# h22hyeon/PC-GNN

Measured on NVIDIA B200. Metric: train target-nodes/sec (fwd+bwd), higher is better.
Workload: dtype f32

## Files before the change

### include/pcgnn_b200.h

```cpp
#ifndef PCGNN_B200_H
#define PCGNN_B200_H

#include <stddef.h>
#include <stdint.h>

#ifdef __cplusplus
extern "C" {
#endif

#define PCG_SLOT 64
#define PCG_MAX_REL 8
#define PCG_NORM_MEAN 0
#define PCG_NORM_RSQRT 1

#define PCG_STATUS_WORDS 12
#define PCG_ST_SLOTS 0
#define PCG_ST_OVERFLOW 3

typedef void* pcg_stream_t;

#define PCG_API __attribute__((visibility("default")))

PCG_API const char* pcg_last_error(void);
PCG_API int pcg_version(void);
PCG_API int pcg_device_sms(void);
PCG_API int pcg_set_pdl(int mask);

PCG_API int pcg_score_table(const float* feat, int64_t n_nodes, int F, int64_t ldf, const float* w, const float* b,
                    float* score, const int32_t* pool, int P, float* ps_score, int32_t* ps_pos, int32_t* ps_id,
                    void* workspace, size_t workspace_bytes, pcg_stream_t stream);

PCG_API int pcg_pool_scores(const float* feat, int F, int64_t ldf, const float* w, const float* b, const int32_t* pool,
                    int P, float* pool_score, pcg_stream_t stream);

PCG_API int pcg_stage(const void* src, void* dst, size_t bytes, pcg_stream_t stream);
PCG_API void* pcg_host_device_ptr(void* host_ptr);
PCG_API int pcg_pool_scores_stage(const float* feat, int F, int64_t ldf, const float* w, const float* b, const int32_t* pool,
                          int P, float* pool_score, const void* stage_src, void* stage_dst, size_t stage_bytes,
                          const uint32_t* cursor, uint32_t count, int64_t src_stride_bytes, pcg_stream_t stream);
PCG_API int pcg_stage_indexed(const void* src, void* dst, size_t bytes, uint32_t* cursor, uint32_t count,
                      int64_t src_stride_bytes, int64_t dst_stride_bytes, int bump, pcg_stream_t stream);

PCG_API size_t pcg_sort_pool_workspace_bytes(int P);
PCG_API int pcg_sort_pool(const float* pool_score, const int32_t* pool, int P, float* ps_score, int32_t* ps_pos,
                  int32_t* ps_id, void* workspace, size_t workspace_bytes, pcg_stream_t stream);

PCG_API int pcg_pool_positions(const int32_t* pool, int P, int64_t n_nodes, int32_t* pool_pos_of, pcg_stream_t stream);
PCG_API int pcg_entry_pool_positions(const int32_t* indices, int64_t nnz, const int32_t* pool_pos_of,
                             int32_t* entry_pool_pos, pcg_stream_t stream);

PCG_API size_t pcg_choose_workspace_bytes(int B, int R, int64_t max_degree, int64_t n_nodes);
PCG_API size_t pcg_choose_sticky_offset(int64_t n_nodes);
PCG_API int pcg_choose_workspace_init(void* workspace, size_t workspace_bytes, int64_t n_nodes, pcg_stream_t stream);

PCG_API int pcg_choose(const int64_t* indptr, const int32_t* indices, int64_t n_nodes, int64_t row_lo, int R,
               const float* score,
               const float* entry_score, const float* center_score, const int32_t* targets,
               const int64_t* labels, int B, const double* thresh_host, const int32_t* k_override, double rho,
               const float* ps_score, const int32_t* ps_pos, const int32_t* ps_id, const int32_t* entry_pool_pos, int P,
               int train, int64_t max_degree,
               int32_t* sel_idx, float* sel_dist, int64_t cap_slots, int32_t* slot_item, int32_t* it_slot0,
               int32_t* it_m, int64_t* it_base, int32_t* it_done, int32_t* it_rep, void* workspace,
               size_t workspace_bytes, int32_t* status, int phases, pcg_stream_t stream);

PCG_API int pcg_select_all(const int64_t* indptr, const int32_t* indices, int64_t n_nodes, int R, const int32_t* targets,
                   int B, int add_self, int64_t cap_slots, int32_t* slot_item, int32_t* it_slot0, int32_t* it_m,
                   int64_t* it_base, int32_t* it_extra, int32_t* it_done, int32_t* status, pcg_stream_t stream);

PCG_API int pcg_aggregate(const float* feat, int64_t ldf, const int32_t* idx, const int32_t* slot_item,
                  const int32_t* it_slot0, const int32_t* it_m, const int64_t* it_base, const int32_t* it_extra,
                  const int32_t* it_rep, int copy_dups, int n_items, int64_t cap_slots, const int32_t* status,
                  int norm, float* partial, int32_t* it_done, float* agg, pcg_stream_t stream);

PCG_API int pcg_aggregate_bwd(const float* d_agg, int64_t ldf, const int32_t* idx, const int32_t* slot_item,
                      const int32_t* it_slot0, const int32_t* it_m, const int64_t* it_base, const int32_t* it_extra,
                      int n_items, int64_t cap_slots, const int32_t* status, int norm, float* feat_grad,
                      pcg_stream_t stream);

PCG_API int pcg_dense_fwd(const float* feat, int64_t ldf, int F, const int32_t* targets, int B, int R, int E,
                  const float* agg, const int32_t* agg_rep, const float* const* w_intra_host, const float* w_inter,
                  float* cat, float* out, pcg_stream_t stream);

PCG_API size_t pcg_dense_bwd_scratch_floats(int B, int R, int F, int E);
PCG_API int pcg_dense_bwd(int64_t ldf, int F, int B, int R, int E, const float* agg, const int32_t* agg_rep,
                  const float* w_inter,
                  const float* cat, const float* out, const float* d_out, float* const* d_w_intra_host,
                  float* d_w_inter, float* scratch, pcg_stream_t stream);

PCG_API int pcg_tile_supported(int B, int R, int F, int E);
PCG_API int pcg_tile_fwd(const float* feat, int64_t ldf, int F, const int32_t* targets, int B, int R, int E,
                 const float* agg, int64_t lda, const int32_t* agg_rep, const float* const* w_intra_host,
                 const float* w_inter, const float* w_clf, const float* b_clf, int keep_cat, float* out,
                 float* center, float* cat, pcg_stream_t stream);
PCG_API size_t pcg_tile_scratch_floats(int B, int R, int F, int E);
PCG_API int pcg_tile_train(const float* feat, int64_t ldf, int F, const int32_t* targets, int B, int R, int E,
                   const float* agg, int64_t lda, const int32_t* agg_rep, const float* const* w_intra_host,
                   const float* w_inter, const float* w_clf, const float* b_clf, const float* w_head,
                   const int64_t* labels, float lambda, float* out, float* center, float* logits, float* loss,
                   float* const* d_w_intra_host, float* d_w_inter, float* d_w_clf, float* d_b_clf, float* d_w_head,
                   float* scratch, int pdl, pcg_stream_t stream);

PCG_API size_t pcg_head_scratch_floats(int B, int F, int E);
PCG_API int pcg_center_fwd(const float* feat, int64_t ldf, int F, const int32_t* targets, int B, const float* w,
                   const float* b, float* center, pcg_stream_t stream);
PCG_API int pcg_center_bwd(const float* feat, int64_t ldf, int F, const int32_t* targets, int B, const float* d_center,
                   float* d_w, float* d_b, float* scratch, int32_t* ticket, pcg_stream_t stream);

PCG_API int pcg_head_loss_fwd(const float* emb, int E, int B, const float* w, const float* center,
                      const int64_t* labels, float lambda, float* logits, float* p1, float* q1, float* loss,
                      float* scratch, int32_t* ticket, pcg_stream_t stream);
PCG_API int pcg_head_loss_bwd(const float* emb, int E, int B, const float* w, const int64_t* labels, const float* p1,
                      const float* q1, float lambda, const float* d_loss, float* d_emb, float* d_center, float* d_w,
                      float* scratch, int32_t* ticket, pcg_stream_t stream);

PCG_API size_t pcg_encoder_scratch_floats(int B, int F_in, int E);
PCG_API int pcg_encoder_fwd(const float* agg, int64_t lda, const float* feat, int64_t ldf, const int32_t* targets, int F,
                    const float* w, int B, int E, float* out, pcg_stream_t stream);
PCG_API int pcg_encoder_bwd(const float* agg, int64_t lda, const float* feat, int64_t ldf, const int32_t* targets, int F,
                    int B, int E, const float* out, const float* d_out, float* d_w, float* scratch, int32_t* ticket,
                    pcg_stream_t stream);

PCG_API int pcg_pick_step(const double* cum, int64_t n, const double* u, int64_t k, const int32_t* idx_train,
                  int32_t* out, pcg_stream_t stream);
PCG_API int pcg_pick_step_philox(const double* cum, int64_t n, uint64_t seed, uint64_t offset, int64_t k,
                         const int32_t* idx_train, int32_t* out, pcg_stream_t stream);

PCG_API size_t pcg_comm_region_bytes(int64_t n_params);
PCG_API int pcg_comm_alloc(void** ptr, size_t bytes);
PCG_API int pcg_comm_free(void* ptr);
PCG_API int pcg_comm_export(void* ptr, unsigned char* handle64);
PCG_API int pcg_comm_import(const unsigned char* handle64, void** ptr);
PCG_API int pcg_comm_unmap(void* ptr);
PCG_API int pcg_allreduce_adam(float* grad, float* param, float* m, float* v, int64_t n_params,
                       void* const* peer_regions_host, int rank, int world, uint32_t* epoch, int32_t* ticket,
                       float lr, float beta1, float beta2, float eps, float weight_decay, int do_adam,
                       pcg_stream_t stream);

PCG_API size_t pcg_score_region_bytes(int64_t n_global);
PCG_API int pcg_score_bcast(const float* feat_rows, int64_t n_rows, int F, int64_t ldf, const float* w, const float* b,
                    int64_t row_lo, int64_t n_global, void* const* regions_host, int rank, int world,
                    uint32_t* epoch, pcg_stream_t stream);

#define PCG_METRICS_WORDS 17
#define PCG_MT_AUC 0
#define PCG_MT_F1 1
#define PCG_MT_F1_MACRO 2
#define PCG_MT_RECALL 3
#define PCG_MT_PRECISION 4
#define PCG_MT_RECALL_MACRO 5
#define PCG_MT_PRECISION_MACRO 6
#define PCG_MT_ACCURACY 7
#define PCG_MT_GMEAN 8
#define PCG_MT_BEST_F1_MACRO 9
#define PCG_MT_BEST_THRESHOLD 10
#define PCG_MT_N_POS 11
#define PCG_MT_N_NEG 12
#define PCG_MT_TP 13
#define PCG_MT_FP 14
#define PCG_MT_TN 15
#define PCG_MT_FN 16
PCG_API int pcg_eval_head(const float* emb, int E, int B, const float* w_head, int mode, int64_t n_total,
                  const uint32_t* cursor, uint32_t count, float* prob, pcg_stream_t stream);
PCG_API size_t pcg_binary_metrics_workspace_bytes(int64_t n);
PCG_API int pcg_binary_metrics(const float* prob, const int32_t* labels, int64_t n, double* out, void* workspace,
                       size_t workspace_bytes, pcg_stream_t stream);

#ifdef __cplusplus
}
#endif
#endif
```

### pc-gnn_b200/_lib.py

```python
from __future__ import annotations

import ctypes as C
import os

_HERE = os.path.dirname(os.path.abspath(__file__))
SO_PATH = os.path.join(_HERE, "libpcgnn_b200_trace.so" if os.environ.get("PCG_LIB_VARIANT") == "trace"
                       else "libpcgnn_b200.so")

SLOT = 64
MAX_REL = 8
STATUS_WORDS = 12
ST_SLOTS, ST_OVERFLOW = 0, 3
NORM_MEAN, NORM_RSQRT = 0, 1
KB_MAX_POOL = 8192
METRICS_KEYS = ("auc", "f1", "f1_macro", "recall", "precision", "recall_macro", "precision_macro", "accuracy", "gmean",
                "best_f1_macro", "best_threshold", "n_pos", "n_neg", "tp", "fp", "tn", "fn")
METRICS_WORDS = len(METRICS_KEYS)

_p = C.c_void_p
_i = C.c_int
_l = C.c_int64
_z = C.c_size_t
_d = C.c_double
_u64 = C.c_uint64

SIGNATURES = {
    "pcg_last_error": (C.c_char_p, []),
    "pcg_version": (_i, []),
    "pcg_device_sms": (_i, []),
    "pcg_set_pdl": (_i, [_i]),
    "pcg_score_table": (_i, [_p, _l, _i, _l, _p, _p, _p, _p, _i, _p, _p, _p, _p, _z, _p]),
    "pcg_pool_scores": (_i, [_p, _i, _l, _p, _p, _p, _i, _p, _p]),
    "pcg_stage": (_i, [_p, _p, _z, _p]),
    "pcg_host_device_ptr": (_p, [_p]),
    "pcg_pool_scores_stage": (_i, [_p, _i, _l, _p, _p, _p, _i, _p, _p, _p, _z, _p, C.c_uint32, _l, _p]),
    "pcg_stage_indexed": (_i, [_p, _p, _z, _p, C.c_uint32, _l, _l, _i, _p]),
    "pcg_sort_pool_workspace_bytes": (_z, [_i]),
    "pcg_sort_pool": (_i, [_p, _p, _i, _p, _p, _p, _p, _z, _p]),
    "pcg_choose_workspace_bytes": (_z, [_i, _i, _l, _l]),
    "pcg_choose_sticky_offset": (_z, [_l]),
    "pcg_choose_workspace_init": (_i, [_p, _z, _l, _p]),
    "pcg_pool_positions": (_i, [_p, _i, _l, _p, _p]),
    "pcg_entry_pool_positions": (_i, [_p, _l, _p, _p, _p]),
    "pcg_choose": (_i, [_p, _p, _l, _l, _i, _p, _p, _p, _p, _p, _i, C.POINTER(_d), _p, _d, _p, _p, _p, _p, _i, _i, _l,
                        _p, _p, _l, _p, _p, _p, _p, _p, _p, _p, _z, _p, _i, _p]),
    "pcg_select_all": (_i, [_p, _p, _l, _i, _p, _i, _i, _l, _p, _p, _p, _p, _p, _p, _p, _p]),
    "pcg_aggregate": (_i, [_p, _l, _p, _p, _p, _p, _p, _p, _p, _i, _i, _l, _p, _i, _p, _p, _p, _p]),
    "pcg_aggregate_bwd": (_i, [_p, _l, _p, _p, _p, _p, _p, _p, _i, _l, _p, _i, _p, _p]),
    "pcg_dense_fwd": (_i, [_p, _l, _i, _p, _i, _i, _i, _p, _p, C.POINTER(_p), _p, _p, _p, _p]),
    "pcg_dense_bwd_scratch_floats": (_z, [_i, _i, _i, _i]),
    "pcg_dense_bwd": (_i, [_l, _i, _i, _i, _i, _p, _p, _p, _p, _p, _p, C.POINTER(_p), _p, _p, _p]),
    "pcg_tile_supported": (_i, [_i, _i, _i, _i]),
    "pcg_tile_fwd": (_i, [_p, _l, _i, _p, _i, _i, _i, _p, _l, _p, C.POINTER(_p), _p, _p, _p, _i, _p, _p, _p, _p]),
    "pcg_tile_scratch_floats": (_z, [_i, _i, _i, _i]),
    "pcg_tile_train": (_i, [_p, _l, _i, _p, _i, _i, _i, _p, _l, _p, C.POINTER(_p), _p, _p, _p, _p, _p, C.c_float,
                            _p, _p, _p, _p, C.POINTER(_p), _p, _p, _p, _p, _p, _i, _p]),
    "pcg_head_scratch_floats": (_z, [_i, _i, _i]),
    "pcg_center_fwd": (_i, [_p, _l, _i, _p, _i, _p, _p, _p, _p]),
    "pcg_center_bwd": (_i, [_p, _l, _i, _p, _i, _p, _p, _p, _p, _p, _p]),
    "pcg_head_loss_fwd": (_i, [_p, _i, _i, _p, _p, _p, C.c_float, _p, _p, _p, _p, _p, _p, _p]),
    "pcg_head_loss_bwd": (_i, [_p, _i, _i, _p, _p, _p, _p, C.c_float, _p, _p, _p, _p, _p, _p, _p]),
    "pcg_encoder_scratch_floats": (_z, [_i, _i, _i]),
    "pcg_encoder_fwd": (_i, [_p, _l, _p, _l, _p, _i, _p, _i, _i, _p, _p]),
    "pcg_encoder_bwd": (_i, [_p, _l, _p, _l, _p, _i, _i, _i, _p, _p, _p, _p, _p, _p]),
    "pcg_comm_region_bytes": (_z, [_l]),
    "pcg_comm_alloc": (_i, [C.POINTER(_p), _z]),
    "pcg_comm_free": (_i, [_p]),
    "pcg_comm_export": (_i, [_p, C.c_char_p]),
    "pcg_comm_import": (_i, [C.c_char_p, C.POINTER(_p)]),
    "pcg_comm_unmap": (_i, [_p]),
    "pcg_allreduce_adam": (_i, [_p, _p, _p, _p, _l, C.POINTER(_p), _i, _i, _p, _p, C.c_float, C.c_float, C.c_float,
                                C.c_float, C.c_float, _i, _p]),
    "pcg_score_region_bytes": (_z, [_l]),
    "pcg_score_bcast": (_i, [_p, _l, _i, _l, _p, _p, _l, _l, C.POINTER(_p), _i, _i, _p, _p]),
    "pcg_pick_step": (_i, [_p, _l, _p, _l, _p, _p, _p]),
    "pcg_pick_step_philox": (_i, [_p, _l, _u64, _u64, _l, _p, _p, _p]),
    "pcg_eval_head": (_i, [_p, _i, _i, _p, _i, _l, _p, C.c_uint32, _p, _p]),
    "pcg_binary_metrics_workspace_bytes": (_z, [_l]),
    "pcg_binary_metrics": (_i, [_p, _p, _l, _p, _p, _z, _p]),
}

_lib = None


class PcgError(RuntimeError):
    pass


def lib():
    global _lib
    if _lib is None:
        if not os.path.exists(SO_PATH):
            raise PcgError(
                f"{SO_PATH} is missing: the CUDA extension has not been built "
                "(run `python -c \"import __graft_entry__ as g; g.build()\"`). There is no CPU fallback.")
        L = C.CDLL(SO_PATH)
        for name, (res, args) in SIGNATURES.items():
            fn = getattr(L, name)
            fn.restype = res
            fn.argtypes = args
        _lib = L
    return _lib


def check(rc: int, what: str = ""):
    if rc != 0:
        msg = lib().pcg_last_error().decode("utf-8", "replace")
        raise PcgError(f"{what or 'pcgnn_b200'} failed (code {rc}): {msg}")


def ptr(t):
    return None if t is None else t.data_ptr()


def host_device_ptr(pinned_tensor) -> int:
    dev = lib().pcg_host_device_ptr(pinned_tensor.data_ptr())
    if not dev:
        raise PcgError(lib().pcg_last_error().decode("utf-8", "replace"))
    return int(dev)


class capture:

    def __init__(self, graph, **kw):
        import torch

        self._ctx = torch.cuda.graph(graph, **kw)
        self._was = False

    def __enter__(self):
        import gc

        gc.collect()
        self._was = gc.isenabled()
        gc.disable()
        try:
            return self._ctx.__enter__()
        except BaseException:
            if self._was:
                gc.enable()
            raise

    def __exit__(self, *exc):
        import gc

        try:
            return self._ctx.__exit__(*exc)
        finally:
            if self._was:
                gc.enable()


def stream_ptr():
    import torch

    return torch.cuda.current_stream().cuda_stream
```

### pc-gnn_b200/csrc/pcg_choose.cu

```cuda
#include "pcg_common.cuh"

#include <cooperative_groups.h>
namespace cg = cooperative_groups;




#define PCG_SMALL_MAX 256
#define PCG_WARPS_PER_CTA 8
#define PCG_GRP_NT 256
#define PCG_CTA_MAX 2048
#define PCG_LARGE_NT 1024
#define PCG_CL 8
#define PCG_CL_MAX 16384
#define PCG_HUGE_MAX 131072
#define PCG_HUGE16_MAX 262144
#define PCG_KB_WORDS 256
#define PCG_CAND_CAP 2048
#define PCG_PREP_NT 1024

struct ChooseP {
    const int64_t* indptr;
    const int32_t* indices;
    const float* score;
    const float* entry_score;
    const float* center_score;
    const int32_t* targets;
    const int64_t* labels;
    const int32_t* k_override;
    const float* ps_score;
    const int32_t* ps_pos;
    const int32_t* ps_id;
    const int32_t* entry_pool_pos;
    int64_t n_nodes;
    int64_t row_lo;
    int R, B, P, train;
    double thresh[PCG_MAX_REL];
    double rho;
    int32_t* sel_idx;
    float* sel_dist;
    int64_t cap_slots;
    int32_t* slot_item;
    int32_t* it_slot0;
    int32_t* it_m;
    int64_t* it_base;
    int32_t* it_done;
    int32_t* it_rep;
    int32_t* status;
    int32_t* first;
    int32_t* q_warp;
    int32_t* q_cta;
    int32_t* q_cl;
    int32_t* q_huge;
    int32_t* q_huge16;
    int huge16_ok;
    int32_t* q_big;
    uint32_t* bits_slab;
    int64_t slab_words;
    int32_t* sticky;
};

#ifdef PCG_TRACE
#define PCG_TRACE_SLOTS 40
__device__ long long* g_trace = nullptr;
__device__ __forceinline__ long long trace_now() {
    long long t;
    asm volatile("mov.u64 %0, %%globaltimer;" : "=l"(t));
    return t;
}
#define TRACE(slot) do { if (g_trace && tid == 0) g_trace[(int64_t)w * PCG_TRACE_SLOTS + (slot)] = trace_now(); } while (0)
#define TRACE_VAL(slot, val) do { if (g_trace && tid == 0) g_trace[(int64_t)w * PCG_TRACE_SLOTS + (slot)] = (val); } while (0)
#define PTRACE(slot) do { if (g_trace && threadIdx.x == 0) g_trace[(int64_t)p.R * p.B * PCG_TRACE_SLOTS + (slot)] = trace_now(); } while (0)
#define TRACE0(slot) do { if (g_trace && tid == 0 && cg::this_cluster().block_rank() == 0) g_trace[(int64_t)w * PCG_TRACE_SLOTS + (slot)] = trace_now(); } while (0)
#define TRACE0_VAL(slot, val) do { if (g_trace && tid == 0 && cg::this_cluster().block_rank() == 0) g_trace[(int64_t)w * PCG_TRACE_SLOTS + (slot)] = (val); } while (0)
#else
#define PTRACE(slot) do {} while (0)
#define TRACE(slot) do {} while (0)
#define TRACE_VAL(slot, val) do {} while (0)
#define TRACE0(slot) do {} while (0)
#define TRACE0_VAL(slot, val) do {} while (0)
#endif
template <int NT>
__device__ __forceinline__ void grp_sync() {
    if (NT == 32) __syncwarp(); else __syncthreads();
}

template <int NT>
__device__ __forceinline__ void grp_excl2(bool fa, bool fb, int tid, int* xw, int& ea, int& eb, int& ta, int& tb) {
    const unsigned lt = lanemask_lt();
    unsigned ma = __ballot_sync(PCG_FULL, fa), mb = __ballot_sync(PCG_FULL, fb);
    ea = __popc(ma & lt);
    eb = __popc(mb & lt);
    if (NT == 32) {
        ta = __popc(ma);
        tb = __popc(mb);
    } else {
        constexpr int NW = NT / 32;
        const int wid = tid >> 5, lane = tid & 31;
        if (lane == 0) xw[wid] = __popc(ma) | (__popc(mb) << 16);
        __syncthreads();
        int pk = lane < NW ? xw[lane] : 0;
        int incl = pk;
#pragma unroll
        for (int off = 1; off < NW; off <<= 1) {
            int t = __shfl_up_sync(PCG_FULL, incl, off);
            if (lane >= off) incl += t;
        }
        const int tot = __shfl_sync(PCG_FULL, incl, NW - 1);
        const int mine = __shfl_sync(PCG_FULL, incl - pk, wid);
        ea += mine & 0xffff;
        eb += mine >> 16;
        ta = tot & 0xffff;
        tb = tot >> 16;
        __syncthreads();
    }
}

template <int NT, class Get>
__device__ __forceinline__ void grp_minmax(Get get, int n, int tid, int* xw, uint32_t& kmin, uint32_t& kmax) {
    uint32_t lo = 0xffffffffu, hi = 0u;
    for (int j = tid; j < n; j += NT) { const uint32_t x = get(j); lo = min(lo, x); hi = max(hi, x); }
#pragma unroll
    for (int off = 16; off > 0; off >>= 1) {
        lo = min(lo, __shfl_xor_sync(PCG_FULL, lo, off));
        hi = max(hi, __shfl_xor_sync(PCG_FULL, hi, off));
    }
    if (NT > 32) {
        if (tid == 0) { xw[24] = (int)0xffffffffu; xw[25] = 0; }
        __syncthreads();
        if ((tid & 31) == 0) { atomicMin((uint32_t*)&xw[24], lo); atomicMax((uint32_t*)&xw[25], hi); }
        __syncthreads();
        lo = (uint32_t)xw[24];
        hi = (uint32_t)xw[25];
        __syncthreads();
    }
    kmin = lo;
    kmax = hi;
}
template <int NT, class Get>
__device__ __forceinline__ void radix_select(Get get, int n, int kth, uint32_t* hist, int* xw, int tid, uint32_t& T,
                                             int& need) {
    uint32_t kmin, kmax;
    grp_minmax<NT>(get, n, tid, xw, kmin, kmax);
    if (kmin == kmax) { T = kmin; need = kth; return; }
    int hb = 31 - __clz(kmin ^ kmax);
    uint32_t mask = hb == 31 ? 0u : ~((2u << hb) - 1u);
    uint32_t prefix = kmin & mask;
    int remaining = kth;
    bool first = true;
    while (hb >= 0) {
        const int shift = max(hb - 7, 0);
        const uint32_t dmask = (1u << (hb - shift + 1)) - 1u;
        for (int b = tid; b < 256; b += NT) hist[b] = 0;
        grp_sync<NT>();
        const int n_up = (n + 31) & ~31;
        for (int j = tid; j < n_up; j += NT) {
            const bool valid = j < n;
            const uint32_t key = valid ? get(j) : 0u;
            const bool active = valid && (key & mask) == prefix;
            const uint32_t digit = (key >> shift) & dmask;
            if (first) {
                unsigned rem = __ballot_sync(PCG_FULL, active);
#pragma unroll 1
                for (int it = 0; it < 2 && rem; ++it) {
                    const int ldr = __ffs(rem) - 1;
                    const uint32_t d0 = __shfl_sync(PCG_FULL, digit, ldr);
                    const unsigned same = __ballot_sync(PCG_FULL, active && digit == d0);
                    if ((tid & 31) == ldr) atomicAdd(&hist[d0], (uint32_t)__popc(same));
                    rem &= ~same;
                }
                if ((rem >> (tid & 31)) & 1u) atomicAdd(&hist[digit], 1u);
            } else if (active) {
                atomicAdd(&hist[digit], 1u);
            }
        }
        grp_sync<NT>();
        if (tid < 32) {
            uint32_t c[8];
            int s = 0;
#pragma unroll
            for (int b = 0; b < 8; ++b) { c[b] = hist[tid * 8 + b]; s += (int)c[b]; }
            int incl = s;
#pragma unroll
            for (int off = 1; off < 32; off <<= 1) {
                int t = __shfl_up_sync(PCG_FULL, incl, off);
                if (tid >= off) incl += t;
            }
            int excl = incl - s;
            if (excl < remaining && remaining <= incl) {
                int run = excl;
#pragma unroll
                for (int b = 0; b < 8; ++b) {
                    if (run + (int)c[b] >= remaining) { xw[30] = tid * 8 + b; xw[31] = remaining - run; break; }
                    run += (int)c[b];
                }
            }
        }
        grp_sync<NT>();
        const uint32_t digit = (uint32_t)xw[30];
        remaining = xw[31];
        prefix |= digit << shift;
        mask |= dmask << shift;
        hb = shift - 1;
        first = false;
    }
    T = prefix;
    need = remaining;
}

__device__ __forceinline__ uint32_t pick_digit(int c0, int c1, int c2, int& remaining) {
    if (remaining <= c0) return 0u;
    remaining -= c0;
    if (remaining <= c1) return 1u;
    remaining -= c1;
    if (remaining <= c2) return 2u;
    remaining -= c2;
    return 3u;
}

template <int NT, class Get>
__device__ __forceinline__ void cta_bitselect(Get get, int n, int kth, uint32_t* cand, int cand_cap, int* wsum, int* xw,
                                              int tid, uint32_t& T, int& need) {
    constexpr int NW = NT / 32;
    const int wid = tid >> 5, lane = tid & 31;
    uint32_t kmin, kmax;
    grp_minmax<NT>(get, n, tid, xw, kmin, kmax);
    if (kmin == kmax) { T = kmin; need = kth; return; }
    int hb = 31 - __clz(kmin ^ kmax);
    uint32_t mask = hb == 31 ? 0u : ~((2u << hb) - 1u);
    uint32_t prefix = kmin & mask;
    int remaining = kth;
    bool listed = false;
    int n_list = 0;
    int n_act = n;
    while (hb >= 0) {
        const int shift = max(hb - 1, 0);
        const uint32_t dmask = hb >= 1 ? 3u : 1u;
        int c0 = 0, c1 = 0, c2 = 0;
        const int lim = listed ? n_list : n;
        for (int j = tid; j < lim; j += NT) {
            const uint32_t key = listed ? cand[j] : get(j);
            const bool active = ((key ^ prefix) & mask) == 0u;
            const uint32_t dg = (key >> shift) & dmask;
            c0 += active && dg == 0u;
            c1 += active && dg == 1u;
            c2 += active && dg == 2u;
        }
        c0 = __reduce_add_sync(PCG_FULL, c0);
        c1 = __reduce_add_sync(PCG_FULL, c1);
        c2 = __reduce_add_sync(PCG_FULL, c2);
        if (lane == 0) { wsum[wid * 3] = c0; wsum[wid * 3 + 1] = c1; wsum[wid * 3 + 2] = c2; }
        __syncthreads();
        c0 = lane < NW ? wsum[lane * 3] : 0;
        c1 = lane < NW ? wsum[lane * 3 + 1] : 0;
        c2 = lane < NW ? wsum[lane * 3 + 2] : 0;
        c0 = __reduce_add_sync(PCG_FULL, c0);
        c1 = __reduce_add_sync(PCG_FULL, c1);
        c2 = __reduce_add_sync(PCG_FULL, c2);
        const uint32_t dg = pick_digit(c0, c1, c2, remaining);
        const int cnt_dg = dg == 0u ? c0 : (dg == 1u ? c1 : (dg == 2u ? c2 : n_act - c0 - c1 - c2));
        prefix |= dg << shift;
        mask |= dmask << shift;
        hb = shift - 1;
        n_act = cnt_dg;
        __syncthreads();
        if (!listed && hb >= 0 && n_act <= cand_cap) {
            if (tid == 0) xw[26] = 0;
            __syncthreads();
            const int n_up = (n + 31) & ~31;
            for (int j = tid; j < n_up; j += NT) {
                const uint32_t key = j < n ? get(j) : 0u;
                const bool active = j < n && ((key ^ prefix) & mask) == 0u;
                const unsigned m = __ballot_sync(PCG_FULL, active);
                int base = 0;
                if (lane == 0 && m) base = atomicAdd(&xw[26], __popc(m));
                base = __shfl_sync(PCG_FULL, base, 0);
                if (active) cand[base + __popc(m & lanemask_lt())] = key;
            }
            __syncthreads();
            listed = true;
            n_list = n_act;
        }
    }
    T = prefix;
    need = remaining;
}
template <int NT, int NE, int CL = 1>
__device__ __forceinline__ void hist_select(const uint32_t (&key)[NE], uint32_t vmask, int kth, uint32_t* hist, int* xw,
                                            int tid, uint32_t& T, int& need, uint32_t* chist = nullptr,
                                            int* par = nullptr, int w = 0) {

    constexpr int NH = NT == 32 ? 1 : 8;
    const int lane = tid & 31, wid = tid >> 5;
    uint32_t* myh = hist + (NT == 32 ? 0 : (wid & (NH - 1)) * 256);
    uint32_t prefix = 0u, mask = 0u;
    int remaining = kth;
#pragma unroll 1
    for (int step = 0; step < 4; ++step) {
        const int shift = step == 3 ? 0 : 23 - 8 * step;
        const uint32_t dmask = step == 3 ? 0x7fu : 0xffu;
        if (step == 0) {
            uint32_t pd[3];
            {
                const bool a0 = vmask & 1u;
                const uint32_t dg0 = key[0] >> 23;
                unsigned rem = __ballot_sync(PCG_FULL, a0);
#pragma unroll
                for (int q = 0; q < 3; ++q) {
                    const int ldr = rem ? __ffs(rem) - 1 : 0;
                    pd[q] = rem ? __shfl_sync(PCG_FULL, dg0, ldr) : 0xffffffffu;
                    rem &= ~__ballot_sync(PCG_FULL, a0 && dg0 == pd[q]);
                }
            }
            int pc0 = 0, pc1 = 0, pc2 = 0;
#pragma unroll
            for (int e = 0; e < NE; ++e) {
                const bool active = (vmask >> e) & 1u;
                const uint32_t digit = key[e] >> 23;
                const bool m0 = active && digit == pd[0], m1 = active && digit == pd[1], m2 = active && digit == pd[2];
                pc0 += m0; pc1 += m1; pc2 += m2;
                if (active && !(m0 || m1 || m2)) atomicAdd(&myh[digit], 1u);
            }
            pc0 = __reduce_add_sync(PCG_FULL, pc0);
            pc1 = __reduce_add_sync(PCG_FULL, pc1);
            pc2 = __reduce_add_sync(PCG_FULL, pc2);
            if (lane == 0 && pc0) atomicAdd(&myh[pd[0]], (uint32_t)pc0);
            if (lane == 1 && pc1) atomicAdd(&myh[pd[1]], (uint32_t)pc1);
            if (lane == 2 && pc2) atomicAdd(&myh[pd[2]], (uint32_t)pc2);
        } else {
#pragma unroll
            for (int e = 0; e < NE; ++e) {
                const bool active = ((vmask >> e) & 1u) && ((key[e] ^ prefix) & mask) == 0u;
                if (active) atomicAdd(&myh[(key[e] >> shift) & dmask], 1u);
            }
        }
        grp_sync<NT>();
        if (CL > 1) { TRACE0(12 + 4 * step); TRACE0_VAL(11, step + 1); }
        int dg = -1, rem_in = 0, cnt_in = 0;
        if (NT == 32) {
            uint32_t c[8];
            int s = 0;
#pragma unroll
            for (int b = 0; b < 8; ++b) { c[b] = hist[lane * 8 + b]; hist[lane * 8 + b] = 0u; s += (int)c[b]; }
            int incl = s;
#pragma unroll
            for (int off = 1; off < 32; off <<= 1) {
                const int t = __shfl_up_sync(PCG_FULL, incl, off);
                if (lane >= off) incl += t;
            }
            int run = incl - s;
            if (run < remaining && remaining <= incl) {
#pragma unroll
                for (int b = 0; b < 8; ++b) {
                    if (dg < 0 && run + (int)c[b] >= remaining) { dg = lane * 8 + b; rem_in = remaining - run; cnt_in = (int)c[b]; }
                    run += (int)c[b];
                }
            }
            const unsigned who = __ballot_sync(PCG_FULL, dg >= 0);
            const int src = __ffs(who) - 1;
            dg = __shfl_sync(PCG_FULL, dg, src);
            rem_in = __shfl_sync(PCG_FULL, rem_in, src);
            cnt_in = __shfl_sync(PCG_FULL, cnt_in, src);
        } else {
            int c = 0, incl = 0;
            if (tid < 256) {
#pragma unroll
                for (int h = 0; h < NH; ++h) { c += (int)hist[h * 256 + tid]; hist[h * 256 + tid] = 0u; }
            }
            if (CL > 1) {
                cg::cluster_group cl = cg::this_cluster();
                uint32_t* mine_h = chist + *par * 256 + (tid & 255);
                if (tid < 256) *mine_h = (uint32_t)c;
                cl.sync();
                TRACE0(13 + 4 * step);
                if (tid < 256) {
                    c = 0;
#pragma unroll
                    for (int r = 0; r < CL; ++r) c += (int)*cl.map_shared_rank(mine_h, r);
                }
                *par ^= 1;
                TRACE0(14 + 4 * step);
            }
            if (tid < 256) {
                incl = c;
#pragma unroll
                for (int off = 1; off < 32; off <<= 1) {
                    const int t = __shfl_up_sync(PCG_FULL, incl, off);
                    if (lane >= off) incl += t;
                }
                if (lane == 31) xw[wid] = incl;
            }
            __syncthreads();
            if (tid < 256) {
                int base = 0;
#pragma unroll
                for (int q = 0; q < 8; ++q) base += q < wid ? xw[q] : 0;
                const int excl = base + incl - c;
                if (excl < remaining && remaining <= excl + c) { xw[16] = tid; xw[17] = remaining - excl; xw[18] = c; }
            }
            __syncthreads();
            dg = xw[16]; rem_in = xw[17]; cnt_in = xw[18];
            if (CL > 1) TRACE0(15 + 4 * step);
        }
        remaining = rem_in;
        prefix |= (uint32_t)dg << shift;
        mask |= dmask << shift;
        if (cnt_in == 1 && step < 3) {
            uint32_t mine = 0u;
            bool have = false;
#pragma unroll
            for (int e = 0; e < NE; ++e)
                if (((vmask >> e) & 1u) && ((key[e] ^ prefix) & mask) == 0u) { mine = key[e]; have = true; }
            if (NT == 32) {
                const unsigned who = __ballot_sync(PCG_FULL, have);
                prefix = __shfl_sync(PCG_FULL, mine, __ffs(who) - 1);
            } else if (CL == 1) {
                if (have) xw[19] = (int)mine;
                __syncthreads();
                prefix = (uint32_t)xw[19];
            } else {
                cg::cluster_group cl = cg::this_cluster();
                if (have)
                    for (int r = 0; r < CL; ++r) *cl.map_shared_rank(&xw[19], r) = (int)mine;
                cl.sync();
                prefix = (uint32_t)xw[19];
            }
            break;
        }
    }
    T = prefix;
    need = remaining;
}

template <class Pred>
__device__ __forceinline__ int warp_partition_point(int lo, int hi, Pred pred) {
    const int lane = threadIdx.x & 31;
    while (hi > lo) {
        const int span = hi - lo;
        const int step = (span + 31) >> 5;
        const int idx = lo + lane * step;
        const bool t = idx < hi ? pred(idx) : false;
        const int cnt = __popc(__ballot_sync(PCG_FULL, t));
        if (cnt == 0) return lo;
        const int nlo = lo + (cnt - 1) * step + 1;
        hi = min(hi, lo + cnt * step);
        lo = nlo;
    }
    return lo;
}
struct Item {
    int w, r, i, d, k, o, nslots, slot0;
    int32_t v;
    int64_t beg, off;
    float sv;
    bool use_kb, want_bits;
};

__device__ __forceinline__ void item_header(const ChooseP& p, int w, Item& it) {
    it.w = w;
    it.r = w / p.B;
    it.i = w - it.r * p.B;
    it.v = p.targets[it.i];
    const int64_t row = (int64_t)it.r * p.n_nodes + (it.v - p.row_lo);
    it.beg = p.indptr[row];
    it.d = (int)(p.indptr[row + 1] - it.beg);
    it.sv = p.center_score ? p.center_score[it.i] : p.score[it.v];
    const bool positive = p.train && p.labels && p.labels[it.i] == 1;
    item_counts(it.d, p.thresh[it.r], p.rho, positive, p.P, p.k_override ? p.k_override[w] : 0, p.k_override != nullptr,
                it.k, it.o);
    it.nslots = (it.k + it.o + PCG_SLOT - 1) / PCG_SLOT;
    it.slot0 = p.it_slot0[w];
    it.off = (int64_t)it.slot0 * PCG_SLOT;
    it.use_kb = it.o > 0 && p.entry_pool_pos != nullptr && p.P <= PCG_KB_WORDS * 32;
    it.want_bits = it.o > 0 && !it.use_kb;
}

template <int NT>
__device__ __forceinline__ int oversample(const ChooseP& p, const Item& it, int tid, const int32_t* __restrict__ nbr,
                                          const uint32_t* kbits, const uint32_t* bits, uint32_t* hist, int* xw) {
    const float* __restrict__ S = p.ps_score;
    const int32_t* __restrict__ SP = p.ps_pos;
    const int32_t* __restrict__ SI = p.ps_id;
    const int P = p.P, o = it.o, k = it.k, d = it.d;
    const float sv = it.sv;
    const int w = it.w;
    int c = 0, a_less = 0, a_le = 0, b_less = 0, b_le = 0;
    uint32_t Tp = 0;
    if (NT == 32 || tid < 32) {
        c = warp_partition_point(0, P, [&](int q) { return __ldg(S + q) < sv; });
        const int nA0 = c, nB0 = P - c;
        auto A0 = [&](int q) -> uint32_t { return dist_bits(sv, __ldg(S + (c - 1 - q))); };
        auto B0 = [&](int q) -> uint32_t { return dist_bits(sv, __ldg(S + (c + q))); };
        const int ia = warp_partition_point(max(0, o - nB0), min(o, nA0), [&](int m) { return B0(o - m - 1) > A0(m); });
        const int ib = o - ia;
        if (ia > 0) Tp = A0(ia - 1);
        if (ib > 0) Tp = max(Tp, B0(ib - 1));
        a_less = warp_partition_point(0, nA0, [&](int q) { return A0(q) < Tp; });
        a_le = warp_partition_point(a_less, nA0, [&](int q) { return A0(q) <= Tp; });
        b_less = warp_partition_point(0, nB0, [&](int q) { return B0(q) < Tp; });
        b_le = warp_partition_point(b_less, nB0, [&](int q) { return B0(q) <= Tp; });
    }
    if (NT > 32) {
        if (tid == 0) {
            hist[64] = (uint32_t)c; hist[65] = (uint32_t)a_less; hist[66] = (uint32_t)a_le;
            hist[67] = (uint32_t)b_less; hist[68] = (uint32_t)b_le; hist[69] = Tp;
        }
        __syncthreads();
        c = (int)hist[64]; a_less = (int)hist[65]; a_le = (int)hist[66];
        b_less = (int)hist[67]; b_le = (int)hist[68]; Tp = hist[69];
        __syncthreads();
    }
    if (NT > 32) { TRACE(31); }
    const int cnt_less = a_less + b_less;
    const int tie_a = a_le - a_less, ties = tie_a + (b_le - b_less);
    const int needp = o - cnt_less;
    auto tie_index = [&](int t) -> int { return t < tie_a ? c - 1 - (a_less + t) : c + b_less + (t - tie_a); };
    uint32_t Tpos = 0xffffffffu;
    if (needp < ties) {
        auto getpos = [&](int t) -> uint32_t { return (uint32_t)__ldg(SP + tie_index(t)); };
        int unused;
        radix_select<NT>(getpos, ties, needp, hist, xw, tid, Tpos, unused);
    }
    TRACE(5);
    const int total = cnt_less + ties;
    int run_sel = 0, n_emit = 0;
    for (int base = 0; base < total; base += NT) {
        const int e = base + tid;
        const bool valid = e < total;
        int idx = 0, pos = 0;
        if (valid) {
            idx = e < a_less ? c - 1 - e : (e < cnt_less ? c + (e - a_less) : tie_index(e - cnt_less));
            pos = __ldg(SP + idx);
        }
        const bool selp = valid && (e < cnt_less || (uint32_t)pos <= Tpos);
        bool emit = false;
        int32_t id = 0;
        if (selp) {
            id = __ldg(SI + idx);
            bool dup;
            if (it.use_kb) {
                dup = (kbits[pos >> 5] >> (pos & 31)) & 1u;
            } else {
                int l = 0, h = d;
                while (l < h) {
                    const int mid = (l + h) >> 1;
                    if (nbr[mid] < id) l = mid + 1; else h = mid;
                }
                dup = l < d && nbr[l] == id && ((k == d) || ((bits[l >> 5] >> (l & 31)) & 1u));
            }
            emit = !dup;
        }
        int es, ee, ts, te;
        grp_excl2<NT>(selp, emit, tid, xw, es, ee, ts, te);
        if (selp && p.sel_dist) p.sel_dist[it.off + k + run_sel + es] = __uint_as_float(dist_bits(sv, __ldg(S + idx)));
        if (emit) p.sel_idx[it.off + k + n_emit + ee] = id;
        run_sel += ts;
        n_emit += te;
    }
    return n_emit;
}

template <int NT>
__device__ __forceinline__ void item_finish(const ChooseP& p, const Item& it, int tid, int m) {
    if (tid == 0) {
        p.it_slot0[it.w] = it.slot0;
        p.it_m[it.w] = m;
        p.it_base[it.w] = it.off;
        p.it_done[it.w] = 0;
    }
    for (int c = tid; c < it.nslots; c += NT) p.slot_item[it.slot0 + c] = (c * PCG_SLOT < m) ? it.w : -1;
}
struct WarpSmem {
    uint32_t shist[256];
    uint32_t hist[256];
    uint32_t kbits[PCG_KB_WORDS];
    uint32_t bits[PCG_SMALL_MAX / 32];
    int xw[32];
};

template <int NT, int NE>
__device__ __forceinline__ void row_in_regs(const ChooseP& p, const Item& it, const int32_t* __restrict__ nbr,
                                            uint32_t* kbits, uint32_t* bits, uint32_t* hist, int* xw) {
    const int tid = NT == 32 ? (threadIdx.x & 31) : threadIdx.x;
    const int lane = tid & 31;
    const int w = it.w;
    const int d = it.d, k = it.k;
    const float* __restrict__ escore = p.entry_score ? p.entry_score + it.beg : nullptr;
    const int32_t* __restrict__ epp = it.use_kb ? p.entry_pool_pos + it.beg : nullptr;
    const bool all = k >= d;
    const bool need_dist = !all || p.sel_dist != nullptr;
    int32_t id[NE];
    int pp[NE];
    uint32_t key[NE];
    uint32_t vmask = 0;
#pragma unroll
    for (int e = 0; e < NE; ++e) {
        const int j = e * NT + tid;
        const bool valid = j < d;
        vmask |= (uint32_t)valid << e;
        id[e] = valid ? __ldg(nbr + j) : 0;
        pp[e] = (valid && epp) ? __ldg(epp + j) : -1;
    }
#pragma unroll
    for (int e = 0; e < NE; ++e) {
        const int j = e * NT + tid;
        uint32_t x = 0u;
        if (((vmask >> e) & 1u) && need_dist) x = dist_bits(it.sv, escore ? escore[j] : __ldg(p.score + id[e]));
        key[e] = x;
    }
    TRACE(2);
    uint32_t T = 0xffffffffu;
    int need = 0x7fffffff;
    if (!all) {
        if (k > 0) hist_select<NT, NE>(key, vmask, k, hist, xw, tid, T, need);
        else { T = 0; need = 0; }
    }
    TRACE(3);
    int run_less = 0, run_tie = 0;
#pragma unroll
    for (int e = 0; e < NE; ++e) {
        if (e * NT < d) {
            const bool valid = (vmask >> e) & 1u;
            const bool less = valid && (all || key[e] < T);
            const bool tie = valid && !all && key[e] == T;
            int el, et, tl, tt;
            grp_excl2<NT>(less, tie, tid, xw, el, et, tl, tt);
            const int tie_before = run_tie + et;
            const bool sel = less || (tie && tie_before < need);
            if (sel) {
                const int64_t at = it.off + run_less + el + min(tie_before, need);
                p.sel_idx[at] = id[e];
                if (p.sel_dist) p.sel_dist[at] = __uint_as_float(key[e]);
                if (pp[e] >= 0) atomicOr(&kbits[pp[e] >> 5], 1u << (pp[e] & 31));
            }
            if (it.want_bits) {
                const unsigned sm = __ballot_sync(PCG_FULL, sel);
                if (lane == 0) bits[(e * NT + tid) >> 5] = sm;
            }
            run_less += tl;
            run_tie += tt;
        }
    }
    grp_sync<NT>();
    TRACE(4);
}
__device__ void choose_item_warp(const ChooseP& p, int w, WarpSmem& s) {
    const int lane = threadIdx.x & 31;
    const int tid = lane;
    Item it;
    item_header(p, w, it);
    TRACE(0); TRACE_VAL(8, it.d); TRACE_VAL(9, it.k); TRACE_VAL(10, it.o);
    TRACE(1);
    const int32_t* __restrict__ nbr = p.indices + it.beg;
    if (it.use_kb) {
        for (int q = lane; q < (p.P + 31) >> 5; q += 32) s.kbits[q] = 0u;
        __syncwarp();
    }
    const int d = it.d;
    if (d <= 32) row_in_regs<32, 1>(p, it, nbr, s.kbits, s.bits, s.shist, s.xw);
    else if (d <= 64) row_in_regs<32, 2>(p, it, nbr, s.kbits, s.bits, s.shist, s.xw);
    else if (d <= 128) row_in_regs<32, 4>(p, it, nbr, s.kbits, s.bits, s.shist, s.xw);
    else row_in_regs<32, 8>(p, it, nbr, s.kbits, s.bits, s.shist, s.xw);
    int m = it.k;
    if (it.o > 0) m += oversample<32>(p, it, lane, nbr, s.kbits, s.bits, s.hist, s.xw);
    TRACE(6);
    item_finish<32>(p, it, lane, m);
    __syncwarp();
    TRACE(7);
}


template <int NT>
struct CtaSmem {
    uint32_t hist[8 * 256];
    uint32_t chist[2 * 256];
    int ctot;
    int cnt[16 * (NT / 32)];
    int pre[16 * (NT / 32)];
    uint32_t ohist[256];
    uint32_t kbits[PCG_KB_WORDS];
    uint32_t bits[PCG_CL_MAX / 32];
    int xw[32];
};

template <int NT, int NE, int CL>
__device__ __forceinline__ void cta_body(const ChooseP& p, const Item& it, CtaSmem<NT>& s, int32_t* sid, int16_t* spp,
                                         uint32_t* bits_local, int rank, int* par) {
    constexpr int NW = NT / 32;
    constexpr bool STASH = NT > PCG_GRP_NT;
    const int tid = threadIdx.x, lane = tid & 31, wid = tid >> 5;
    const int w = it.w;
    const int d = it.d, k = it.k;
    const int32_t* __restrict__ nbr = p.indices + it.beg;
    const float* __restrict__ escore = p.entry_score ? p.entry_score + it.beg : nullptr;
    const int32_t* __restrict__ epp = it.use_kb ? p.entry_pool_pos + it.beg : nullptr;
    const bool all = k >= d;
    const bool need_dist = !all || p.sel_dist != nullptr;
    const int pos0 = rank * (NE * NT) + tid;
    uint32_t key[NE];
    int32_t id[NE];
    int pp[NE];
    uint32_t vmask = 0;
#pragma unroll
    for (int e = 0; e < NE; ++e) {
        const int j = pos0 + e * NT;
        const bool valid = j < d;
        vmask |= (uint32_t)valid << e;
        id[e] = valid ? __ldg(nbr + j) : 0;
        pp[e] = (valid && epp) ? __ldg(epp + j) : -1;
    }
#pragma unroll
    for (int e = 0; e < NE; ++e) {
        const int j = pos0 + e * NT;
        uint32_t x = 0u;
        if (((vmask >> e) & 1u) && need_dist) x = dist_bits(it.sv, escore ? escore[j] : __ldg(p.score + id[e]));
        key[e] = x;
        if (STASH) { sid[e * NT + tid] = id[e]; spp[e * NT + tid] = (int16_t)pp[e]; }
    }
    TRACE(2);
    uint32_t T = 0xffffffffu;
    int need = 0x7fffffff;
    if (!all) {
        if (k > 0) hist_select<NT, NE, CL>(key, vmask, k, s.hist, s.xw, tid, T, need, s.chist, par, w);
        else { T = 0; need = 0; }
    }
    TRACE(3);
    const unsigned lt = lanemask_lt();
#pragma unroll
    for (int e = 0; e < NE; ++e) {
        const bool valid = (vmask >> e) & 1u;
        const unsigned ml = __ballot_sync(PCG_FULL, valid && (all || key[e] < T));
        const unsigned mt = __ballot_sync(PCG_FULL, valid && !all && key[e] == T);
        if (lane == 0) s.cnt[e * NW + wid] = __popc(ml) | (__popc(mt) << 16);
    }
    __syncthreads();
    if (CL > 1) TRACE0(28);
    if (wid == 0) {
        constexpr int PER = (NE * NW + 31) / 32;
        int v[PER], sum = 0;
#pragma unroll
        for (int q = 0; q < PER; ++q) {
            const int at = lane * PER + q;
            v[q] = at < NE * NW ? s.cnt[at] : 0;
            sum += v[q];
        }
        int incl = sum;
#pragma unroll
        for (int off = 1; off < 32; off <<= 1) {
            const int t = __shfl_up_sync(PCG_FULL, incl, off);
            if (lane >= off) incl += t;
        }
        int run = incl - sum;
#pragma unroll
        for (int q = 0; q < PER; ++q) {
            const int at = lane * PER + q;
            if (at < NE * NW) s.pre[at] = run;
            run += v[q];
        }
        if (CL > 1 && lane == 31) s.ctot = incl;
    }
    int base_less = 0, base_tie = 0;
    uint32_t* kbits0 = s.kbits;
    uint32_t* bits0 = bits_local;
    if (CL > 1) {
        cg::cluster_group cl = cg::this_cluster();
        cl.sync();
        TRACE0(29);
        for (int c = 0; c < rank; ++c) {
            const int t = *cl.map_shared_rank(&s.ctot, c);
            base_less += t & 0xffff;
            base_tie += t >> 16;
        }
        kbits0 = cl.map_shared_rank(&s.kbits[0], 0);
        bits0 = cl.map_shared_rank(bits_local, 0);
    } else {
        __syncthreads();
    }
#pragma unroll
    for (int e = 0; e < NE; ++e) {
        const int j = pos0 + e * NT;
        const bool valid = (vmask >> e) & 1u;
        const bool less = valid && (all || key[e] < T);
        const bool tie = valid && !all && key[e] == T;
        const unsigned ml = __ballot_sync(PCG_FULL, less), mt = __ballot_sync(PCG_FULL, tie);
        const int pl = s.pre[e * NW + wid];
        const int tie_before = base_tie + (pl >> 16) + __popc(mt & lt);
        const bool sel = less || (tie && tie_before < need);
        if (sel) {
            const int64_t at = it.off + base_less + (pl & 0xffff) + __popc(ml & lt) + min(tie_before, need);
            p.sel_idx[at] = STASH ? sid[e * NT + tid] : id[e];
            if (p.sel_dist) p.sel_dist[at] = __uint_as_float(key[e]);
            const int q = STASH ? (int)spp[e * NT + tid] : pp[e];
            if (q >= 0) atomicOr(&kbits0[q >> 5], 1u << (q & 31));
        }
        if (it.want_bits) {
            const unsigned sm = __ballot_sync(PCG_FULL, sel);
            if (lane == 0 && j < d) bits0[j >> 5] = sm;
        }
    }
    TRACE(4);
}

template <int NT, int CL>
__device__ __forceinline__ void cta_item(const ChooseP& p, int w, CtaSmem<NT>& s, int32_t* sid, int16_t* spp,
                                         uint32_t* bits_local, int rank, int* par) {
    const int tid = threadIdx.x;
    Item it;
    item_header(p, w, it);
    TRACE(0); TRACE_VAL(8, it.d); TRACE_VAL(9, it.k); TRACE_VAL(10, it.o);
    if (rank == 0 && it.use_kb)
        for (int q = tid; q < (p.P + 31) >> 5; q += NT) s.kbits[q] = 0u;
    TRACE(1);
    const int per = (it.d + CL * NT - 1) / (CL * NT);
    constexpr int NE_MAX = NT == PCG_GRP_NT ? 8 : 16;
    if (per <= 1) cta_body<NT, 1, CL>(p, it, s, sid, spp, bits_local, rank, par);
    else if (per <= 2) cta_body<NT, 2, CL>(p, it, s, sid, spp, bits_local, rank, par);
    else if (per <= 4 || NE_MAX == 4) cta_body<NT, 4, CL>(p, it, s, sid, spp, bits_local, rank, par);
    else if (per <= 8 || NE_MAX == 8) cta_body<NT, (NE_MAX < 8 ? NE_MAX : 8), CL>(p, it, s, sid, spp, bits_local, rank, par);
    else cta_body<NT, NE_MAX, CL>(p, it, s, sid, spp, bits_local, rank, par);
    if (CL > 1) {
        if (it.o > 0) cg::this_cluster().sync();
        TRACE0(30);
        if (rank != 0) return;
    }
    __syncthreads();
    int m = it.k;
    if (it.o > 0) m += oversample<NT>(p, it, tid, p.indices + it.beg, s.kbits, bits_local, s.ohist, s.xw);
    TRACE(6);
    item_finish<NT>(p, it, tid, m);
    __syncthreads();
    TRACE(7);
}

__global__ void __launch_bounds__(PCG_GRP_NT, 3) k_choose_small(ChooseP p) {
    constexpr size_t SM_BYTES = sizeof(CtaSmem<PCG_GRP_NT>) > sizeof(WarpSmem) * PCG_WARPS_PER_CTA
                                    ? sizeof(CtaSmem<PCG_GRP_NT>) : sizeof(WarpSmem) * PCG_WARPS_PER_CTA;
    __shared__ __align__(16) unsigned char raw[SM_BYTES];
    __shared__ int s_q;
    const int wid = threadIdx.x >> 5, lane = threadIdx.x & 31;
#pragma unroll 1
    for (int phase = 0; phase < 2; ++phase) {
        const bool cta_phase = ((blockIdx.x + phase) & 1) == 0;
        __syncthreads();
        if (cta_phase) {
            CtaSmem<PCG_GRP_NT>& s = *reinterpret_cast<CtaSmem<PCG_GRP_NT>*>(raw);
            for (int b = threadIdx.x; b < 8 * 256; b += PCG_GRP_NT) s.hist[b] = 0u;
            const int n = p.status[ST_NMID];
            for (;;) {
                __syncthreads();
                if (threadIdx.x == 0) s_q = atomicAdd(&p.status[ST_MID_CTR], 1);
                __syncthreads();
                const int q = s_q;
                if (q >= n) break;
                cta_item<PCG_GRP_NT, 1>(p, p.q_cta[q], s, nullptr, nullptr, s.bits, 0, nullptr);
            }
        } else {
            WarpSmem& ws = reinterpret_cast<WarpSmem*>(raw)[wid];
            for (int b = lane; b < 256; b += 32) ws.shist[b] = 0u;
            __syncwarp();
            const int n = p.status[ST_NSMALL];
            for (;;) {
                int q = 0;
                if (lane == 0) q = atomicAdd(&p.status[ST_SMALL_CTR], 1);
                q = __shfl_sync(PCG_FULL, q, 0);
                if (q >= n) break;
                choose_item_warp(p, p.q_warp[q], ws);
            }
        }
    }
}

__global__ void __cluster_dims__(PCG_CL, 1, 1) __launch_bounds__(PCG_GRP_NT, 3) k_choose_wide(ChooseP p) {
    __shared__ CtaSmem<PCG_GRP_NT> s;
    cg::cluster_group cl = cg::this_cluster();
    const int rank = (int)cl.block_rank();
    for (int b = threadIdx.x; b < 8 * 256; b += PCG_GRP_NT) s.hist[b] = 0u;
    __syncthreads();
    const int n = p.status[ST_NCL];
    const int n_cl = gridDim.x / PCG_CL, cid = blockIdx.x / PCG_CL;
    int par = 0;
    for (int q = cid; q < n; q += n_cl) cta_item<PCG_GRP_NT, PCG_CL>(p, p.q_cl[q], s, nullptr, nullptr, s.bits, rank, &par);
    cl.sync();
}

#define PCG_HUGE_PER_CTA (PCG_HUGE_MAX / PCG_CL)
template <int CL>
__global__ void __launch_bounds__(PCG_LARGE_NT, 1) k_choose_huge(ChooseP p) {
    extern __shared__ uint32_t dyn_huge[];
    int32_t* sid = reinterpret_cast<int32_t*>(dyn_huge);
    int16_t* spp = reinterpret_cast<int16_t*>(dyn_huge + PCG_HUGE_PER_CTA);
    uint32_t* bits = dyn_huge + PCG_HUGE_PER_CTA + PCG_HUGE_PER_CTA / 2;
    __shared__ CtaSmem<PCG_LARGE_NT> s;
    cg::cluster_group cl = cg::this_cluster();
    const int rank = (int)cl.block_rank();
    for (int b = threadIdx.x; b < 8 * 256; b += PCG_LARGE_NT) s.hist[b] = 0u;
    __syncthreads();
    const int n = p.status[CL == 16 ? ST_NHUGE16 : ST_NHUGE];
    const int32_t* queue = CL == 16 ? p.q_huge16 : p.q_huge;
    const int n_cl = gridDim.x / CL, cid = blockIdx.x / CL;
    int par = 0;
    for (int q = cid; q < n; q += n_cl) cta_item<PCG_LARGE_NT, CL>(p, queue[q], s, sid, spp, bits, rank, &par);
    cl.sync();
}

template <int CL>
static cudaError_t launch_huge(const ChooseP& p, int n_clusters, cudaStream_t stream, bool probe_only, int* max_clusters) {
    const size_t dyn = (size_t)PCG_HUGE_PER_CTA * 6 + (size_t)CL * PCG_HUGE_PER_CTA / 8;
    static bool configured_dev[PCG_MAX_DEVICES];
    bool& configured = configured_dev[pcg_current_device()];
    cudaError_t e;
    if (!configured) {
        e = cudaFuncSetAttribute(k_choose_huge<CL>, cudaFuncAttributeMaxDynamicSharedMemorySize, (int)dyn);
        if (e != cudaSuccess) return e;
        if (CL > 8) {
            e = cudaFuncSetAttribute(k_choose_huge<CL>, cudaFuncAttributeNonPortableClusterSizeAllowed, 1);
            if (e != cudaSuccess) return e;
        }
        configured = true;
    }
    cudaLaunchConfig_t cfg = {};
    cfg.gridDim = dim3((unsigned)(n_clusters * CL));
    cfg.blockDim = dim3(PCG_LARGE_NT);
    cfg.dynamicSmemBytes = dyn;
    cfg.stream = stream;
    cudaLaunchAttribute attr[1];
    attr[0].id = cudaLaunchAttributeClusterDimension;
    attr[0].val.clusterDim.x = CL; attr[0].val.clusterDim.y = 1; attr[0].val.clusterDim.z = 1;
    cfg.attrs = attr;
    cfg.numAttrs = 1;
    if (probe_only) return cudaOccupancyMaxActiveClusters(max_clusters, k_choose_huge<CL>, &cfg);
    return cudaLaunchKernelEx(&cfg, k_choose_huge<CL>, p);
}

__device__ void choose_item_big(const ChooseP& p, int w, uint32_t* sd, int sd_cap, uint32_t* hist, uint32_t* kbits,
                                uint32_t* cand, uint32_t* bits, int* xw) {
    constexpr int NT = PCG_LARGE_NT, NW = NT / 32;
    const int tid = threadIdx.x, wid = tid >> 5, lane = tid & 31;
    Item it;
    item_header(p, w, it);
    TRACE(0); TRACE_VAL(8, it.d); TRACE_VAL(9, it.k); TRACE_VAL(10, it.o);
    if (it.use_kb)
        for (int q = tid; q < (p.P + 31) >> 5; q += NT) kbits[q] = 0u;
    __syncthreads();
    TRACE(1);
    const int d = it.d, k = it.k;
    const float sv = it.sv;
    const int32_t* __restrict__ nbr = p.indices + it.beg;
    const float* __restrict__ escore = p.entry_score ? p.entry_score + it.beg : nullptr;
    const float* __restrict__ score = p.score;
    const bool cached = d <= sd_cap;
    if (cached) {
#pragma unroll 4
        for (int j = tid; j < d; j += NT) sd[j] = dist_bits(sv, escore ? escore[j] : __ldg(score + __ldg(nbr + j)));
        __syncthreads();
    }
    auto get = [&](int j) -> uint32_t {
        return cached ? sd[j] : dist_bits(sv, escore ? escore[j] : __ldg(score + __ldg(nbr + j)));
    };
    TRACE(2);
    uint32_t T = 0xffffffffu;
    int need = 0x7fffffff;
    if (k < d) {
        if (k > 0) cta_bitselect<NT>(get, d, k, cand, PCG_CAND_CAP, reinterpret_cast<int*>(hist), xw, tid, T, need);
        else { T = 0; need = 0; }
    }
    TRACE(3);
    const int chunk = (((d + NW - 1) / NW) + 31) & ~31;
    const int cb = min(d, wid * chunk), ce = min(d, cb + chunk);
    int cl = 0, ct = 0;
    if (k < d) {
        for (int base = cb; base < ce; base += 32) {
            const int j = base + lane;
            const uint32_t key = j < ce ? get(j) : 0xffffffffu;
            cl += __popc(__ballot_sync(PCG_FULL, j < ce && key < T));
            ct += __popc(__ballot_sync(PCG_FULL, j < ce && key == T));
        }
    } else {
        cl = ce - cb;
    }
    if (lane == 0) { xw[wid] = cl; hist[wid] = (uint32_t)ct; }
    __syncthreads();
    int run_less = 0, run_tie = 0;
    for (int q = 0; q < wid; ++q) { run_less += xw[q]; run_tie += (int)hist[q]; }
    __syncthreads();
    const int32_t* __restrict__ epp = it.use_kb ? p.entry_pool_pos + it.beg : nullptr;
    int32_t id_n = cb + lane < ce ? __ldg(nbr + cb + lane) : 0;
    int pp_n = (epp && cb + lane < ce) ? __ldg(epp + cb + lane) : -1;
    for (int base = cb; base < ce; base += 32) {
        const int j = base + lane;
        const bool valid = j < ce;
        const int32_t id = id_n;
        const int pp = pp_n;
        if (j + 32 < ce) {
            id_n = __ldg(nbr + j + 32);
            pp_n = epp ? __ldg(epp + j + 32) : -1;
        }
        const uint32_t key = (valid && (k < d || p.sel_dist)) ? get(j) : 0u;
        const bool less = valid && (k >= d || key < T);
        const bool tie = valid && k < d && key == T;
        const unsigned lt = lanemask_lt();
        const unsigned ml = __ballot_sync(PCG_FULL, less), mt = __ballot_sync(PCG_FULL, tie);
        const int tie_before = run_tie + __popc(mt & lt);
        const bool sel = less || (tie && tie_before < need);
        if (sel) {
            const int64_t at = it.off + run_less + __popc(ml & lt) + min(tie_before, need);
            p.sel_idx[at] = id;
            if (p.sel_dist) p.sel_dist[at] = __uint_as_float(key);
            if (pp >= 0) atomicOr(&kbits[pp >> 5], 1u << (pp & 31));
        }
        if (it.want_bits) {
            const unsigned sm = __ballot_sync(PCG_FULL, sel);
            if (lane == 0) bits[base >> 5] = sm;
        }
        run_less += __popc(ml);
        run_tie += __popc(mt);
    }
    __syncthreads();
    TRACE(4);
    int m = k;
    if (it.o > 0) m += oversample<NT>(p, it, tid, nbr, kbits, bits, hist, xw);
    TRACE(6);
    item_finish<NT>(p, it, tid, m);
    __syncthreads();
    TRACE(7);
}

__global__ void __launch_bounds__(PCG_LARGE_NT, 1) k_choose_big(ChooseP p, int sd_cap) {
    extern __shared__ uint32_t dyn[];
    __shared__ uint32_t hist[256];
    __shared__ uint32_t kbits[PCG_KB_WORDS];
    __shared__ uint32_t cand[PCG_CAND_CAP];
    __shared__ int xw[32];
    const int n = p.status[ST_NBIG];
    for (int q = blockIdx.x; q < n; q += gridDim.x)
        choose_item_big(p, p.q_big[q], dyn, sd_cap, hist, kbits, cand, p.bits_slab + (int64_t)blockIdx.x * p.slab_words, xw);
}

#define PCG_PREP_CHUNK 512
#define PCG_PREP_ITEMS 8192

__device__ __forceinline__ void prep_grid_barrier(int32_t* bar, int target) {
    __syncthreads();
    if (threadIdx.x == 0) {
        __threadfence();
        atomicAdd(&bar[0], 1);
        while (*(volatile int32_t*)&bar[0] < target) { }
        __threadfence();
    }
    __syncthreads();
}

template <bool CLUSTER>
__global__ void __launch_bounds__(PCG_PREP_NT, 1) k_choose_prep(ChooseP p, int chunk, int32_t* bar, int32_t* totals) {
    __shared__ int s_info[PCG_PREP_ITEMS];
    __shared__ int s_wsum[32];
    __shared__ int s_base;
    constexpr int NT = PCG_PREP_NT;
    const int tid = threadIdx.x, lane = tid & 31, wid = tid >> 5;
    const int B = p.B, W = p.R * p.B, G = gridDim.x;
    int32_t* first = p.first;
    PTRACE(0);
    if (first)
        for (int i = blockIdx.x * NT + tid; i < B; i += G * NT) {
            const int64_t lv = (int64_t)__ldg(p.targets + i) - p.row_lo;
            if (lv >= 0 && lv < p.n_nodes) atomicMin(&first[lv], i);
        }
    if (blockIdx.x == 0 && tid < PCG_STATUS_WORDS) p.status[tid] = 0;
    auto barrier = [&](int target) {
        if (CLUSTER) { __threadfence(); cg::this_cluster().sync(); }
        else prep_grid_barrier(bar, target);
    };
    barrier(G);
    PTRACE(1);
    const int w0 = min(W, blockIdx.x * chunk), n_items = min(W, w0 + chunk) - w0;
    for (int q0 = tid; q0 < n_items; q0 += 4 * NT) {
        int rr[4], ii[4], rep[4];
        int64_t beg[4], end[4];
        bool pos[4];
#pragma unroll
        for (int u = 0; u < 4; ++u) {
            const int q = q0 + u * NT;
            const int w = w0 + q;
            rr[u] = w / B;
            ii[u] = w - rr[u] * B;
            rep[u] = -1;
            beg[u] = end[u] = 0;
            pos[u] = false;
            if (q < n_items) {
                const int64_t lv = (int64_t)__ldg(p.targets + ii[u]) - p.row_lo;
                if (lv >= 0 && lv < p.n_nodes) {
                    rep[u] = first ? __ldcg(first + lv) : ii[u];
                    const int64_t row = (int64_t)rr[u] * p.n_nodes + lv;
                    beg[u] = __ldg(p.indptr + row);
                    end[u] = __ldg(p.indptr + row + 1);
                    pos[u] = p.train && p.labels && __ldg(p.labels + ii[u]) == 1;
                } else {
                    rep[u] = -2;
                }
            }
        }
#pragma unroll
        for (int u = 0; u < 4; ++u) {
            const int q = q0 + u * NT;
            if (q < n_items) {
                const int w = w0 + q;
                int info = 0;
                p.it_rep[w] = rep[u] >= 0 ? rr[u] * B + rep[u] : w;
                if (rep[u] == -2) {
                    p.it_slot0[w] = 0; p.it_m[w] = 0; p.it_base[w] = 0; p.it_done[w] = 0;
                    atomicExch(&p.status[ST_OVERFLOW], 2);
                    atomicOr(p.sticky, 2);
                }
                if (rep[u] == ii[u]) {
                    const int64_t d = end[u] - beg[u];
                    int k, o;
                    item_counts(d, p.thresh[rr[u]], p.rho, pos[u], p.P, p.k_override ? p.k_override[w] : 0,
                                p.k_override != nullptr, k, o);
                    const int tier = d <= PCG_SMALL_MAX ? 0 : (d <= PCG_CTA_MAX ? 1 : (d <= PCG_CL_MAX ? 2 : (d <= PCG_HUGE_MAX ? 3 :
                                     ((d <= PCG_HUGE16_MAX && p.huge16_ok) ? 4 : 5))));
                    info = (((k + o + PCG_SLOT - 1) / PCG_SLOT) << 3) | (tier + 1);
                }
                s_info[q] = info;
            }
        }
    }
    __syncthreads();
    PTRACE(2);
    const int per = (n_items + NT - 1) / NT;
    const int c0 = min(n_items, tid * per), c1 = min(n_items, c0 + per);
    int mine = 0;
    for (int q = c0; q < c1; ++q) mine += s_info[q] >> 3;
    int incl = mine;
#pragma unroll
    for (int off = 1; off < 32; off <<= 1) {
        const int t = __shfl_up_sync(PCG_FULL, incl, off);
        if (lane >= off) incl += t;
    }
    if (lane == 31) s_wsum[wid] = incl;
    __syncthreads();
    const int ws = s_wsum[lane];
    int wincl = ws;
#pragma unroll
    for (int off = 1; off < 32; off <<= 1) {
        const int t = __shfl_up_sync(PCG_FULL, wincl, off);
        if (lane >= off) wincl += t;
    }
    const int cta_total = __shfl_sync(PCG_FULL, wincl, 31);
    if (tid == 0) totals[blockIdx.x] = cta_total;
    barrier(2 * G);
    if (wid == 0) {
        int acc = 0;
        for (int c = lane; c < (int)blockIdx.x; c += 32) acc += __ldcg(totals + c);
        acc = __reduce_add_sync(PCG_FULL, acc);
        if (lane == 0) s_base = acc;
    }
    __syncthreads();
    int slot0 = s_base + __shfl_sync(PCG_FULL, wincl - ws, wid) + incl - mine;
    bool overflow = false;
    int32_t* const queues[6] = {p.q_warp, p.q_cta, p.q_cl, p.q_huge, p.q_huge16, p.q_big};
    const int counters[6] = {ST_NSMALL, ST_NMID, ST_NCL, ST_NHUGE, ST_NHUGE16, ST_NBIG};
    for (int c = 0; c < per; ++c) {
        const int q = c0 + c;
        int tier = -1;
        if (q < c1) {
            const int info = s_info[q];
            if (info) {
                const int w = w0 + q, nsl = info >> 3;
                tier = (info & 7) - 1;
                if ((int64_t)slot0 + nsl > p.cap_slots) {
                    overflow = true;
                    tier = -1;
                    p.it_slot0[w] = 0; p.it_m[w] = 0; p.it_base[w] = 0; p.it_done[w] = 0;
                    for (int x = 0; x < nsl; ++x)
                        if ((int64_t)slot0 + x < p.cap_slots) p.slot_item[slot0 + x] = -1;
                } else {
                    p.it_slot0[w] = slot0;
                }
                slot0 += nsl;
            }
        }
        unsigned tm[6];
#pragma unroll
        for (int t = 0; t < 6; ++t) tm[t] = __ballot_sync(PCG_FULL, tier == t);
        int qb = 0;
#pragma unroll
        for (int t = 0; t < 6; ++t)
            if (lane == t && tm[t]) qb = atomicAdd(&p.status[counters[t]], __popc(tm[t]));
#pragma unroll
        for (int t = 0; t < 6; ++t) {
            const int b = __shfl_sync(PCG_FULL, qb, t);
            if (tier == t) queues[t][b + __popc(tm[t] & lanemask_lt())] = w0 + q;
        }
    }
    PTRACE(3);
    if (__syncthreads_or(overflow) && tid == 0) { atomicExch(&p.status[ST_OVERFLOW], 1); atomicOr(p.sticky, 1); }
    if (first)
        for (int i = blockIdx.x * NT + tid; i < B; i += G * NT) {
            const int64_t lv = (int64_t)__ldg(p.targets + i) - p.row_lo;
            if (lv >= 0 && lv < p.n_nodes) first[lv] = 0x7f7f7f7f;
        }
    if (tid == 0) {
        if (blockIdx.x == G - 1) p.status[ST_SLOTS] = s_base + cta_total;
        if (!CLUSTER) {
            __threadfence();
            if (atomicAdd(&bar[1], 1) == G - 1) { bar[0] = 0; bar[1] = 0; }
        }
    }
    PTRACE(4);
}

__global__ void k_select_all(const int64_t* __restrict__ indptr, const int32_t* __restrict__ indices, int64_t n_nodes,
                             int R, const int32_t* __restrict__ targets, int B, int add_self, int64_t cap_slots,
                             int32_t* slot_item, int32_t* it_slot0, int32_t* it_m, int64_t* it_base, int32_t* it_extra,
                             int32_t* it_done, int32_t* status) {
    const int w = (blockIdx.x * blockDim.x + threadIdx.x) >> 5, lane = threadIdx.x & 31;
    if (w >= R * B) return;
    const int r = w / B, i = w - r * B;
    const int32_t v = targets[i];
    const int64_t row = (int64_t)r * n_nodes + v;
    const int64_t beg = indptr[row];
    const int d = (int)(indptr[row + 1] - beg);
    int extra = -1;
    if (add_self) {
        int lo = 0, hi = d;
        while (lo < hi) {
            int mid = (lo + hi) >> 1;
            if (indices[beg + mid] < v) lo = mid + 1; else hi = mid;
        }
        if (!(lo < d && indices[beg + lo] == v)) extra = v;
    }
    int nslots = (d + PCG_SLOT - 1) / PCG_SLOT;
    if (nslots == 0 && extra >= 0) nslots = 1;
    int slot0 = 0;
    if (lane == 0) slot0 = atomicAdd(&status[ST_SLOTS], nslots);
    slot0 = __shfl_sync(PCG_FULL, slot0, 0);
    const bool ovf = (int64_t)slot0 + nslots > cap_slots;
    if (lane == 0) {
        if (ovf) atomicExch(&status[ST_OVERFLOW], 1);
        it_slot0[w] = ovf ? 0 : slot0;
        it_m[w] = ovf ? 0 : d;
        it_base[w] = beg;
        it_extra[w] = ovf ? -1 : extra;
        it_done[w] = 0;
    }
    for (int c = lane; c < nslots; c += 32)
        if ((int64_t)slot0 + c < cap_slots) slot_item[slot0 + c] = ovf ? -1 : w;
}

__global__ void k_fill_i32(int32_t* a, int64_t n, int32_t val) {
    const int64_t i = (int64_t)blockIdx.x * blockDim.x + threadIdx.x;
    if (i < n) a[i] = val;
}
__global__ void k_pool_positions(const int32_t* __restrict__ pool, int P, int32_t* __restrict__ pool_pos_of) {
    const int i = blockIdx.x * blockDim.x + threadIdx.x;
    if (i < P) pool_pos_of[pool[i]] = i;
}

__global__ void k_entry_pool_pos(const int32_t* __restrict__ indices, int64_t nnz,
                                 const int32_t* __restrict__ pool_pos_of, int32_t* __restrict__ out) {
    const int64_t e = (int64_t)blockIdx.x * blockDim.x + threadIdx.x;
    if (e < nnz) out[e] = pool_pos_of[indices[e]];
}
struct WsLayout {
    size_t first, bar, totals, bits_slab, q_warp, q_cta, q_cl, q_huge, q_huge16, q_big, total;
    int64_t slab_words;
    int grid_big;
};

static WsLayout ws_layout(int B, int R, int64_t max_degree, int64_t n_nodes, int sms) {
    WsLayout L;
    size_t W = (size_t)B * R;
    auto al = [](size_t x) { return (x + 255) & ~(size_t)255; };
    L.grid_big = sms;
    L.slab_words = max_degree > PCG_HUGE_MAX ? (max_degree + 31) / 32 : 0;
    size_t o = 0;
    L.first = o; o = al(o + (size_t)n_nodes * 4);
    L.bar = o; o = al(o + 16);
    L.totals = o; o = al(o + 1024 * 4);
    L.bits_slab = o; o = al(o + (size_t)L.grid_big * L.slab_words * 4);
    L.q_warp = o; o = al(o + W * 4);
    L.q_cta = o; o = al(o + W * 4);
    L.q_cl = o; o = al(o + W * 4);
    L.q_huge = o; o = al(o + W * 4);
    L.q_huge16 = o; o = al(o + W * 4);
    L.q_big = o; o = al(o + W * 4);
    L.total = o;
    return L;
}

static int g_sms[PCG_MAX_DEVICES];
static int device_sms() {
    const int dev = pcg_current_device();
    if (g_sms[dev] == 0) {
        if (cudaDeviceGetAttribute(&g_sms[dev], cudaDevAttrMultiProcessorCount, dev) != cudaSuccess || g_sms[dev] <= 0)
            g_sms[dev] = 148;
    }
    return g_sms[dev];
}

extern "C" int pcg_device_sms(void) { return device_sms(); }

#ifdef PCG_TRACE
extern "C" __attribute__((visibility("default"))) int pcg_debug_set_trace(long long* buf) {
    return (int)cudaMemcpyToSymbol(g_trace, &buf, sizeof(buf));
}
#endif

extern "C" size_t pcg_choose_workspace_bytes(int B, int R, int64_t max_degree, int64_t n_nodes) {
    return ws_layout(B, R, max_degree, n_nodes, 148 * 2).total;
}

extern "C" size_t pcg_choose_sticky_offset(int64_t n_nodes) { return ws_layout(1, 1, 0, n_nodes, 148).bar + 8; }

extern "C" int pcg_choose_workspace_init(void* workspace, size_t workspace_bytes, int64_t n_nodes, pcg_stream_t stream_) {
    cudaStream_t stream = (cudaStream_t)stream_;
    WsLayout L = ws_layout(1, 1, 0, n_nodes, 148);
    PCG_REQUIRE(workspace && workspace_bytes >= L.bar + 16, "pcg_choose_workspace_init: workspace too small");
    cudaError_t e = cudaMemsetAsync(workspace, 0x7f, (size_t)n_nodes * 4, stream);
    if (e == cudaSuccess) e = cudaMemsetAsync((char*)workspace + L.bar, 0, 16, stream);
    if (e != cudaSuccess) { pcg_set_error("pcg_choose_workspace_init: memset: %s", cudaGetErrorString(e)); return (int)e; }
    return 0;
}

extern "C" int pcg_pool_positions(const int32_t* pool, int P, int64_t n_nodes, int32_t* pool_pos_of,
                                  pcg_stream_t stream_) {
    cudaStream_t stream = (cudaStream_t)stream_;
    PCG_REQUIRE(pool_pos_of && (P == 0 || pool), "pcg_pool_positions: null pointer");
    if (n_nodes > 0) k_fill_i32<<<(int)((n_nodes + 255) / 256), 256, 0, stream>>>(pool_pos_of, n_nodes, -1);
    if (P > 0) k_pool_positions<<<(P + 255) / 256, 256, 0, stream>>>(pool, P, pool_pos_of);
    return pcg_check_launch("pcg_pool_positions");
}

extern "C" int pcg_entry_pool_positions(const int32_t* indices, int64_t nnz, const int32_t* pool_pos_of,
                                        int32_t* entry_pool_pos, pcg_stream_t stream_) {
    cudaStream_t stream = (cudaStream_t)stream_;
    PCG_REQUIRE(nnz == 0 || (indices && pool_pos_of && entry_pool_pos), "pcg_entry_pool_positions: null pointer");
    if (nnz > 0)
        k_entry_pool_pos<<<(unsigned)((nnz + 255) / 256), 256, 0, stream>>>(indices, nnz, pool_pos_of, entry_pool_pos);
    return pcg_check_launch("pcg_entry_pool_positions");
}

#define PCG_N_SIDE 3
struct SideState {
    cudaStream_t side[PCG_N_SIDE];
    cudaEvent_t fork, join[PCG_N_SIDE];
    int huge16_state;
    size_t big_smem;
};
static SideState g_dev[PCG_MAX_DEVICES];

extern "C" int pcg_choose(const int64_t* indptr, const int32_t* indices, int64_t n_nodes, int64_t row_lo, int R,
                          const float* score,
                          const float* entry_score, const float* center_score, const int32_t* targets,
                          const int64_t* labels, int B, const double* thresh_host, const int32_t* k_override,
                          double rho, const float* ps_score, const int32_t* ps_pos, const int32_t* ps_id,
                          const int32_t* entry_pool_pos, int P, int train,
                          int64_t max_degree, int32_t* sel_idx, float* sel_dist, int64_t cap_slots,
                          int32_t* slot_item, int32_t* it_slot0, int32_t* it_m, int64_t* it_base, int32_t* it_done,
                          int32_t* it_rep, void* workspace, size_t workspace_bytes, int32_t* status, int phases,
                          pcg_stream_t stream_) {
    cudaStream_t stream = (cudaStream_t)stream_;
    PCG_REQUIRE(R >= 1 && R <= PCG_MAX_REL, "pcg_choose: R=%d outside [1,%d]", R, PCG_MAX_REL);
    PCG_REQUIRE(phases >= 1 && phases <= 3, "pcg_choose: phases must be 1 (prepare), 2 (select) or 3 (both)");
    PCG_REQUIRE(B >= 0, "pcg_choose: negative batch");
    if (B == 0) {
        if (status) cudaMemsetAsync(status, 0, PCG_STATUS_WORDS * sizeof(int32_t), stream);
        return 0;
    }
    PCG_REQUIRE((phases & 2) == 0 || score || (entry_score && center_score), "pcg_choose: need a score table or explicit scores");
    PCG_REQUIRE(!(train && P > 0) || (ps_score && ps_pos && ps_id), "pcg_choose: sorted pool arrays missing");
    PCG_REQUIRE(indptr && indices && targets && sel_idx && slot_item && it_slot0 && it_m && it_base && it_done &&
                    it_rep && status,
                "pcg_choose: null pointer");
    const int sms = device_sms();
    WsLayout L = ws_layout(B, R, max_degree, n_nodes, sms);
    PCG_REQUIRE(workspace && workspace_bytes >= L.total, "pcg_choose: workspace too small (%zu < %zu)", workspace_bytes,
                L.total);
    cudaError_t e;
    ChooseP p;
    p.indptr = indptr; p.indices = indices; p.score = score; p.entry_score = entry_score;
    p.center_score = center_score; p.targets = targets; p.labels = labels; p.k_override = k_override;
    p.ps_score = ps_score; p.ps_pos = ps_pos; p.ps_id = ps_id; p.entry_pool_pos = entry_pool_pos;
    p.n_nodes = n_nodes; p.row_lo = row_lo; p.R = R; p.B = B;
    p.P = (train && ps_score) ? P : 0; p.train = train;
    for (int r = 0; r < PCG_MAX_REL; ++r) p.thresh[r] = r < R ? thresh_host[r] : 0.5;
    p.rho = rho; p.sel_idx = sel_idx; p.sel_dist = sel_dist; p.cap_slots = cap_slots; p.slot_item = slot_item;
    p.it_slot0 = it_slot0; p.it_m = it_m; p.it_base = it_base; p.it_done = it_done; p.it_rep = it_rep; p.status = status;
    char* ws = (char*)workspace;
    p.first = entry_score == nullptr ? (int32_t*)(ws + L.first) : nullptr;
    p.q_warp = (int32_t*)(ws + L.q_warp);
    p.q_cta = (int32_t*)(ws + L.q_cta);
    p.q_cl = (int32_t*)(ws + L.q_cl);
    p.q_huge = (int32_t*)(ws + L.q_huge);
    p.q_huge16 = (int32_t*)(ws + L.q_huge16);
    p.q_big = (int32_t*)(ws + L.q_big);
    p.sticky = (int32_t*)(ws + L.bar) + 2;
    p.bits_slab = (uint32_t*)(ws + L.bits_slab);
    p.slab_words = L.slab_words;
    const int W = R * B;
    SideState& S = g_dev[pcg_current_device()];
    cudaStream_t* g_side = S.side;
    cudaEvent_t* g_join = S.join;
    cudaEvent_t& g_fork = S.fork;
    if (S.huge16_state == 0) {
        int mc = 0;
        cudaError_t pe = launch_huge<16>(p, 1, stream, true, &mc);
        S.huge16_state = (pe == cudaSuccess && mc >= 1) ? 1 : 2;
        (void)cudaGetLastError();
    }
    p.huge16_ok = S.huge16_state == 1;
    if (phases & 1) {
        cudaLaunchConfig_t cfg = {};
        cfg.blockDim = dim3(PCG_PREP_NT);
        cfg.dynamicSmemBytes = 0;
        cfg.stream = stream;
        cudaLaunchAttribute attr[1];
        cfg.attrs = attr;
        cfg.numAttrs = 1;
        if (W <= 8 * PCG_PREP_ITEMS) {
            int G = 8;
            while (G > 1 && W < G * 64) G >>= 1;
            const int chunk = (W + G - 1) / G;
            cfg.gridDim = dim3((unsigned)G);
            attr[0].id = cudaLaunchAttributeClusterDimension;
            attr[0].val.clusterDim.x = (unsigned)G; attr[0].val.clusterDim.y = 1; attr[0].val.clusterDim.z = 1;
            e = cudaLaunchKernelEx(&cfg, k_choose_prep<true>, p, chunk, (int32_t*)(ws + L.bar), (int32_t*)(ws + L.totals));
        } else {
            int chunk = PCG_PREP_CHUNK;
            if ((W + chunk - 1) / chunk > sms) chunk = (W + sms - 1) / sms;
            PCG_REQUIRE(chunk <= PCG_PREP_ITEMS, "pcg_choose: batch too large (%d items; at most %d)", W, PCG_PREP_ITEMS * sms);
            cfg.gridDim = dim3((unsigned)((W + chunk - 1) / chunk));
            attr[0].id = cudaLaunchAttributeCooperative;
            attr[0].val.cooperative = 1;
            e = cudaLaunchKernelEx(&cfg, k_choose_prep<false>, p, chunk, (int32_t*)(ws + L.bar), (int32_t*)(ws + L.totals));
        }
        if (e != cudaSuccess) { pcg_set_error("pcg_choose: prep launch: %s", cudaGetErrorString(e)); return (int)e; }
    }
    if ((phases & 2) == 0) return pcg_check_launch("pcg_choose");
    const bool have_cta = max_degree > PCG_SMALL_MAX, have_cl = max_degree > PCG_CTA_MAX,
               have_huge = max_degree > PCG_CL_MAX,
               have_big = max_degree > (p.huge16_ok ? PCG_HUGE16_MAX : PCG_HUGE_MAX);
    if (have_cl && !g_fork) {
        int prio_lo = 0, prio_hi = 0;
        cudaDeviceGetStreamPriorityRange(&prio_lo, &prio_hi);
        for (int q = 0; q < PCG_N_SIDE; ++q)
            if ((e = cudaStreamCreateWithPriority(&g_side[q], cudaStreamNonBlocking, prio_hi)) != cudaSuccess ||
                (e = cudaEventCreateWithFlags(&g_join[q], cudaEventDisableTiming)) != cudaSuccess) {
                pcg_set_error("pcg_choose: side stream: %s", cudaGetErrorString(e));
                return (int)e;
            }
        if ((e = cudaEventCreateWithFlags(&g_fork, cudaEventDisableTiming)) != cudaSuccess) {
            pcg_set_error("pcg_choose: event: %s", cudaGetErrorString(e));
            return (int)e;
        }
    }
    if (have_cl) cudaEventRecord(g_fork, stream);
    if (have_big) {
        int64_t cap = max_degree > 49152 ? 49152 : (max_degree + 31) / 32 * 32;
        size_t dyn = (size_t)cap * 4;
        if (dyn > S.big_smem) {
            e = cudaFuncSetAttribute(k_choose_big, cudaFuncAttributeMaxDynamicSharedMemorySize, (int)dyn);
            if (e != cudaSuccess) { pcg_set_error("pcg_choose: smem attr: %s", cudaGetErrorString(e)); return (int)e; }
            S.big_smem = dyn;
        }
        cudaStreamWaitEvent(g_side[2], g_fork, 0);
        k_choose_big<<<W < L.grid_big ? W : L.grid_big, PCG_LARGE_NT, dyn, g_side[2]>>>(p, (int)cap);
        cudaEventRecord(g_join[2], g_side[2]);
    }
    if (have_huge) {
        cudaStreamWaitEvent(g_side[0], g_fork, 0);
        if (max_degree > PCG_HUGE_MAX && p.huge16_ok) {
            e = launch_huge<16>(p, W < 4 ? W : 4, g_side[0], false, nullptr);
            if (e != cudaSuccess) { pcg_set_error("pcg_choose: huge16 launch: %s", cudaGetErrorString(e)); return (int)e; }
        }
        e = launch_huge<8>(p, W < 16 ? W : 16, g_side[0], false, nullptr);
        if (e != cudaSuccess) { pcg_set_error("pcg_choose: huge launch: %s", cudaGetErrorString(e)); return (int)e; }
        cudaEventRecord(g_join[0], g_side[0]);
    }
    if (have_cl) {
        cudaStreamWaitEvent(g_side[1], g_fork, 0);
        const int n_cl = W < 56 ? W : 56;
        k_choose_wide<<<n_cl * PCG_CL, PCG_GRP_NT, 0, g_side[1]>>>(p);
        cudaEventRecord(g_join[1], g_side[1]);
    }
    {
        const int units = W / PCG_WARPS_PER_CTA + 1 + (have_cta ? W : 0);
        const int gs = units < sms * 3 ? units : sms * 3;
        k_choose_small<<<gs, PCG_GRP_NT, 0, stream>>>(p);
    }
    if (have_huge) cudaStreamWaitEvent(stream, g_join[0], 0);
    if (have_cl) cudaStreamWaitEvent(stream, g_join[1], 0);
    if (have_big) cudaStreamWaitEvent(stream, g_join[2], 0);
    return pcg_check_launch("pcg_choose");
}

extern "C" int pcg_select_all(const int64_t* indptr, const int32_t* indices, int64_t n_nodes, int R,
                              const int32_t* targets, int B, int add_self, int64_t cap_slots, int32_t* slot_item,
                              int32_t* it_slot0, int32_t* it_m, int64_t* it_base, int32_t* it_extra, int32_t* it_done,
                              int32_t* status, pcg_stream_t stream_) {
    cudaStream_t stream = (cudaStream_t)stream_;
    PCG_REQUIRE(R >= 1 && B >= 0, "pcg_select_all: bad sizes");
    if (B == 0) {
        if (status) cudaMemsetAsync(status, 0, PCG_STATUS_WORDS * sizeof(int32_t), stream);
        return 0;
    }
    PCG_REQUIRE(indptr && indices && targets && slot_item && it_slot0 && it_m && it_base && it_extra && it_done && status,
                "pcg_select_all: null pointer");
    cudaError_t e = cudaMemsetAsync(status, 0, PCG_STATUS_WORDS * sizeof(int32_t), stream);
    if (e != cudaSuccess) { pcg_set_error("pcg_select_all: memset: %s", cudaGetErrorString(e)); return (int)e; }
    const int W = R * B;
    k_select_all<<<(W * 32 + 255) / 256, 256, 0, stream>>>(indptr, indices, n_nodes, R, targets, B, add_self, cap_slots,
                                                           slot_item, it_slot0, it_m, it_base, it_extra, it_done, status);
    return pcg_check_launch("pcg_select_all");
}
```

### pc-gnn_b200/csrc/pcg_common.cuh

```cuda
#pragma once
#include <cuda_runtime.h>
#include <stdint.h>
#include <stdio.h>

#include "pcgnn_b200.h"

#define PCG_FULL 0xffffffffu

#define ST_SLOTS PCG_ST_SLOTS
#define ST_NSMALL 1
#define ST_NMID 2
#define ST_OVERFLOW PCG_ST_OVERFLOW
#define ST_NCL 4
#define ST_SMALL_CTR 5
#define ST_MID_CTR 7
#define ST_NHUGE 8
#define ST_NHUGE16 9
#define ST_NBIG 6

#define PCG_MAX_DEVICES 64
static inline int pcg_current_device() {
    int dev = 0;
    if (cudaGetDevice(&dev) != cudaSuccess || dev < 0 || dev >= PCG_MAX_DEVICES) dev = 0;
    return dev;
}

void pcg_set_error(const char* fmt, ...);
int pcg_check_launch(const char* what);

int pcg_pdl_enabled();
__device__ __forceinline__ void pcg_grid_dependency_wait() { asm volatile("griddepcontrol.wait;" ::: "memory"); }
__device__ __forceinline__ void pcg_launch_dependents() { asm volatile("griddepcontrol.launch_dependents;" ::: "memory"); }

template <class... KArgs, class... Args>
static inline cudaError_t pcg_launch(void (*kernel)(KArgs...), dim3 grid, dim3 block, size_t smem, cudaStream_t stream,
                                     bool pdl, Args... args) {
    cudaLaunchConfig_t cfg = {};
    cfg.gridDim = grid;
    cfg.blockDim = block;
    cfg.dynamicSmemBytes = smem;
    cfg.stream = stream;
    cudaLaunchAttribute attr[1];
    attr[0].id = cudaLaunchAttributeProgrammaticStreamSerialization;
    attr[0].val.programmaticStreamSerializationAllowed = 1;
    cfg.attrs = attr;
    cfg.numAttrs = pdl ? 1 : 0;
    return cudaLaunchKernelEx(&cfg, kernel, KArgs(args)...);
}

#define PCG_REQUIRE(cond, ...)            \
    do {                                  \
        if (!(cond)) {                    \
            pcg_set_error(__VA_ARGS__);   \
            return (int)cudaErrorInvalidValue; \
        }                                 \
    } while (0)

__device__ __forceinline__ unsigned lanemask_lt() {
    unsigned m;
    asm("mov.u32 %0, %%lanemask_lt;" : "=r"(m));
    return m;
}

__device__ __forceinline__ uint32_t dist_bits(float a, float b) {
    return __float_as_uint(fabsf(__fsub_rn(a, b)));
}

__device__ __forceinline__ void item_counts(int64_t d, double thr, double rho, bool positive, int P, int c_override,
                                            bool has_override, int& k, int& o) {
    int64_t c = has_override ? (int64_t)c_override : (int64_t)ceil((double)d * thr);
    k = (int)((d > c + 1) ? c : d);
    if (k < 0) k = 0;
    int64_t oo = positive ? (int64_t)((double)c * rho) : 0;
    if (oo > P) oo = P;
    if (oo < 0) oo = 0;
    o = (int)oo;
}

__device__ __forceinline__ float4 ld_f4(const float* p) { return __ldg(reinterpret_cast<const float4*>(p)); }
__device__ __forceinline__ float4 ld_f4_cg(const float* p) { return __ldcg(reinterpret_cast<const float4*>(p)); }
__device__ __forceinline__ void f4_add(float4& a, const float4& b) {
    a.x += b.x; a.y += b.y; a.z += b.z; a.w += b.w;
}
```

### pc-gnn_b200/csrc/pcg_misc.cu

```cuda
#include <stdarg.h>

#include <cub/device/device_radix_sort.cuh>

#include "pcg_common.cuh"

static thread_local char g_err[512] = "";

void pcg_set_error(const char* fmt, ...) {
    va_list ap;
    va_start(ap, fmt);
    vsnprintf(g_err, sizeof(g_err), fmt, ap);
    va_end(ap);
}

int pcg_check_launch(const char* what) {
    cudaError_t e = cudaGetLastError();
    if (e != cudaSuccess) {
        pcg_set_error("%s: %s", what, cudaGetErrorString(e));
        return (int)e;
    }
    return 0;
}

extern "C" const char* pcg_last_error(void) { return g_err; }

static int g_pdl = 0;
int pcg_pdl_enabled() { return g_pdl; }
extern "C" int pcg_set_pdl(int enabled) {
    const int old = g_pdl;
    g_pdl = enabled;
    return old;
}
extern "C" int pcg_version(void) { return 100; }

__global__ void __launch_bounds__(256) k_score_table(const float* __restrict__ feat, int64_t n, int F, int64_t ldf,
                                                     const float* __restrict__ w, const float* __restrict__ b, float* __restrict__ score) {
    extern __shared__ float sw[];
    pcg_launch_dependents();
    for (int c = threadIdx.x; c < ldf; c += blockDim.x) sw[c] = c < F ? w[c] : 0.f;
    const float bias = b ? b[0] : 0.f;
    __syncthreads();
    const int l = threadIdx.x & 7;
    const int V = (int)(ldf >> 2);
    const int64_t rows_per_block = blockDim.x >> 3;
    for (int64_t vb = (int64_t)blockIdx.x * rows_per_block + ((threadIdx.x >> 5) << 2); vb < n;
         vb += (int64_t)gridDim.x * rows_per_block) {
        const int64_t v = vb + ((threadIdx.x & 31) >> 3);
        float acc = 0.f;
        if (v < n) {
            const float* rowp = feat + v * ldf;
            for (int c = l; c < V; c += 8) {
                float4 x = ld_f4(rowp + 4 * c);
                const float4 ww = *reinterpret_cast<const float4*>(sw + 4 * c);
                acc = fmaf(x.x, ww.x, acc); acc = fmaf(x.y, ww.y, acc);
                acc = fmaf(x.z, ww.z, acc); acc = fmaf(x.w, ww.w, acc);
            }
        }
        acc += __shfl_xor_sync(PCG_FULL, acc, 4);
        acc += __shfl_xor_sync(PCG_FULL, acc, 2);
        acc += __shfl_xor_sync(PCG_FULL, acc, 1);
        if (l == 0 && v < n) score[v] = acc + bias;
    }
}

__device__ __forceinline__ uint32_t ld_sys(const uint32_t* p) {
    uint32_t v;
    asm volatile("ld.volatile.global.u32 %0, [%1];" : "=r"(v) : "l"(p) : "memory");
    return v;
}
__device__ __forceinline__ void st_sys(uint32_t* p, uint32_t v) {
    asm volatile("st.volatile.global.u32 [%0], %1;" ::"l"(p), "r"(v) : "memory");
}
__device__ __forceinline__ void stage_copy(const uint32_t* src, uint32_t* dst, int64_t n, int64_t first, int64_t stride) {
    for (int64_t i = first; i < n; i += 4 * stride) {
        uint32_t v[4];
#pragma unroll
        for (int u = 0; u < 4; ++u) v[u] = i + u * stride < n ? ld_sys(src + i + u * stride) : 0u;
#pragma unroll
        for (int u = 0; u < 4; ++u)
            if (i + u * stride < n) st_sys(dst + i + u * stride, v[u]);
    }
}

__global__ void __launch_bounds__(256) k_stage(const uint32_t* src, uint32_t* dst, int64_t n, uint32_t* cursor,
                                               uint32_t count, int64_t src_stride, int64_t dst_stride, int bump) {
    uint32_t at = 0;
    if (cursor) {
        at = *(volatile uint32_t*)cursor;
        src += (int64_t)(at % count) * src_stride;
        dst += (int64_t)(at % count) * dst_stride;
    }
    stage_copy(src, dst, n, (int64_t)blockIdx.x * blockDim.x + threadIdx.x, (int64_t)gridDim.x * blockDim.x);
    if (cursor && bump) {
        __syncthreads();
        if (threadIdx.x == 0) *(volatile uint32_t*)cursor = at + 1u;
    }
}

__global__ void __launch_bounds__(256) k_pool_scores(const float* __restrict__ feat, int F, int64_t ldf,
                                                     const float* __restrict__ w, const float* __restrict__ b,
                                                     const int32_t* __restrict__ pool, int P, float* __restrict__ pool_score,
                                                     int score_blocks, const uint32_t* stage_src, uint32_t* stage_dst,
                                                     int64_t stage_words, const uint32_t* cursor, uint32_t count,
                                                     int64_t src_stride) {
    if ((int)blockIdx.x >= score_blocks) {
        const int64_t nb = gridDim.x - score_blocks;
        if (cursor) stage_src += (int64_t)(*(volatile const uint32_t*)cursor % count) * src_stride;
        stage_copy(stage_src, stage_dst, stage_words, (int64_t)(blockIdx.x - score_blocks) * blockDim.x + threadIdx.x,
                   nb * blockDim.x);
        return;
    }
    extern __shared__ float sw[];
    for (int c = threadIdx.x; c < ldf; c += blockDim.x) sw[c] = c < F ? w[c] : 0.f;
    const float bias = b ? b[0] : 0.f;
    __syncthreads();
    const int l = threadIdx.x & 7;
    const int V = (int)(ldf >> 2);
    const int rows_per_block = blockDim.x >> 3;
    for (int ib = blockIdx.x * rows_per_block + ((threadIdx.x >> 5) << 2); ib < P; ib += score_blocks * rows_per_block) {
        const int i = ib + ((threadIdx.x & 31) >> 3);
        float acc = 0.f;
        if (i < P) {
            const float* rowp = feat + (int64_t)__ldg(pool + i) * ldf;
            for (int c = l; c < V; c += 8) {
                float4 x = ld_f4(rowp + 4 * c);
                const float4 ww = *reinterpret_cast<const float4*>(sw + 4 * c);
                acc = fmaf(x.x, ww.x, acc); acc = fmaf(x.y, ww.y, acc);
                acc = fmaf(x.z, ww.z, acc); acc = fmaf(x.w, ww.w, acc);
            }
        }
        acc += __shfl_xor_sync(PCG_FULL, acc, 4);
        acc += __shfl_xor_sync(PCG_FULL, acc, 2);
        acc += __shfl_xor_sync(PCG_FULL, acc, 1);
        if (l == 0 && i < P) pool_score[i] = acc + bias;
    }
}

__global__ void k_gather_pool(const float* __restrict__ score, const int32_t* __restrict__ pool, int P,
                              float* __restrict__ pool_score) {
    const int p = blockIdx.x * blockDim.x + threadIdx.x;
    if (p < P) pool_score[p] = score[pool[p]];
}

__device__ __forceinline__ uint32_t orderable(float f) {
    const uint32_t u = __float_as_uint(f);
    return (u & 0x80000000u) ? ~u : (u | 0x80000000u);
}

__device__ __forceinline__ uint32_t unorderable(uint32_t k) {
    return (k & 0x80000000u) ? (k ^ 0x80000000u) : ~k;
}
#define RANK_NT 512
#define RANK_PER 32
__global__ void __launch_bounds__(RANK_NT) k_sort_pool_rank(const float* __restrict__ pool_score, int gather,
                                                            const int32_t* __restrict__ pool, int P,
                                                            float* __restrict__ ps_score, int32_t* __restrict__ ps_pos,
                                                            int32_t* __restrict__ ps_id) {
    extern __shared__ unsigned long long keys[];
    pcg_grid_dependency_wait();
    for (int base = 0; base < P; base += RANK_NT * 8) {
        int32_t id[8];
#pragma unroll
        for (int u = 0; u < 8; ++u) {
            const int i = base + u * RANK_NT + threadIdx.x;
            id[u] = (i < P && gather) ? __ldg(pool + i) : i;
        }
#pragma unroll
        for (int u = 0; u < 8; ++u) {
            const int i = base + u * RANK_NT + threadIdx.x;
            if (i < P) keys[i] = ((unsigned long long)orderable(__ldg(pool_score + id[u])) << 32) | (unsigned)i;
        }
    }
    __syncthreads();
    const int e = threadIdx.x >> 4, part = threadIdx.x & 15;
    const int i = blockIdx.x * RANK_PER + e;
    const unsigned long long mine = i < P ? keys[i] : ~0ull;
    int cnt = 0;
#pragma unroll 4
    for (int j = part; j < P; j += 16) cnt += keys[j] < mine;
    cnt += __shfl_xor_sync(PCG_FULL, cnt, 1);
    cnt += __shfl_xor_sync(PCG_FULL, cnt, 2);
    cnt += __shfl_xor_sync(PCG_FULL, cnt, 4);
    cnt += __shfl_xor_sync(PCG_FULL, cnt, 8);
    if (part == 0 && i < P) {
        ps_score[cnt] = __uint_as_float(unorderable((uint32_t)(mine >> 32)));
        ps_pos[cnt] = i;
        ps_id[cnt] = pool[i];
    }
}

__global__ void k_sort_prepare(const float* __restrict__ pool_score, int P, uint32_t* __restrict__ keys,
                               int32_t* __restrict__ vals) {
    const int i = blockIdx.x * blockDim.x + threadIdx.x;
    if (i < P) { keys[i] = orderable(pool_score[i]); vals[i] = i; }
}

__global__ void k_sort_finish(const float* __restrict__ pool_score, const int32_t* __restrict__ pool,
                              const int32_t* __restrict__ order, int P, float* __restrict__ ps_score,
                              int32_t* __restrict__ ps_pos, int32_t* __restrict__ ps_id) {
    const int i = blockIdx.x * blockDim.x + threadIdx.x;
    if (i < P) { const int pos = order[i]; ps_score[i] = pool_score[pos]; ps_pos[i] = pos; ps_id[i] = pool[pos]; }
}

#define PCG_SORT_SMALL_MAX 8192

static size_t align256(size_t x) { return (x + 255) & ~(size_t)255; }

static size_t cub_sort_temp_bytes(int P) {
    size_t temp = 0;
    cub::DeviceRadixSort::SortPairs(nullptr, temp, (const uint32_t*)nullptr, (uint32_t*)nullptr,
                                    (const int32_t*)nullptr, (int32_t*)nullptr, P);
    return temp;
}

extern "C" size_t pcg_sort_pool_workspace_bytes(int P) {
    size_t o = align256((size_t)(P > 0 ? P : 1) * 4);
    if (P > PCG_SORT_SMALL_MAX) o += 4 * align256((size_t)P * 4) + align256(cub_sort_temp_bytes(P));
    return o;
}

static int sort_pool_impl(const float* pool_score, int gather, const int32_t* pool, int P, float* ps_score, int32_t* ps_pos,
                          int32_t* ps_id, char* ws, size_t ws_bytes, cudaStream_t stream) {
    if (P <= 0) return 0;
    if (P <= PCG_SORT_SMALL_MAX) {
        const size_t smem = (size_t)P * 8;
        static bool configured_dev[PCG_MAX_DEVICES];
        bool& configured = configured_dev[pcg_current_device()];
        if (!configured) {
            cudaError_t e = cudaFuncSetAttribute(k_sort_pool_rank, cudaFuncAttributeMaxDynamicSharedMemorySize,
                                                 PCG_SORT_SMALL_MAX * 8);
            if (e != cudaSuccess) { pcg_set_error("pcg_sort_pool: smem attr: %s", cudaGetErrorString(e)); return (int)e; }
            configured = true;
        }
        cudaError_t le = pcg_launch(k_sort_pool_rank, dim3((P + RANK_PER - 1) / RANK_PER), dim3(RANK_NT), smem, stream,
                                    gather && (pcg_pdl_enabled() & 1), pool_score, gather, pool, P, ps_score, ps_pos, ps_id);
        if (le != cudaSuccess) { pcg_set_error("pcg_sort_pool: launch: %s", cudaGetErrorString(le)); return (int)le; }
        return 0;
    }
    const size_t a = align256((size_t)P * 4);
    size_t temp = cub_sort_temp_bytes(P);
    PCG_REQUIRE(ws && ws_bytes >= 4 * a + align256(temp), "pcg_sort_pool: workspace too small");
    uint32_t* k_in = (uint32_t*)ws;
    uint32_t* k_out = (uint32_t*)(ws + a);
    int32_t* v_in = (int32_t*)(ws + 2 * a);
    int32_t* v_out = (int32_t*)(ws + 3 * a);
    void* d_temp = ws + 4 * a;
    k_sort_prepare<<<(P + 255) / 256, 256, 0, stream>>>(pool_score, P, k_in, v_in);
    cudaError_t e = cub::DeviceRadixSort::SortPairs(d_temp, temp, k_in, k_out, v_in, v_out, P, 0, 32, stream);
    if (e != cudaSuccess) { pcg_set_error("pcg_sort_pool: cub: %s", cudaGetErrorString(e)); return (int)e; }
    k_sort_finish<<<(P + 255) / 256, 256, 0, stream>>>(pool_score, pool, v_out, P, ps_score, ps_pos, ps_id);
    return 0;
}

extern "C" int pcg_sort_pool(const float* pool_score, const int32_t* pool, int P, float* ps_score, int32_t* ps_pos,
                             int32_t* ps_id, void* workspace, size_t workspace_bytes, pcg_stream_t stream_) {
    cudaStream_t stream = (cudaStream_t)stream_;
    if (P <= 0) return 0;
    PCG_REQUIRE(pool_score && pool && ps_score && ps_pos && ps_id, "pcg_sort_pool: null pointer");
    size_t skip = align256((size_t)P * 4);
    char* ws = workspace ? (char*)workspace + skip : nullptr;
    int rc = sort_pool_impl(pool_score, 0, pool, P, ps_score, ps_pos, ps_id, ws,
                            workspace_bytes > skip ? workspace_bytes - skip : 0, stream);
    if (rc) return rc;
    return pcg_check_launch("pcg_sort_pool");
}

static int pool_scores_impl(const char* who, const float* feat, int F, int64_t ldf, const float* w, const float* b,
                            const int32_t* pool, int P, float* pool_score, const void* stage_src, void* stage_dst,
                            size_t stage_bytes, const uint32_t* cursor, uint32_t count, int64_t src_stride_bytes,
                            cudaStream_t stream) {
    PCG_REQUIRE(stage_bytes == 0 || (stage_src && stage_dst), "%s: staging pointers missing", who);
    PCG_REQUIRE(stage_bytes % 4 == 0 && ((uintptr_t)stage_src & 3) == 0 && ((uintptr_t)stage_dst & 3) == 0,
                "%s: the staged copy works on aligned 32-bit words", who);
    PCG_REQUIRE(!cursor || (count > 0 && src_stride_bytes % 4 == 0), "%s: a plan cursor needs count > 0 and a stride of whole words", who);
    if (P <= 0) {
        if (stage_bytes) {
            const int64_t n = (int64_t)(stage_bytes / 4);
            k_stage<<<(int)((n + 1023) / 1024 < 64 ? (n + 1023) / 1024 : 64), 256, 0, stream>>>(
                (const uint32_t*)stage_src, (uint32_t*)stage_dst, n, const_cast<uint32_t*>(cursor), count, src_stride_bytes / 4, 0, 0);
            return pcg_check_launch(who);
        }
        return 0;
    }
    PCG_REQUIRE(feat && w && pool && pool_score, "%s: null pointer", who);
    PCG_REQUIRE(ldf % 4 == 0 && F <= ldf && F > 0 && ldf * 4 <= 48 * 1024 && ((uintptr_t)feat & 15) == 0,
                "%s: need F <= ldf, ldf %% 4 == 0, 16-byte aligned rows (F=%d ldf=%lld)", who, F, (long long)ldf);
    int blocks = (P + 31) / 32;
    const int sms = pcg_device_sms();
    if (blocks > sms * 16) blocks = sms * 16;
    const int64_t words = (int64_t)(stage_bytes / 4);
    int64_t rider = (words + 1023) / 1024;
    if (rider > 64) rider = 64;
    k_pool_scores<<<blocks + (int)rider, 256, (size_t)ldf * 4, stream>>>(feat, F, ldf, w, b, pool, P, pool_score, blocks,
                                                                         (const uint32_t*)stage_src, (uint32_t*)stage_dst,
                                                                         words, cursor, count, src_stride_bytes / 4);
    return pcg_check_launch(who);
}

extern "C" int pcg_pool_scores(const float* feat, int F, int64_t ldf, const float* w, const float* b, const int32_t* pool,
                               int P, float* pool_score, pcg_stream_t stream_) {
    return pool_scores_impl("pcg_pool_scores", feat, F, ldf, w, b, pool, P, pool_score, nullptr, nullptr, 0, nullptr, 0, 0,
                            (cudaStream_t)stream_);
}

extern "C" int pcg_pool_scores_stage(const float* feat, int F, int64_t ldf, const float* w, const float* b,
                                     const int32_t* pool, int P, float* pool_score, const void* stage_src, void* stage_dst,
                                     size_t stage_bytes, const uint32_t* cursor, uint32_t count, int64_t src_stride_bytes,
                                     pcg_stream_t stream_) {
    return pool_scores_impl("pcg_pool_scores_stage", feat, F, ldf, w, b, pool, P, pool_score, stage_src, stage_dst,
                            stage_bytes, cursor, count, src_stride_bytes, (cudaStream_t)stream_);
}

extern "C" void* pcg_host_device_ptr(void* host_ptr) {
    void* dev = nullptr;
    cudaError_t e = cudaHostGetDevicePointer(&dev, host_ptr, 0);
    if (e != cudaSuccess) {
        (void)cudaGetLastError();
        pcg_set_error("pcg_host_device_ptr: %s (not page-locked / not mapped)", cudaGetErrorString(e));
        return nullptr;
    }
    return dev;
}

extern "C" int pcg_stage(const void* src, void* dst, size_t bytes, pcg_stream_t stream_) {
    cudaStream_t stream = (cudaStream_t)stream_;
    if (bytes == 0) return 0;
    PCG_REQUIRE(src && dst, "pcg_stage: null pointer");
    PCG_REQUIRE(bytes % 4 == 0 && ((uintptr_t)src & 3) == 0 && ((uintptr_t)dst & 3) == 0,
                "pcg_stage: the copy works on aligned 32-bit words");
    const int64_t n = (int64_t)(bytes / 4);
    int64_t blocks = (n + 1023) / 1024;
    if (blocks > 64) blocks = 64;
    k_stage<<<(int)blocks, 256, 0, stream>>>((const uint32_t*)src, (uint32_t*)dst, n, nullptr, 0, 0, 0, 0);
    return pcg_check_launch("pcg_stage");
}

extern "C" int pcg_stage_indexed(const void* src, void* dst, size_t bytes, uint32_t* cursor, uint32_t count,
                                 int64_t src_stride_bytes, int64_t dst_stride_bytes, int bump, pcg_stream_t stream_) {
    cudaStream_t stream = (cudaStream_t)stream_;
    if (bytes == 0) return 0;
    PCG_REQUIRE(src && dst && cursor && count > 0, "pcg_stage_indexed: null pointer or empty plan");
    PCG_REQUIRE(bytes % 4 == 0 && ((uintptr_t)src & 3) == 0 && ((uintptr_t)dst & 3) == 0 && src_stride_bytes % 4 == 0 &&
                    dst_stride_bytes % 4 == 0,
                "pcg_stage_indexed: the copy works on aligned 32-bit words");
    const int64_t n = (int64_t)(bytes / 4);
    int64_t blocks = (n + 1023) / 1024;
    if (blocks > 64) blocks = 64;
    PCG_REQUIRE(!bump || blocks == 1, "pcg_stage_indexed: a copy that advances the cursor is at most 4 KB (one CTA)");
    k_stage<<<(int)blocks, 256, 0, stream>>>((const uint32_t*)src, (uint32_t*)dst, n, cursor, count, src_stride_bytes / 4,
                                             dst_stride_bytes / 4, bump);
    return pcg_check_launch("pcg_stage_indexed");
}

extern "C" int pcg_score_table(const float* feat, int64_t n_nodes, int F, int64_t ldf, const float* w, const float* b,
                               float* score, const int32_t* pool, int P, float* ps_score, int32_t* ps_pos,
                               int32_t* ps_id, void* workspace, size_t workspace_bytes, pcg_stream_t stream_) {
    cudaStream_t stream = (cudaStream_t)stream_;
    PCG_REQUIRE(feat && w && score, "pcg_score_table: null pointer");
    PCG_REQUIRE(ldf % 4 == 0 && F <= ldf && F > 0, "pcg_score_table: need F <= ldf, ldf %% 4 == 0 (F=%d ldf=%lld)", F,
                (long long)ldf);
    PCG_REQUIRE(ldf * 4 <= 48 * 1024, "pcg_score_table: rows wider than 12288 floats unsupported");
    PCG_REQUIRE(((uintptr_t)feat & 15) == 0, "pcg_score_table: feat must be 16-byte aligned");
    if (n_nodes > 0) {
        int64_t blocks = (n_nodes + 31) / 32;
        const int sms = pcg_device_sms();
        if (blocks > (int64_t)sms * 16) blocks = (int64_t)sms * 16;
        k_score_table<<<(int)blocks, 256, (size_t)ldf * 4, stream>>>(feat, n_nodes, F, ldf, w, b, score);
    }
    if (P > 0 && pool) {
        PCG_REQUIRE(ps_score && ps_pos && ps_id, "pcg_score_table: sorted pool outputs missing");
        const size_t skip = align256((size_t)P * 4);
        PCG_REQUIRE(workspace && workspace_bytes >= skip, "pcg_score_table: workspace too small");
        int rc;
        if (P <= PCG_SORT_SMALL_MAX) {
            rc = sort_pool_impl(score, 1, pool, P, ps_score, ps_pos, ps_id, nullptr, 0, stream);
        } else {
            float* gathered = (float*)workspace;
            k_gather_pool<<<(P + 255) / 256, 256, 0, stream>>>(score, pool, P, gathered);
            rc = sort_pool_impl(gathered, 0, pool, P, ps_score, ps_pos, ps_id, (char*)workspace + skip,
                                workspace_bytes - skip, stream);
        }
        if (rc) return rc;
    }
    return pcg_check_launch("pcg_score_table");
}

__device__ __forceinline__ int64_t bisect_right_hi(const double* __restrict__ cum, int64_t n, double x) {
    int64_t lo = 0, hi = n - 1;
    while (lo < hi) {
        const int64_t mid = (lo + hi) >> 1;
        if (x < cum[mid]) hi = mid; else lo = mid + 1;
    }
    return lo;
}

__global__ void k_pick_replay(const double* __restrict__ cum, int64_t n, const double* __restrict__ u, int64_t k,
                              const int32_t* __restrict__ idx_train, int32_t* __restrict__ out) {
    const int64_t t = (int64_t)blockIdx.x * blockDim.x + threadIdx.x;
    if (t >= k) return;
    const double total = cum[n - 1] + 0.0;
    const int64_t pos = bisect_right_hi(cum, n, __dmul_rn(u[t], total));
    out[t] = idx_train ? idx_train[pos] : (int32_t)pos;
}

__device__ __forceinline__ void philox_round(uint32_t& c0, uint32_t& c1, uint32_t& c2, uint32_t& c3, uint32_t k0,
                                             uint32_t k1) {
    const uint32_t hi0 = __umulhi(0xD2511F53u, c0), lo0 = 0xD2511F53u * c0;
    const uint32_t hi1 = __umulhi(0xCD9E8D57u, c2), lo1 = 0xCD9E8D57u * c2;
    const uint32_t n0 = hi1 ^ c1 ^ k0, n1 = lo1, n2 = hi0 ^ c3 ^ k1, n3 = lo0;
    c0 = n0; c1 = n1; c2 = n2; c3 = n3;
}

__global__ void k_pick_philox(const double* __restrict__ cum, int64_t n, uint64_t seed, uint64_t offset, int64_t k,
                              const int32_t* __restrict__ idx_train, int32_t* __restrict__ out) {
    const int64_t t = (int64_t)blockIdx.x * blockDim.x + threadIdx.x;
    if (t >= k) return;
    const uint64_t ctr = offset + (uint64_t)t;
    uint32_t c0 = (uint32_t)ctr, c1 = (uint32_t)(ctr >> 32), c2 = 0, c3 = 0;
    uint32_t k0 = (uint32_t)seed, k1 = (uint32_t)(seed >> 32);
#pragma unroll
    for (int r = 0; r < 10; ++r) {
        philox_round(c0, c1, c2, c3, k0, k1);
        k0 += 0x9E3779B9u;
        k1 += 0xBB67AE85u;
    }
    const double u = ((double)(c0 >> 5) * 67108864.0 + (double)(c1 >> 6)) * (1.0 / 9007199254740992.0);
    const double total = cum[n - 1] + 0.0;
    const int64_t pos = bisect_right_hi(cum, n, __dmul_rn(u, total));
    out[t] = idx_train ? idx_train[pos] : (int32_t)pos;
}

extern "C" int pcg_pick_step(const double* cum, int64_t n, const double* u, int64_t k, const int32_t* idx_train,
                             int32_t* out, pcg_stream_t stream_) {
    cudaStream_t stream = (cudaStream_t)stream_;
    PCG_REQUIRE(cum && u && out && n > 0, "pcg_pick_step: null pointer or empty population");
    if (k > 0) k_pick_replay<<<(int)((k + 255) / 256), 256, 0, stream>>>(cum, n, u, k, idx_train, out);
    return pcg_check_launch("pcg_pick_step");
}

extern "C" int pcg_pick_step_philox(const double* cum, int64_t n, uint64_t seed, uint64_t offset, int64_t k,
                                    const int32_t* idx_train, int32_t* out, pcg_stream_t stream_) {
    cudaStream_t stream = (cudaStream_t)stream_;
    PCG_REQUIRE(cum && out && n > 0, "pcg_pick_step_philox: null pointer or empty population");
    if (k > 0) k_pick_philox<<<(int)((k + 255) / 256), 256, 0, stream>>>(cum, n, seed, offset, k, idx_train, out);
    return pcg_check_launch("pcg_pick_step_philox");
}
```

### pc-gnn_b200/engine.py

```python
from __future__ import annotations

import ctypes as C

import numpy as np
import torch

from . import _lib
from .graph import RelGraph

__all__ = ["Engine", "Selection", "PinnedStaging", "padded_ld"]


def padded_ld(feat_dim: int) -> int:
    return 32 if feat_dim <= 32 else (feat_dim + 3) // 4 * 4


class PinnedStaging:

    def __init__(self, n: int, dtype, depth: int = 3):
        self.n, self.dtype = int(n), dtype
        self.bufs = [torch.empty(self.n, dtype=dtype, pin_memory=True) for _ in range(depth)]
        self.events = [None] * depth
        self.i = 0

    def upload(self, host_array, dst: torch.Tensor):
        k = len(host_array)
        i = self.i
        self.i = (i + 1) % len(self.bufs)
        if self.events[i] is not None:
            self.events[i].synchronize()
        self.bufs[i].numpy()[:k] = host_array
        dst[:k].copy_(self.bufs[i][:k], non_blocking=True)
        ev = torch.cuda.Event()
        ev.record(torch.cuda.current_stream(dst.device))
        self.events[i] = ev
        return dst[:k]


class Selection:

    __slots__ = ("B", "R", "idx", "slot_item", "it_slot0", "it_m", "it_base", "it_extra", "it_done", "it_rep",
                 "status", "cap_slots", "norm", "_blob")

    def lists(self):
        m, base = self.item_sizes()
        idx = self.idx.cpu().numpy()
        extra = self.it_extra.cpu().numpy() if self.it_extra is not None else None
        out = []
        for w in range(self.B * self.R):
            ids = idx[base[w]:base[w] + m[w]]
            if extra is not None and extra[w] >= 0:
                ids = np.append(ids, extra[w])
            out.append(np.sort(ids))
        return out

    def item_sizes(self):
        m = self.it_m.cpu().numpy()
        base = self.it_base.cpu().numpy()
        if self.it_rep is not None:
            rep = self.it_rep.cpu().numpy()
            m, base = m[rep], base[rep]
        return m, base

    def overflowed(self) -> bool:
        return bool(self.status[_lib.ST_OVERFLOW].item())


class Engine:
    def __init__(self, graph: RelGraph | None, device=None):
        if not torch.cuda.is_available():
            raise _lib.PcgError("pcgnn_b200 needs a CUDA device (B200, sm_100a); there is no CPU fallback")
        self.lib = _lib.lib()
        self.device = torch.device(device if device is not None else f"cuda:{torch.cuda.current_device()}")
        if self.device.type != "cuda":
            raise _lib.PcgError(f"pcgnn_b200 runs on CUDA devices only (got {self.device})")
        if self.device.index is None:
            self.device = torch.device("cuda", torch.cuda.current_device())
        if self.device.index != torch.cuda.current_device():
            raise _lib.PcgError(f"engine for {self.device} but the current device is cuda:{torch.cuda.current_device()}: "
                                "call torch.cuda.set_device() first (one process per GPU)")
        self.graph = graph
        self.row_lo = 0
        if graph is not None:
            self.N, self.R = graph.n_nodes, graph.n_rel
            self.row_lo, self.N_global = graph.row_lo, graph.n_global
            if self.R > _lib.MAX_REL:
                raise ValueError(f"at most {_lib.MAX_REL} relations are supported")
            self.indptr, self.indices = graph.device(self.device)
            deg = np.diff(graph.indptr)
            self.max_degree = int(deg.max()) if deg.size else 0
        else:
            self.N = self.N_global = self.R = self.max_degree = 0
            self.indptr = self.indices = None
        self.strict_rows = True
        self._feat_key = None
        self._feat_src = None
        self.feat = None
        self.F = self.ldf = 0
        self.score = None
        self.pool = None
        self.sorted_pool = None
        self.pool_pos_of = None
        self.entry_pool_pos = None
        self.P = 0
        self._pin = None
        self._ws = None
        self._ws_nodes = None
        self.score_group = None
        self.grad_sink = None
        self.grads_in_sinks = False
        self._bcast = None

    def set_features(self, weight: torch.Tensor):
        key = (weight._version, tuple(weight.shape), weight.device)
        if self._feat_src is weight and key == self._feat_key:
            return self.feat
        self._feat_src = weight
        w = weight.detach()
        if self.graph is not None and self.strict_rows and w.shape[0] != self.N_global:
            raise ValueError(f"feature table has {w.shape[0]} rows, graph has {self.N_global} nodes")
        F_ = w.shape[1]
        ld = padded_ld(F_)
        if ld == F_ and w.is_contiguous() and w.dtype == torch.float32 and w.device == self.device \
                and w.data_ptr() % 16 == 0:
            feat = w
        else:
            feat = torch.zeros((w.shape[0], ld), dtype=torch.float32, device=self.device)
            feat[:, :F_] = w.to(self.device, torch.float32)
        self.feat, self.F, self.ldf = feat, F_, ld
        self._feat_key = key
        if self.score is None and self.graph is not None:
            self.score = torch.empty(self.N_global, dtype=torch.float32, device=self.device)
        return feat

    def set_pool(self, train_pos):
        if isinstance(train_pos, torch.Tensor):
            self.pool = train_pos.to(self.device, torch.int32).contiguous()
        else:
            self.pool = torch.from_numpy(np.asarray(list(train_pos), dtype=np.int32)).to(self.device)
        self.P = int(self.pool.shape[0])
        self.sorted_pool = self._alloc_sorted_pool(self.P)
        self.pool_pos_of = None
        self.entry_pool_pos = None
        if self.graph is not None:
            self.pool_pos_of = torch.empty(self.N_global, dtype=torch.int32, device=self.device)
            rc = self.lib.pcg_pool_positions(self.pool.data_ptr(), self.P, self.N_global, self.pool_pos_of.data_ptr(),
                                             _lib.stream_ptr())
            _lib.check(rc, "pcg_pool_positions")
            if self.P <= _lib.KB_MAX_POOL:
                self.entry_pool_pos = torch.empty(max(self.indices.shape[0], 1), dtype=torch.int32, device=self.device)
                rc = self.lib.pcg_entry_pool_positions(self.indices.data_ptr(), self.indices.shape[0],
                                                       self.pool_pos_of.data_ptr(), self.entry_pool_pos.data_ptr(),
                                                       _lib.stream_ptr())
                _lib.check(rc, "pcg_entry_pool_positions")

    def _alloc_sorted_pool(self, P):
        n = max(P, 1)
        dev = self.device
        ws = torch.empty(int(self.lib.pcg_sort_pool_workspace_bytes(P)), dtype=torch.uint8, device=dev)
        return (torch.empty(n, dtype=torch.float32, device=dev), torch.empty(n, dtype=torch.int32, device=dev),
                torch.empty(n, dtype=torch.int32, device=dev), ws)

    def sort_pool(self, pool, pool_score):
        P = int(pool.shape[0])
        ps, pp, pi, ws = self._alloc_sorted_pool(P)
        rc = self.lib.pcg_sort_pool(pool_score.data_ptr(), pool.data_ptr(), P, ps.data_ptr(), pp.data_ptr(),
                                    pi.data_ptr(), ws.data_ptr(), ws.numel(), _lib.stream_ptr())
        _lib.check(rc, "pcg_sort_pool")
        return ps, pp, pi

    def score_table(self, clf_weight: torch.Tensor, clf_bias: torch.Tensor):
        w = clf_weight.detach()
        b = clf_bias.detach()
        if not w.is_contiguous():
            w = w.contiguous()
        ps, pp, pi, ws = self.sorted_pool if self.pool is not None else (None, None, None, None)
        if self._bcast is not None:
            region, epoch = self._bcast
            lo = self.row_lo
            rc = self.lib.pcg_score_bcast(self.feat.data_ptr() + lo * self.ldf * 4, self.N, self.F, self.ldf,
                                          w.data_ptr(), b.data_ptr(), lo, self.N_global, region.regions, region.rank,
                                          region.world, epoch.data_ptr(), _lib.stream_ptr())
            _lib.check(rc, "pcg_score_bcast")
            self.resort_pool()
            return self.score
        if self.score_group is not None:
            self.score_local(w, b)
            self.score_exchange()
            self.resort_pool()
            return self.score
        rc = self.lib.pcg_score_table(self.feat.data_ptr(), self.N_global, self.F, self.ldf, w.data_ptr(), b.data_ptr(),
                                      self.score.data_ptr(), _lib.ptr(self.pool), self.P, _lib.ptr(ps), _lib.ptr(pp),
                                      _lib.ptr(pi), _lib.ptr(ws), 0 if ws is None else ws.numel(), _lib.stream_ptr())
        _lib.check(rc, "pcg_score_table")
        return self.score

    def stage(self, src_ptr: int, dst_ptr: int, nbytes: int, cursor_ptr: int = 0, count: int = 0, src_stride: int = 0):
        if cursor_ptr:
            _lib.check(self.lib.pcg_stage_indexed(src_ptr, dst_ptr, int(nbytes), cursor_ptr, int(count), int(src_stride), 0,
                                                  0, _lib.stream_ptr()), "pcg_stage_indexed")
        else:
            _lib.check(self.lib.pcg_stage(src_ptr, dst_ptr, int(nbytes), _lib.stream_ptr()), "pcg_stage")

    def pool_scores(self, clf_weight: torch.Tensor, clf_bias: torch.Tensor, stage=None):
        if not self.P:
            if stage is not None:
                self.stage(*stage)
            return None
        if getattr(self, "_pool_score", None) is None or self._pool_score.shape[0] != self.P:
            self._pool_score = torch.empty(self.P, dtype=torch.float32, device=self.device)
        w = clf_weight.detach()
        w = w if w.is_contiguous() else w.contiguous()
        if stage is not None:
            rc = self.lib.pcg_pool_scores_stage(self.feat.data_ptr(), self.F, self.ldf, w.data_ptr(),
                                                clf_bias.detach().data_ptr(), self.pool.data_ptr(), self.P,
                                                self._pool_score.data_ptr(), stage[0], stage[1], int(stage[2]),
                                                stage[3] if len(stage) > 3 else None, int(stage[4]) if len(stage) > 3 else 0,
                                                int(stage[5]) if len(stage) > 3 else 0, _lib.stream_ptr())
        else:
            rc = self.lib.pcg_pool_scores(self.feat.data_ptr(), self.F, self.ldf, w.data_ptr(),
                                          clf_bias.detach().data_ptr(), self.pool.data_ptr(), self.P,
                                          self._pool_score.data_ptr(), _lib.stream_ptr())
        _lib.check(rc, "pcg_pool_scores")
        return self._pool_score

    def sort_pool_from(self, pool_score: torch.Tensor):
        ps, pp, pi, ws = self.sorted_pool
        rc = self.lib.pcg_sort_pool(pool_score.data_ptr(), self.pool.data_ptr(), self.P, ps.data_ptr(), pp.data_ptr(),
                                    pi.data_ptr(), ws.data_ptr(), ws.numel(), _lib.stream_ptr())
        _lib.check(rc, "pcg_sort_pool")

    def score_table_only(self, clf_weight: torch.Tensor, clf_bias: torch.Tensor):
        w = clf_weight.detach()
        w = w if w.is_contiguous() else w.contiguous()
        b = clf_bias.detach()
        if self._bcast is not None:
            region, epoch = self._bcast
            lo = self.row_lo
            rc = self.lib.pcg_score_bcast(self.feat.data_ptr() + lo * self.ldf * 4, self.N, self.F, self.ldf,
                                          w.data_ptr(), b.data_ptr(), lo, self.N_global, region.regions, region.rank,
                                          region.world, epoch.data_ptr(), _lib.stream_ptr())
            _lib.check(rc, "pcg_score_bcast")
            return self.score
        if self.score_group is not None:
            self.score_local(w, b)
            self.score_exchange()
            return self.score
        rc = self.lib.pcg_score_table(self.feat.data_ptr(), self.N_global, self.F, self.ldf, w.data_ptr(), b.data_ptr(),
                                      self.score.data_ptr(), None, 0, None, None, None, None, 0, _lib.stream_ptr())
        _lib.check(rc, "pcg_score_table")
        return self.score

    def enable_score_broadcast(self, group=None):
        from .parallel import PeerRegion

        region = PeerRegion(int(self.lib.pcg_score_region_bytes(self.N_global)), group)
        if region.world == 1:
            return
        if region.world * self.N != self.N_global:
            raise ValueError("score broadcast needs equal row ranges (n_global == world * rows per rank)")

        class _Mem:
            def __init__(self, ptr, n):
                self.__cuda_array_interface__ = {"shape": (n,), "typestr": "<f4", "data": (ptr, False), "version": 2}

        self._score_mem = _Mem(region.own, self.N_global)
        self.score = torch.as_tensor(self._score_mem, device=self.device)
        self._bcast = (region, torch.zeros(1, dtype=torch.int32, device=self.device))
        self.score_group = None

    def score_local(self, w: torch.Tensor, b: torch.Tensor):
        lo = self.row_lo
        rc = self.lib.pcg_score_table(self.feat.data_ptr() + lo * self.ldf * 4, self.N, self.F, self.ldf,
                                      w.detach().data_ptr(), b.detach().data_ptr(), self.score.data_ptr() + lo * 4,
                                      None, 0, None, None, None, None, 0, _lib.stream_ptr())
        _lib.check(rc, "pcg_score_table")

    def score_exchange(self):
        import torch.distributed as dist

        world = dist.get_world_size(self.score_group)
        if world * self.N != self.N_global:
            raise ValueError("score exchange needs equal row ranges (n_global == world * rows per rank)")
        dist.all_gather_into_tensor(self.score, self.score[self.row_lo:self.row_lo + self.N], group=self.score_group)

    def resort_pool(self):
        if self.P:
            ps, pp, pi, ws = self.sorted_pool
            gathered = self.score[self.pool.long()].contiguous()
            rc = self.lib.pcg_sort_pool(gathered.data_ptr(), self.pool.data_ptr(), self.P, ps.data_ptr(), pp.data_ptr(),
                                        pi.data_ptr(), ws.data_ptr(), ws.numel(), _lib.stream_ptr())
            _lib.check(rc, "pcg_sort_pool")

    def upload_targets(self, nodes):
        if isinstance(nodes, torch.Tensor):
            if nodes.is_cuda:
                return nodes.to(torch.int32), None
            host = nodes.numpy().astype(np.int32, copy=False)
        else:
            host = np.asarray(nodes, dtype=np.int32)
        B = host.shape[0]
        if self._pin is None or self._pin.n < B:
            self._pin = PinnedStaging(max(B, 1024), torch.int32)
        dst = torch.empty(B, dtype=torch.int32, device=self.device)
        return self._pin.upload(host, dst), host

    def slots_bound(self, host_targets, thresh, rho, train) -> int:
        demand = self.graph.choose_slot_demand(thresh, rho, self.P, train)
        return max(int(demand[np.asarray(host_targets, dtype=np.int64) - self.row_lo].sum()), 1)

    def _new_selection(self, B, R, cap_slots, with_sel_idx, with_extra):
        W = B * R
        dev = self.device
        n64 = W
        n32 = (cap_slots * _lib.SLOT if with_sel_idx else 0) + cap_slots + 4 * W + (W if with_extra else 0) \
            + _lib.STATUS_WORDS
        blob = torch.empty(n64 * 2 + n32, dtype=torch.int32, device=dev)
        s = Selection()
        s._blob = blob
        s.B, s.R, s.cap_slots = B, R, cap_slots
        s.it_base = blob[:n64 * 2].view(torch.int64)
        o = n64 * 2

        def take(n):
            nonlocal o
            v = blob[o:o + n]
            o += n
            return v

        s.idx = take(cap_slots * _lib.SLOT) if with_sel_idx else self.indices
        s.slot_item = take(cap_slots)
        s.it_slot0 = take(W)
        s.it_m = take(W)
        s.it_done = take(W)
        s.it_extra = take(W) if with_extra else None
        s.it_rep = take(W) if with_sel_idx else None
        s.status = take(_lib.STATUS_WORDS)
        s.norm = _lib.NORM_MEAN
        return s

    def choose(self, targets, labels, train: bool, thresh, rho: float, cap_slots: int, *,
               entry_score=None, center_score=None, k_override=None, sorted_pool=None,
               indptr=None, indices=None, n_nodes=None, n_rel=None, max_degree=None,
               want_dist: bool = False, phases: int = 3, sel: Selection | None = None, workspace=None):
        B = int(targets.shape[0])
        R = self.R if n_rel is None else n_rel
        s = sel if sel is not None else self._new_selection(B, R, cap_slots, True, False)
        maxdeg = self.max_degree if max_degree is None else max_degree
        nn_ = self.N if n_nodes is None else n_nodes
        ws_bytes = self.lib.pcg_choose_workspace_bytes(B, R, maxdeg, nn_)
        if workspace is not None:
            if workspace.numel() < ws_bytes:
                raise _lib.PcgError(f"choose workspace has {workspace.numel()} bytes, this call needs {ws_bytes}")
            ws = workspace
        elif self._ws is None or self._ws.numel() < ws_bytes or self._ws_nodes != nn_:
            if self._ws is None or self._ws.numel() < ws_bytes:
                self._ws = torch.empty(int(ws_bytes), dtype=torch.uint8, device=self.device)
            _lib.check(self.lib.pcg_choose_workspace_init(self._ws.data_ptr(), self._ws.numel(), nn_, _lib.stream_ptr()),
                       "pcg_choose_workspace_init")
            self._ws_nodes = nn_
        if workspace is None:
            ws = self._ws
        th = (C.c_double * R)(*[float(x) for x in thresh])
        use_table = entry_score is None
        if sorted_pool is None and self.sorted_pool is not None and use_table:
            sorted_pool = self.sorted_pool[:3]
        ps, pp, pi = sorted_pool if sorted_pool is not None else (None, None, None)
        P = (self.P if use_table else int(ps.shape[0])) if ps is not None else 0
        dist = torch.empty(cap_slots * _lib.SLOT, dtype=torch.float32, device=self.device) if want_dist else None
        rc = self.lib.pcg_choose(
            (self.indptr if indptr is None else indptr).data_ptr(),
            (self.indices if indices is None else indices).data_ptr(),
            self.N if n_nodes is None else n_nodes, self.row_lo if n_nodes is None else 0, R,
            (self.score.data_ptr() if self.score is not None else None) if use_table else None, _lib.ptr(entry_score),
            _lib.ptr(center_score),
            targets.data_ptr(), _lib.ptr(labels) if train else None, B, th, _lib.ptr(k_override), float(rho),
            _lib.ptr(ps), _lib.ptr(pp), _lib.ptr(pi), _lib.ptr(self.entry_pool_pos) if use_table else None, P,
            int(bool(train)), maxdeg, s.idx.data_ptr(), _lib.ptr(dist),
            cap_slots, s.slot_item.data_ptr(), s.it_slot0.data_ptr(), s.it_m.data_ptr(), s.it_base.data_ptr(),
            s.it_done.data_ptr(), s.it_rep.data_ptr(), ws.data_ptr(), int(ws_bytes), s.status.data_ptr(),
            int(phases), _lib.stream_ptr())
        _lib.check(rc, "pcg_choose")
        return (s, dist) if want_dist else s

    def overflow_since_reset(self) -> bool:
        if self._ws is None:
            return False
        off = int(self.lib.pcg_choose_sticky_offset(self._ws_nodes))
        word = self._ws[off:off + 4].view(torch.int32)
        hit = bool(word.item())
        if hit:
            word.zero_()
        return hit

    def select_all(self, targets, add_self: bool, cap_slots: int, norm: int) -> Selection:
        if self.graph is not None and self.graph.partitioned:
            raise NotImplementedError("select-all runs on unpartitioned graphs only")
        B = int(targets.shape[0])
        s = self._new_selection(B, self.R, cap_slots, False, True)
        s.norm = norm
        rc = self.lib.pcg_select_all(self.indptr.data_ptr(), self.indices.data_ptr(), self.N, self.R,
                                     targets.data_ptr(), B, int(bool(add_self)), cap_slots, s.slot_item.data_ptr(),
                                     s.it_slot0.data_ptr(), s.it_m.data_ptr(), s.it_base.data_ptr(),
                                     s.it_extra.data_ptr(), s.it_done.data_ptr(), s.status.data_ptr(),
                                     _lib.stream_ptr())
        _lib.check(rc, "pcg_select_all")
        return s

    def aggregate(self, sel: Selection, feat=None, copy_dups: bool = True) -> torch.Tensor:
        feat = self.feat if feat is None else feat
        ldf = feat.shape[1]
        W = sel.B * sel.R
        agg = torch.empty((W, ldf), dtype=torch.float32, device=self.device)
        partial = torch.empty((sel.cap_slots, ldf), dtype=torch.float32, device=self.device)
        rc = self.lib.pcg_aggregate(feat.data_ptr(), ldf, sel.idx.data_ptr(), sel.slot_item.data_ptr(),
                                    sel.it_slot0.data_ptr(), sel.it_m.data_ptr(), sel.it_base.data_ptr(),
                                    _lib.ptr(sel.it_extra), _lib.ptr(sel.it_rep), int(copy_dups), W, sel.cap_slots,
                                    sel.status.data_ptr(), sel.norm, partial.data_ptr(), sel.it_done.data_ptr(),
                                    agg.data_ptr(), _lib.stream_ptr())
        _lib.check(rc, "pcg_aggregate")
        return agg

    def aggregate_bwd(self, sel: Selection, d_agg: torch.Tensor, feat_grad: torch.Tensor):
        ldf = feat_grad.shape[1]
        W = sel.B * sel.R
        d_agg = d_agg.contiguous()
        if sel.it_rep is not None:
            folded = torch.zeros_like(d_agg)
            folded.index_add_(0, sel.it_rep.long(), d_agg)
            d_agg = folded
        rc = self.lib.pcg_aggregate_bwd(d_agg.data_ptr(), ldf, sel.idx.data_ptr(), sel.slot_item.data_ptr(),
                                        sel.it_slot0.data_ptr(), sel.it_m.data_ptr(), sel.it_base.data_ptr(),
                                        _lib.ptr(sel.it_extra), W, sel.cap_slots, sel.status.data_ptr(), sel.norm,
                                        feat_grad.data_ptr(), _lib.stream_ptr())
        _lib.check(rc, "pcg_aggregate_bwd")
        return feat_grad

    def dense_fwd(self, targets, agg, w_intra, w_inter, feat_dim, agg_rep=None):
        B = int(targets.shape[0])
        R = len(w_intra)
        E = int(w_inter.shape[1])
        K2 = feat_dim + R * E
        cat = torch.empty((B, K2), dtype=torch.float32, device=self.device)
        out = torch.empty((E, B), dtype=torch.float32, device=self.device)
        ptrs = (C.c_void_p * R)(*[w.data_ptr() for w in w_intra])
        rc = self.lib.pcg_dense_fwd(self.feat.data_ptr(), self.ldf, feat_dim, targets.data_ptr(), B, R, E,
                                    agg.data_ptr(), _lib.ptr(agg_rep), ptrs, w_inter.data_ptr(), cat.data_ptr(), out.data_ptr(),
                                    _lib.stream_ptr())
        _lib.check(rc, "pcg_dense_fwd")
        return out, cat

    def tile_supported(self, B: int, R: int, E: int) -> bool:
        return B > 0 and bool(self.lib.pcg_tile_supported(int(B), int(R), int(self.F), int(E)))

    def tile_fwd(self, targets, agg, agg_rep, w_intra, w_inter, w_clf, b_clf, keep_cat: bool):
        B, R, E = int(targets.shape[0]), len(w_intra), int(w_inter.shape[1])
        dev = self.device
        out = torch.empty((E, B), dtype=torch.float32, device=dev)
        center = torch.empty((B, 2), dtype=torch.float32, device=dev) if w_clf is not None else None
        cat = torch.empty((B, self.F + R * E), dtype=torch.float32, device=dev) if keep_cat else None
        ptrs = (C.c_void_p * R)(*[w.data_ptr() for w in w_intra])
        rc = self.lib.pcg_tile_fwd(self.feat.data_ptr(), self.ldf, self.F, targets.data_ptr(), B, R, E, agg.data_ptr(),
                                   agg.shape[1], _lib.ptr(agg_rep), ptrs, w_inter.data_ptr(), _lib.ptr(w_clf),
                                   _lib.ptr(b_clf), int(bool(keep_cat)), out.data_ptr(), _lib.ptr(center),
                                   _lib.ptr(cat), _lib.stream_ptr())
        _lib.check(rc, "pcg_tile_fwd")
        return out, center, cat

    def tile_train(self, targets, labels, agg, agg_rep, w_intra, w_inter, w_clf, b_clf, w_head, lam, grads,
                   want_logits=False, pdl=False):
        B, R, E = int(targets.shape[0]), len(w_intra), int(w_inter.shape[1])
        dev = self.device
        buf = torch.empty(E * B + 2 * B + (2 * B if want_logits else 0) + 1, dtype=torch.float32, device=dev)
        out = buf[:E * B].view(E, B)
        center = buf[E * B:E * B + 2 * B].view(B, 2)
        logits = buf[E * B + 2 * B:E * B + 4 * B].view(B, 2) if want_logits else None
        loss = buf[-1:]
        scratch = torch.empty(int(self.lib.pcg_tile_scratch_floats(B, R, self.F, E)), dtype=torch.float32, device=dev)
        ptrs = (C.c_void_p * R)(*[w.data_ptr() for w in w_intra])
        gptrs = (C.c_void_p * R)(*[g.data_ptr() for g in grads["intra"]])
        rc = self.lib.pcg_tile_train(self.feat.data_ptr(), self.ldf, self.F, targets.data_ptr(), B, R, E, agg.data_ptr(),
                                     agg.shape[1], _lib.ptr(agg_rep), ptrs, w_inter.data_ptr(), w_clf.data_ptr(),
                                     b_clf.data_ptr(), w_head.data_ptr(), labels.data_ptr(), float(lam), out.data_ptr(),
                                     center.data_ptr(), _lib.ptr(logits), loss.data_ptr(), gptrs,
                                     grads["inter"].data_ptr(), grads["clf_w"].data_ptr(), grads["clf_b"].data_ptr(),
                                     grads["head"].data_ptr(), scratch.data_ptr(), int(bool(pdl)), _lib.stream_ptr())
        _lib.check(rc, "pcg_tile_train")
        return loss.view(()), out, center, logits

    def fork_point(self):
        if getattr(self, "_fork_word", None) is None:
            self._fork_word = torch.zeros(1, dtype=torch.int32, device=self.device)
        self._fork_word.zero_()

    def side_stream(self, which: int = 0):
        if getattr(self, "_sides", None) is None:
            self._sides = {}
        if which not in self._sides:
            self._sides[which] = torch.cuda.Stream(device=self.device, priority=-1)
        return self._sides[which]

    def sink_of(self, param):
        return None if self.grad_sink is None else self.grad_sink.get(param.data_ptr())

    def dense_bwd(self, agg, w_inter, cat, out, d_out, feat_dim, n_rel, agg_rep=None, sinks=None):
        B = int(cat.shape[0])
        E = int(w_inter.shape[1])
        K2 = feat_dim + n_rel * E
        n = int(self.lib.pcg_dense_bwd_scratch_floats(B, n_rel, feat_dim, E))
        scratch = torch.empty(n, dtype=torch.float32, device=self.device)
        if sinks is not None:
            d_inter, d_intra = sinks
        else:
            flat = torch.empty(K2 * E + n_rel * 2 * feat_dim * E, dtype=torch.float32, device=self.device)
            d_inter = flat[:K2 * E].view(K2, E)
            d_intra = [flat[K2 * E + r * 2 * feat_dim * E: K2 * E + (r + 1) * 2 * feat_dim * E].view(2 * feat_dim, E)
                       for r in range(n_rel)]
        ptrs = (C.c_void_p * n_rel)(*[g.data_ptr() for g in d_intra])
        d_out = d_out.contiguous()
        rc = self.lib.pcg_dense_bwd(agg.shape[1], feat_dim, B, n_rel, E, agg.data_ptr(), _lib.ptr(agg_rep), w_inter.data_ptr(),
                                    cat.data_ptr(), out.data_ptr(), d_out.data_ptr(), ptrs, d_inter.data_ptr(),
                                    scratch.data_ptr(), _lib.stream_ptr())
        _lib.check(rc, "pcg_dense_bwd")
        return d_intra, d_inter

    def encoder_fwd(self, agg, w, targets=None):
        B, E = int(agg.shape[0]), int(w.shape[0])
        out = torch.empty((E, B), dtype=torch.float32, device=self.device)
        rc = self.lib.pcg_encoder_fwd(agg.data_ptr(), agg.stride(0), self.feat.data_ptr() if targets is not None else None,
                                      self.ldf, _lib.ptr(targets), self.F, w.data_ptr(), B, E, out.data_ptr(),
                                      _lib.stream_ptr())
        _lib.check(rc, "pcg_encoder_fwd")
        return out

    def encoder_bwd(self, agg, out, d_out, targets=None, sink=None):
        B, E = int(agg.shape[0]), int(out.shape[0])
        f_in = self.F * (2 if targets is not None else 1)
        d_w = sink if sink is not None else torch.empty((E, f_in), dtype=torch.float32, device=self.device)
        scratch = torch.empty(int(self.lib.pcg_encoder_scratch_floats(B, f_in, E)), dtype=torch.float32, device=self.device)
        rc = self.lib.pcg_encoder_bwd(agg.data_ptr(), agg.stride(0), self.feat.data_ptr() if targets is not None else None,
                                      self.ldf, _lib.ptr(targets), self.F, B, E, out.data_ptr(), d_out.contiguous().data_ptr(),
                                      d_w.data_ptr(), scratch.data_ptr(), self._tickets()[3:].data_ptr(), _lib.stream_ptr())
        _lib.check(rc, "pcg_encoder_bwd")
        return d_w

    def _tickets(self):
        if getattr(self, "_ticket_buf", None) is None:
            self._ticket_buf = torch.zeros(8, dtype=torch.int32, device=self.device)
        return self._ticket_buf

    def center_fwd(self, targets, w, b):
        B = int(targets.shape[0])
        out = torch.empty((B, 2), dtype=torch.float32, device=self.device)
        rc = self.lib.pcg_center_fwd(self.feat.data_ptr(), self.ldf, self.F, targets.data_ptr(), B, w.data_ptr(),
                                     b.data_ptr(), out.data_ptr(), _lib.stream_ptr())
        _lib.check(rc, "pcg_center_fwd")
        return out

    def center_bwd(self, targets, d_center, sinks=None):
        B = int(targets.shape[0])
        if sinks is not None:
            d_w, d_b = sinks
        else:
            flat = torch.empty(2 * self.F + 2, dtype=torch.float32, device=self.device)
            d_w, d_b = flat[:2 * self.F].view(2, self.F), flat[2 * self.F:]
        scratch = torch.empty(int(self.lib.pcg_head_scratch_floats(B, self.F, 1)), dtype=torch.float32,
                              device=self.device)
        d_center = d_center.contiguous()
        rc = self.lib.pcg_center_bwd(self.feat.data_ptr(), self.ldf, self.F, targets.data_ptr(), B, d_center.data_ptr(),
                                     d_w.data_ptr(), d_b.data_ptr(), scratch.data_ptr(),
                                     self._tickets()[0:].data_ptr(), _lib.stream_ptr())
        _lib.check(rc, "pcg_center_bwd")
        return d_w, d_b

    def head_loss_fwd(self, emb, w, center, labels, lam):
        E, B = int(emb.shape[0]), int(emb.shape[1])
        buf = torch.empty(4 * B + 1, dtype=torch.float32, device=self.device)
        logits, p1, q1, loss = buf[:2 * B].view(B, 2), buf[2 * B:3 * B], buf[3 * B:4 * B], buf[4 * B:]
        scratch = torch.empty(int(self.lib.pcg_head_scratch_floats(B, 1, E)), dtype=torch.float32, device=self.device)
        rc = self.lib.pcg_head_loss_fwd(emb.data_ptr(), E, B, w.data_ptr(), center.data_ptr(), labels.data_ptr(),
                                        float(lam), logits.data_ptr(), p1.data_ptr(), q1.data_ptr(), loss.data_ptr(),
                                        scratch.data_ptr(), self._tickets()[1:].data_ptr(), _lib.stream_ptr())
        _lib.check(rc, "pcg_head_loss_fwd")
        return loss.view(()), logits, p1, q1

    def head_loss_bwd(self, emb, w, labels, p1, q1, lam, d_loss, sink=None):
        E, B = int(emb.shape[0]), int(emb.shape[1])
        d_emb = torch.empty((E, B), dtype=torch.float32, device=self.device)
        d_center = torch.empty((B, 2), dtype=torch.float32, device=self.device)
        d_w = sink if sink is not None else torch.empty((2, E), dtype=torch.float32, device=self.device)
        scratch = torch.empty(int(self.lib.pcg_head_scratch_floats(B, 1, E)), dtype=torch.float32, device=self.device)
        d_loss = d_loss.contiguous()
        rc = self.lib.pcg_head_loss_bwd(emb.data_ptr(), E, B, w.data_ptr(), labels.data_ptr(), p1.data_ptr(),
                                        q1.data_ptr(), float(lam), d_loss.data_ptr(), d_emb.data_ptr(),
                                        d_center.data_ptr(), d_w.data_ptr(), scratch.data_ptr(),
                                        self._tickets()[2:].data_ptr(), _lib.stream_ptr())
        _lib.check(rc, "pcg_head_loss_bwd")
        return d_emb, d_center, d_w
```

### pc-gnn_b200/layers.py

```python
from __future__ import annotations

from itertools import chain

import numpy as np
import torch
import torch.nn as nn
import torch.nn.functional as F
from torch.nn import init

from . import _lib
from .engine import Engine
from .graph import RelGraph, item_slots

__all__ = ["InterAgg1", "InterAgg3", "InterAgg5", "InterAgg", "IntraAgg", "choose_step_neighs",
           "choose_step_test", "HeadLossFn", "TrainStepFn"]


class _AggregateFn(torch.autograd.Function):

    @staticmethod
    def forward(ctx, table, engine, sel, feat_dim):
        feat = engine.set_features(table)
        ctx.engine, ctx.sel, ctx.feat_dim, ctx.shape = engine, sel, feat_dim, tuple(feat.shape)
        return engine.aggregate(sel, feat)

    @staticmethod
    def backward(ctx, d_agg):
        g = torch.zeros(ctx.shape, dtype=torch.float32, device=d_agg.device)
        ctx.engine.aggregate_bwd(ctx.sel, d_agg, g)
        return g[:, :ctx.feat_dim], None, None, None


class _DenseFn(torch.autograd.Function):

    @staticmethod
    def forward(ctx, engine, targets, agg, agg_rep, feat_dim, w_inter, *w_intra):
        w_intra = [w.contiguous() for w in w_intra]
        w_inter = w_inter.contiguous()
        out, cat = engine.dense_fwd(targets, agg, w_intra, w_inter, feat_dim, agg_rep)
        ctx.engine, ctx.feat_dim, ctx.n_rel, ctx.agg_rep = engine, feat_dim, len(w_intra), agg_rep
        ctx.w_ptrs = [w_inter.data_ptr()] + [w.data_ptr() for w in w_intra]
        ctx.save_for_backward(agg, w_inter, cat, out)
        return out

    @staticmethod
    def backward(ctx, d_out):
        agg, w_inter, cat, out = ctx.saved_tensors
        eng = ctx.engine
        sinks = None
        if eng.grad_sink is not None:
            views = [eng.grad_sink.get(q) for q in ctx.w_ptrs]
            if all(v is not None for v in views):
                sinks = (views[0], views[1:])
        d_intra, d_inter = eng.dense_bwd(agg, w_inter, cat, out, d_out, ctx.feat_dim, ctx.n_rel, ctx.agg_rep, sinks)
        if sinks is not None:
            return (None,) * (6 + ctx.n_rel)
        return (None, None, None, None, None, d_inter, *d_intra)


class _CenterFn(torch.autograd.Function):

    @staticmethod
    def forward(ctx, engine, targets, weight, bias):
        weight = weight.contiguous()
        ctx.engine, ctx.targets = engine, targets
        ctx.w_ptrs = (weight.data_ptr(), bias.data_ptr())
        return engine.center_fwd(targets, weight, bias)

    @staticmethod
    def backward(ctx, d_center):
        eng = ctx.engine
        sinks = None
        if eng.grad_sink is not None:
            views = (eng.grad_sink.get(ctx.w_ptrs[0]), eng.grad_sink.get(ctx.w_ptrs[1]))
            if views[0] is not None and views[1] is not None:
                sinks = views
        d_w, d_b = eng.center_bwd(ctx.targets, d_center, sinks)
        if sinks is not None:
            return None, None, None, None
        return None, None, d_w, d_b


class HeadLossFn(torch.autograd.Function):

    @staticmethod
    def forward(ctx, engine, combined, weight, center, labels, lam):
        combined, weight, center = combined.contiguous(), weight.contiguous(), center.contiguous()
        loss, logits, p1, q1 = engine.head_loss_fwd(combined, weight, center, labels, lam)
        ctx.engine, ctx.lam = engine, lam
        ctx.w_ptr = weight.data_ptr()
        ctx.save_for_backward(combined, weight, labels, p1, q1)
        ctx.mark_non_differentiable(logits)
        return loss, logits

    @staticmethod
    def backward(ctx, d_loss, _d_logits):
        combined, weight, labels, p1, q1 = ctx.saved_tensors
        eng = ctx.engine
        sink = eng.grad_sink.get(ctx.w_ptr) if eng.grad_sink is not None else None
        d_emb, d_center, d_w = eng.head_loss_bwd(combined, weight, labels, p1, q1, ctx.lam, d_loss, sink)
        return None, d_emb, (None if sink is not None else d_w), d_center, None, None


class _TileFn(torch.autograd.Function):

    @staticmethod
    def forward(ctx, engine, targets, agg, agg_rep, feat_dim, need_grad, clf_w, clf_b, w_inter, *w_intra):
        w_intra = [w.contiguous() for w in w_intra]
        w_inter, clf_w = w_inter.contiguous(), clf_w.contiguous()
        out, center, cat = engine.tile_fwd(targets, agg, agg_rep, w_intra, w_inter, clf_w, clf_b, need_grad)
        ctx.engine, ctx.feat_dim, ctx.n_rel, ctx.agg_rep, ctx.targets = engine, feat_dim, len(w_intra), agg_rep, targets
        ctx.w_ptrs = [w_inter.data_ptr()] + [w.data_ptr() for w in w_intra]
        ctx.clf_ptrs = (clf_w.data_ptr(), clf_b.data_ptr())
        if need_grad:
            ctx.save_for_backward(agg, w_inter, cat, out)
        return out, center

    @staticmethod
    def backward(ctx, d_out, d_center):
        agg, w_inter, cat, out = ctx.saved_tensors
        eng = ctx.engine
        n_in = 9 + ctx.n_rel
        grads = [None] * n_in
        if d_center is not None:
            sinks = None
            if eng.grad_sink is not None:
                views = (eng.grad_sink.get(ctx.clf_ptrs[0]), eng.grad_sink.get(ctx.clf_ptrs[1]))
                sinks = views if views[0] is not None and views[1] is not None else None
            d_w, d_b = eng.center_bwd(ctx.targets, d_center, sinks)
            if sinks is None:
                grads[6], grads[7] = d_w, d_b
        if d_out is not None:
            sinks = None
            if eng.grad_sink is not None:
                views = [eng.grad_sink.get(q) for q in ctx.w_ptrs]
                sinks = (views[0], views[1:]) if all(v is not None for v in views) else None
            d_intra, d_inter = eng.dense_bwd(agg, w_inter, cat, out, d_out, ctx.feat_dim, ctx.n_rel, ctx.agg_rep, sinks)
            if sinks is None:
                grads[8] = d_inter
                grads[9:] = list(d_intra)
        return tuple(grads)


class TrainStepFn(torch.autograd.Function):

    @staticmethod
    def forward(ctx, engine, targets, labels, agg, agg_rep, lam, pdl, w_head, clf_w, clf_b, w_inter, *w_intra):
        params = [w_head, clf_w, clf_b, w_inter, *w_intra]
        cont = [w.contiguous() for w in params]
        sink = engine.grad_sink
        views = [sink.get(w.data_ptr()) for w in params] if sink is not None else None
        if views is not None and all(v is not None for v in views):
            g = views
            ctx.flat = None
            engine.grads_in_sinks = True
        else:
            sizes = [w.numel() for w in params]
            pad = [(n + 3) // 4 * 4 for n in sizes]
            flat = torch.empty(sum(pad), dtype=torch.float32, device=engine.device)
            g, o = [], 0
            for w, n, q in zip(params, sizes, pad):
                g.append(flat[o:o + n].view_as(w))
                o += q
            ctx.flat, ctx.views = flat, g
        grads = dict(head=g[0], clf_w=g[1], clf_b=g[2], inter=g[3], intra=g[4:])
        loss, out, center, _ = engine.tile_train(targets, labels, agg, agg_rep, cont[4:], cont[3], cont[1], cont[2],
                                                 cont[0], lam, grads, pdl=pdl)
        ctx.n_in = 7 + len(params)
        ctx.mark_non_differentiable(out, center)
        return loss, out, center

    @staticmethod
    def backward(ctx, d_loss, _d_out, _d_center):
        if ctx.flat is None:
            return (None,) * ctx.n_in
        ctx.flat.mul_(d_loss)
        return (None,) * 7 + tuple(ctx.views)


def _feature_table(features, n_nodes, device, ids=None):
    if isinstance(features, nn.Embedding):
        return features.weight
    w = getattr(features, "weight", None)
    if isinstance(w, torch.Tensor) and w.dim() == 2 and (n_nodes is None or w.shape[0] >= n_nodes):
        return w
    if n_nodes is None:
        lists, nodes, pool = ids
        n_nodes = 1 + max(max((int(x) for x in chain.from_iterable(lists)), default=0),
                          max((int(v) for v in nodes), default=0), max((int(p) for p in pool), default=0))
    return features(torch.arange(n_nodes, device=device))


def _as_device_labels(labels, device):
    if labels is None:
        return None
    if not isinstance(labels, torch.Tensor):
        labels = torch.as_tensor(np.asarray(labels))
    return labels.to(device=device, dtype=torch.int64).reshape(-1).contiguous()


class IntraAgg(nn.Module):

    def __init__(self, features, feat_dim, embed_dim, train_pos, rho, cuda=False):
        super().__init__()
        self.features = features
        self.cuda = cuda
        self.feat_dim = feat_dim
        self.embed_dim = embed_dim
        self.train_pos = train_pos
        self.rho = rho
        self.weight = nn.Parameter(torch.FloatTensor(2 * self.feat_dim, self.embed_dim))
        init.xavier_uniform_(self.weight)
        self._engine = None

    def transform(self, self_feats, agg_feats):
        return F.relu(torch.cat((self_feats, agg_feats), dim=1).mm(self.weight))

    def forward(self, nodes, batch_labels, to_neighs_list, batch_scores, neigh_scores, pos_scores, sample_list,
                train_flag):
        dev = self.weight.device
        if self._engine is None or self._engine.device != dev:
            self._engine = Engine(None, dev)
        eng = self._engine
        sel, dist, meta = _choose_explicit(eng, batch_scores, batch_labels if train_flag else None, neigh_scores,
                                           to_neighs_list, pos_scores if train_flag else None,
                                           self.train_pos if train_flag else None, sample_list, self.rho, train_flag)
        table = _feature_table(self.features, None, dev, ids=(to_neighs_list, nodes, self.train_pos))
        agg = _AggregateFn.apply(table, eng, sel, self.feat_dim)
        idx = torch.as_tensor(np.asarray([int(v) for v in nodes]), device=dev, dtype=torch.long)
        to_feats = self.transform(self.features(idx), agg[:, :self.feat_dim])
        lab = _as_device_labels(batch_labels, dev) if train_flag else None
        return to_feats, _LazyScores(sel, dist, meta, lab, train_flag)


class _LazyScores:

    def __init__(self, sel, dist, meta, labels, train):
        self._args = (sel, dist, meta, labels, train)
        self._val = None

    def _get(self):
        if self._val is None:
            sel, dist, meta, labels, train = self._args
            lab = labels.cpu().numpy() if labels is not None else None
            self._val = _sets_and_scores(sel, dist, meta, lab, train)[1]
            self._args = None
        return self._val

    def __iter__(self):
        return iter(self._get())

    def __len__(self):
        return len(self._get())

    def __getitem__(self, i):
        return self._get()[i]


def _explicit_csr(neighs_list, neigh_scores, device):
    lens = np.fromiter((len(x) for x in neighs_list), dtype=np.int64, count=len(neighs_list))
    indptr = np.zeros(len(lens) + 1, dtype=np.int64)
    np.cumsum(lens, out=indptr[1:])
    ids = np.fromiter((int(x) for x in chain.from_iterable(neighs_list)), dtype=np.int64, count=int(indptr[-1]))
    rows = np.repeat(np.arange(len(lens), dtype=np.int64), lens)
    order = np.lexsort((ids, rows))
    flat = torch.cat([torch.as_tensor(s).reshape(-1, 2)[:, 0] for s in neigh_scores]).detach()
    entry_score = flat.to(device=device, dtype=torch.float32)[torch.from_numpy(order).to(device)].contiguous()
    return (torch.from_numpy(indptr).to(device), torch.from_numpy(ids[order].astype(np.int32)).to(device),
            entry_score, lens)


def _choose_explicit(eng, center_scores, center_labels, neigh_scores, neighs_list, minor_scores, minor_list,
                     sample_list, sample_rate, train):
    dev = eng.device
    B = len(neighs_list)
    indptr, indices, entry_score, lens = _explicit_csr(neighs_list, neigh_scores, dev)
    center = torch.as_tensor(center_scores).detach().to(dev, torch.float32).reshape(-1, 2)[:, 0].contiguous()
    k_list = np.asarray([int(k) for k in sample_list], dtype=np.int64)
    k_over = torch.from_numpy(k_list.astype(np.int32)).to(dev)
    sorted_pool = None
    P = 0
    if train and minor_list is not None and len(minor_list):
        pool = torch.as_tensor(np.asarray([int(p) for p in minor_list], dtype=np.int32)).to(dev)
        pool_score = torch.as_tensor(minor_scores).detach().to(dev, torch.float32).reshape(-1, 2)[:, 0].contiguous()
        P = int(pool.shape[0])
        sorted_pool = eng.sort_pool(pool, pool_score)
    oo = np.minimum((k_list * float(sample_rate)).astype(np.int64), P) if train else np.zeros_like(k_list)
    cap = int(item_slots(lens, k_list, sample_rate, P, train).sum()) + 1
    targets = torch.arange(B, dtype=torch.int32, device=dev)
    labels = _as_device_labels(center_labels, dev) if train else None
    sel, dist = eng.choose(targets, labels, train, [0.5], float(sample_rate), cap, entry_score=entry_score,
                           center_score=center, k_override=k_over, sorted_pool=sorted_pool,
                           indptr=indptr, indices=indices, n_nodes=B, n_rel=1,
                           max_degree=int(lens.max()) if B else 0, want_dist=True)
    return sel, dist, (lens, k_list, oo)


def _sets_and_scores(sel, dist, meta, labels_host, train):
    lens, k_list, oo = meta
    base = sel.it_base.cpu().numpy()
    m = sel.it_m.cpu().numpy()
    idx = sel.idx.cpu().numpy()
    dist = dist.cpu().numpy()
    sets, scores = [], []
    for i in range(sel.B):
        d, c = int(lens[i]), int(k_list[i])
        k = c if d > c + 1 else d
        sets.append(set(idx[base[i]:base[i] + m[i]].tolist()))
        seg = dist[base[i]:base[i] + k]
        row = np.sort(seg, kind="stable").tolist() if d > c + 1 else seg.tolist()
        if train and labels_host is not None and labels_host[i] == 1:
            o = int(oo[i])
            row = row + np.sort(dist[base[i] + k:base[i] + k + o], kind="stable").tolist()
        scores.append(row)
    return sets, scores


def choose_step_neighs(center_scores, center_labels, neigh_scores, neighs_list, minor_scores, minor_list, sample_list,
                       sample_rate):
    dev = torch.device("cuda", torch.cuda.current_device())
    eng = Engine(None, dev)
    sel, dist, meta = _choose_explicit(eng, center_scores, center_labels, neigh_scores, neighs_list, minor_scores,
                                       minor_list, sample_list, sample_rate, True)
    lab = _as_device_labels(center_labels, dev).cpu().numpy()
    return _sets_and_scores(sel, dist, meta, lab, True)


def choose_step_test(center_scores, neigh_scores, neighs_list, sample_list):
    dev = torch.device("cuda", torch.cuda.current_device())
    eng = Engine(None, dev)
    sel, dist, meta = _choose_explicit(eng, center_scores, None, neigh_scores, neighs_list, None, None, sample_list,
                                       0.0, False)
    return _sets_and_scores(sel, dist, meta, None, False)


class InterAgg(nn.Module):

    n_relations = None

    def __init__(self, features, feature_dim, embed_dim, train_pos, adj_lists, intraggs, inter='GNN', cuda=True):
        super().__init__()
        R = len(intraggs)
        if self.n_relations is not None and R != self.n_relations:
            raise ValueError(f"{type(self).__name__} takes {self.n_relations} intra-aggregators, got {R}")
        self.features = features
        self.dropout = 0.6
        self.adj_lists = adj_lists
        for r, ia in enumerate(intraggs):
            setattr(self, f"intra_agg{r + 1}", ia)
            ia.cuda = cuda
        self.embed_dim = embed_dim
        self.feat_dim = feature_dim
        self.cuda = cuda
        self.train_pos = train_pos
        self.thresholds = [0.5] * R
        self.weight = nn.Parameter(torch.FloatTensor(self.embed_dim * R + self.feat_dim, self.embed_dim))
        init.xavier_uniform_(self.weight)
        self.label_clf = nn.Linear(self.feat_dim, 2)
        self.weights_log = []
        self.thresholds_log = [self.thresholds]
        self.relation_score_log = []
        self._R = R
        self._graph = adj_lists if isinstance(adj_lists, RelGraph) else None
        self._engine = None
        self.cap_slots_hint = None
        self.score_override = None
        self.center_on_side_stream = False
        self.scores_external = False
        self.last_selection = None
        self.use_pdl = False
        self.graph_cache = True
        self.stage_in = None
        self._graphs = None
        self._fused_memo = {}

    def intra_aggs(self):
        return [getattr(self, f"intra_agg{r + 1}") for r in range(self._R)]

    def engine(self) -> Engine:
        dev = self.weight.device
        if self._engine is None or self._engine.device != dev:
            if self._graph is None:
                self._graph = RelGraph.from_adj_lists(self.adj_lists)
            if self._graph.n_rel != self._R:
                raise ValueError(f"{self._R} intra-aggregators but {self._graph.n_rel} relations")
            self._engine = Engine(self._graph, dev)
            self._engine.set_pool(self.train_pos)
        return self._engine

    def _select(self, eng, targets, lab, train_flag, cap, *, workspace=None):
        rho = self.intra_agg1.rho
        dev = eng.device
        cur = torch.cuda.current_stream(dev)
        side = eng.side_stream(0)
        own_scores = self.score_override is None and not self.scores_external
        stage, self.stage_in = self.stage_in, None

        if own_scores and eng.P and train_flag:
            pool_score = eng.pool_scores(self.label_clf.weight, self.label_clf.bias, stage=stage)
            side1 = eng.side_stream(1)
            side.wait_stream(cur)
            side1.wait_stream(cur)
            with torch.cuda.stream(side):
                sel = eng.choose(targets, lab, train_flag, self.thresholds, rho, cap, phases=1, workspace=workspace)
            with torch.cuda.stream(side1):
                eng.sort_pool_from(pool_score)
            eng.score_table_only(self.label_clf.weight, self.label_clf.bias)
            cur.wait_stream(side)
            cur.wait_stream(side1)
        else:
            if stage is not None:
                eng.stage(*stage)
            else:
                eng.fork_point()
            side.wait_stream(cur)
            with torch.cuda.stream(side):
                sel = eng.choose(targets, lab, train_flag, self.thresholds, rho, cap, phases=1, workspace=workspace)
            if self.score_override is not None:
                eng.score.copy_(self.score_override)
                eng.resort_pool()
            elif self.scores_external:
                eng.resort_pool()
            elif train_flag:
                eng.score_table(self.label_clf.weight, self.label_clf.bias)
            else:
                eng.score_table_only(self.label_clf.weight, self.label_clf.bias)
            cur.wait_stream(side)
        eng.choose(targets, lab, train_flag, self.thresholds, rho, cap, phases=2, sel=sel, workspace=workspace)
        self.last_selection = sel
        return sel

    def _choose_and_aggregate(self, nodes, labels, train_flag):
        eng = self.engine()
        dev = eng.device
        table = _feature_table(self.features, eng.N_global, dev)
        eng.set_features(table)
        targets, host = eng.upload_targets(nodes)
        rho = self.intra_agg1.rho
        lab = _as_device_labels(labels, dev) if train_flag else None
        if self.cap_slots_hint is not None:
            cap = int(self.cap_slots_hint)
        else:
            cap = eng.slots_bound(targets.cpu().numpy() if host is None else host, self.thresholds, rho, train_flag)
        return eng, table, targets, lab, self._select(eng, targets, lab, train_flag, cap)

    def graphs(self):
        if self._graphs is None:
            from .stepgraph import StepGraphCache

            self._graphs = StepGraphCache(self)
        return self._graphs

    def _frozen_fast_path(self, table, B) -> bool:
        return (not table.requires_grad) and self.embed_dim <= 256 and B > 0 \
            and isinstance(self.label_clf, nn.Linear) and self.label_clf.bias is not None

    def _fused_ok(self, eng, table, B) -> bool:
        if not self._frozen_fast_path(table, B):
            return False
        eng.set_features(table)
        key = (B, eng.F, self.embed_dim)
        ok = self._fused_memo.get(key)
        if ok is None:
            ok = self._fused_memo[key] = eng.tile_supported(B, self._R, self.embed_dim)
        return ok

    def train_loss(self, nodes, labels, head_weight, lam):
        eng = self.engine()
        table = _feature_table(self.features, eng.N_global, eng.device)
        B = len(nodes) if not isinstance(nodes, torch.Tensor) else int(nodes.shape[0])
        if not self._fused_ok(eng, table, B):
            return None
        if self.graphs().usable(eng, table, B):
            loss = self.graphs().train_loss(eng, nodes, labels, head_weight, float(lam))
            if loss is not None:
                return loss
        eng, table, targets, lab, sel = self._choose_and_aggregate(nodes, labels, True)
        agg = eng.aggregate(sel, copy_dups=False)
        loss, _, _ = TrainStepFn.apply(eng, targets, lab, agg, sel.it_rep, float(lam), bool(self.use_pdl), head_weight,
                                       self.label_clf.weight, self.label_clf.bias, self.weight,
                                       *[ia.weight for ia in self.intra_aggs()])
        return loss

    def forward(self, nodes, labels, train_flag=True):
        if not torch.is_grad_enabled() or not any(p.requires_grad for p in self.parameters()):
            eng = self.engine()
            table = _feature_table(self.features, eng.N_global, eng.device)
            B = len(nodes) if not isinstance(nodes, torch.Tensor) else int(nodes.shape[0])
            if self._fused_ok(eng, table, B) and self.graphs().usable(eng, table, B):
                res = self.graphs().infer(eng, nodes, labels, train_flag)
                if res is not None:
                    return res
        eng, table, targets, lab, sel = self._choose_and_aggregate(nodes, labels, train_flag)
        dev = eng.device
        B = targets.shape[0]
        fused = self._frozen_fast_path(table, B)
        if fused and eng.tile_supported(B, self._R, self.embed_dim):
            agg = eng.aggregate(sel, copy_dups=False)
            ws = [self.label_clf.weight, self.label_clf.bias, self.weight] + [ia.weight for ia in self.intra_aggs()]
            need_grad = torch.is_grad_enabled() and any(w.requires_grad for w in ws)
            return _TileFn.apply(eng, targets, agg, sel.it_rep, self.feat_dim, need_grad, *ws)
        side = None
        if fused:
            if self.center_on_side_stream:
                cur = torch.cuda.current_stream(dev)
                side = eng.side_stream()
                side.wait_stream(cur)
                with torch.cuda.stream(side):
                    center_scores = _CenterFn.apply(eng, targets, self.label_clf.weight, self.label_clf.bias)
            else:
                center_scores = _CenterFn.apply(eng, targets, self.label_clf.weight, self.label_clf.bias)
        else:
            idx = targets.long()
            self_feats = self.features(idx)
            center_scores = self.label_clf(self_feats)
        if fused:
            agg = eng.aggregate(sel, copy_dups=False)
            combined = _DenseFn.apply(eng, targets, agg, sel.it_rep, self.feat_dim, self.weight,
                                      *[ia.weight for ia in self.intra_aggs()])
            if side is not None:
                torch.cuda.current_stream(dev).wait_stream(side)
            return combined, center_scores
        agg = _AggregateFn.apply(table, eng, sel, self.feat_dim)
        agg = agg.view(self._R, B, -1)[:, :, :self.feat_dim]

        r_feats = [ia.transform(self_feats, agg[r]) for r, ia in enumerate(self.intra_aggs())]
        cat_feats = torch.cat([self_feats] + r_feats, dim=1)
        combined = F.relu(cat_feats.mm(self.weight).t())
        return combined, center_scores


class InterAgg1(InterAgg):
    n_relations = 1


class InterAgg3(InterAgg):
    n_relations = 3


class InterAgg5(InterAgg):
    n_relations = 5
```

Measured before the change: 11.47 million.

## Fuse staging, score table, pool sort and choose prep into one clustered kernel

Adds a pcg_front kernel that gives different thread-block clusters different roles. One cluster stages inputs and runs choose-prep, several clusters score the pool and rank-sort it through distributed shared memory, and the rest compute the full score table. The training select path now uses this single launch instead of separate pool-score, sort, score-table and prep launches spread over side streams. The aim is to remove launch and cross-stream synchronisation overhead. In exchange it is limited to pools up to 8192 and a bounded item count, and prep now runs on a single cluster.

```diff
diff --git a/include/pcgnn_b200.h b/include/pcgnn_b200.h
--- a/include/pcgnn_b200.h
+++ b/include/pcgnn_b200.h
@@ -62,6 +62,15 @@
                int32_t* sel_idx, float* sel_dist, int64_t cap_slots, int32_t* slot_item, int32_t* it_slot0,
                int32_t* it_m, int64_t* it_base, int32_t* it_done, int32_t* it_rep, void* workspace,
                size_t workspace_bytes, int32_t* status, int phases, pcg_stream_t stream);
+
+PCG_API int pcg_front(const float* feat, int64_t n_table, int F, int64_t ldf, const float* w, const float* b, float* score,
+              const int32_t* pool, int P, float* ps_score, int32_t* ps_pos, int32_t* ps_id, const void* stage_src,
+              void* stage_dst, size_t stage_bytes, const uint32_t* cursor, uint32_t count, int64_t src_stride_bytes,
+              const int64_t* indptr, const int32_t* indices, int64_t n_nodes, int64_t row_lo, int R,
+              const int32_t* targets, const int64_t* labels, int B, const double* thresh_host, double rho,
+              const int32_t* entry_pool_pos, int64_t max_degree, int64_t cap_slots, int32_t* slot_item,
+              int32_t* it_slot0, int32_t* it_m, int64_t* it_base, int32_t* it_done, int32_t* it_rep, void* workspace,
+              size_t workspace_bytes, int32_t* status, pcg_stream_t stream);
 
 PCG_API int pcg_select_all(const int64_t* indptr, const int32_t* indices, int64_t n_nodes, int R, const int32_t* targets,
                    int B, int add_self, int64_t cap_slots, int32_t* slot_item, int32_t* it_slot0, int32_t* it_m,
diff --git a/pc-gnn_b200/_lib.py b/pc-gnn_b200/_lib.py
--- a/pc-gnn_b200/_lib.py
+++ b/pc-gnn_b200/_lib.py
@@ -13,6 +13,8 @@
 ST_SLOTS, ST_OVERFLOW = 0, 3
 NORM_MEAN, NORM_RSQRT = 0, 1
 KB_MAX_POOL = 8192
+FRONT_MAX_POOL = 8192
+FRONT_MAX_ITEMS = 65536
 METRICS_KEYS = ("auc", "f1", "f1_macro", "recall", "precision", "recall_macro", "precision_macro", "accuracy", "gmean",
                 "best_f1_macro", "best_threshold", "n_pos", "n_neg", "tp", "fp", "tn", "fn")
 METRICS_WORDS = len(METRICS_KEYS)
@@ -44,6 +46,8 @@
     "pcg_entry_pool_positions": (_i, [_p, _l, _p, _p, _p]),
     "pcg_choose": (_i, [_p, _p, _l, _l, _i, _p, _p, _p, _p, _p, _i, C.POINTER(_d), _p, _d, _p, _p, _p, _p, _i, _i, _l,
                         _p, _p, _l, _p, _p, _p, _p, _p, _p, _p, _z, _p, _i, _p]),
+    "pcg_front": (_i, [_p, _l, _i, _l, _p, _p, _p, _p, _i, _p, _p, _p, _p, _p, _z, _p, C.c_uint32, _l, _p, _p, _l, _l, _i,
+                       _p, _p, _i, C.POINTER(_d), _d, _p, _l, _l, _p, _p, _p, _p, _p, _p, _p, _z, _p, _p]),
     "pcg_select_all": (_i, [_p, _p, _l, _i, _p, _i, _i, _l, _p, _p, _p, _p, _p, _p, _p, _p]),
     "pcg_aggregate": (_i, [_p, _l, _p, _p, _p, _p, _p, _p, _p, _i, _i, _l, _p, _i, _p, _p, _p, _p]),
     "pcg_aggregate_bwd": (_i, [_p, _l, _p, _p, _p, _p, _p, _p, _i, _l, _p, _i, _p, _p]),
diff --git a/pc-gnn_b200/csrc/pcg_choose.cu b/pc-gnn_b200/csrc/pcg_choose.cu
--- a/pc-gnn_b200/csrc/pcg_choose.cu
+++ b/pc-gnn_b200/csrc/pcg_choose.cu
@@ -1,5 +1,6 @@
 #include "pcg_common.cuh"
 
+#include <algorithm>
 #include <cooperative_groups.h>
 namespace cg = cooperative_groups;
 
@@ -1051,28 +1052,28 @@
 }
 
 template <bool CLUSTER>
-__global__ void __launch_bounds__(PCG_PREP_NT, 1) k_choose_prep(ChooseP p, int chunk, int32_t* bar, int32_t* totals) {
-    __shared__ int s_info[PCG_PREP_ITEMS];
+__device__ __forceinline__ void choose_prep(const ChooseP& p, int chunk, int32_t* bar, int32_t* totals, int* s_info,
+                                            int cta, int G) {
     __shared__ int s_wsum[32];
     __shared__ int s_base;
     constexpr int NT = PCG_PREP_NT;
     const int tid = threadIdx.x, lane = tid & 31, wid = tid >> 5;
-    const int B = p.B, W = p.R * p.B, G = gridDim.x;
+    const int B = p.B, W = p.R * p.B;
     int32_t* first = p.first;
     PTRACE(0);
     if (first)
-        for (int i = blockIdx.x * NT + tid; i < B; i += G * NT) {
-            const int64_t lv = (int64_t)__ldg(p.targets + i) - p.row_lo;
+        for (int i = cta * NT + tid; i < B; i += G * NT) {
+            const int64_t lv = (int64_t)__ldcg(p.targets + i) - p.row_lo;
             if (lv >= 0 && lv < p.n_nodes) atomicMin(&first[lv], i);
         }
-    if (blockIdx.x == 0 && tid < PCG_STATUS_WORDS) p.status[tid] = 0;
+    if (cta == 0 && tid < PCG_STATUS_WORDS) p.status[tid] = 0;
     auto barrier = [&](int target) {
         if (CLUSTER) { __threadfence(); cg::this_cluster().sync(); }
         else prep_grid_barrier(bar, target);
     };
     barrier(G);
     PTRACE(1);
-    const int w0 = min(W, blockIdx.x * chunk), n_items = min(W, w0 + chunk) - w0;
+    const int w0 = min(W, cta * chunk), n_items = min(W, w0 + chunk) - w0;
     for (int q0 = tid; q0 < n_items; q0 += 4 * NT) {
         int rr[4], ii[4], rep[4];
         int64_t beg[4], end[4];
@@ -1087,13 +1088,13 @@
             beg[u] = end[u] = 0;
             pos[u] = false;
             if (q < n_items) {
-                const int64_t lv = (int64_t)__ldg(p.targets + ii[u]) - p.row_lo;
+                const int64_t lv = (int64_t)__ldcg(p.targets + ii[u]) - p.row_lo;
                 if (lv >= 0 && lv < p.n_nodes) {
                     rep[u] = first ? __ldcg(first + lv) : ii[u];
                     const int64_t row = (int64_t)rr[u] * p.n_nodes + lv;
                     beg[u] = __ldg(p.indptr + row);
                     end[u] = __ldg(p.indptr + row + 1);
-                    pos[u] = p.train && p.labels && __ldg(p.labels + ii[u]) == 1;
+                    pos[u] = p.train && p.labels && __ldcg(p.labels + ii[u]) == 1;
                 } else {
                     rep[u] = -2;
                 }
@@ -1146,11 +1147,11 @@
         if (lane >= off) wincl += t;
     }
     const int cta_total = __shfl_sync(PCG_FULL, wincl, 31);
-    if (tid == 0) totals[blockIdx.x] = cta_total;
+    if (tid == 0) totals[cta] = cta_total;
     barrier(2 * G);
     if (wid == 0) {
         int acc = 0;
-        for (int c = lane; c < (int)blockIdx.x; c += 32) acc += __ldcg(totals + c);
+        for (int c = lane; c < cta; c += 32) acc += __ldcg(totals + c);
         acc = __reduce_add_sync(PCG_FULL, acc);
         if (lane == 0) s_base = acc;
     }
@@ -1195,18 +1196,162 @@
     PTRACE(3);
     if (__syncthreads_or(overflow) && tid == 0) { atomicExch(&p.status[ST_OVERFLOW], 1); atomicOr(p.sticky, 1); }
     if (first)
-        for (int i = blockIdx.x * NT + tid; i < B; i += G * NT) {
-            const int64_t lv = (int64_t)__ldg(p.targets + i) - p.row_lo;
+        for (int i = cta * NT + tid; i < B; i += G * NT) {
+            const int64_t lv = (int64_t)__ldcg(p.targets + i) - p.row_lo;
             if (lv >= 0 && lv < p.n_nodes) first[lv] = 0x7f7f7f7f;
         }
     if (tid == 0) {
-        if (blockIdx.x == G - 1) p.status[ST_SLOTS] = s_base + cta_total;
+        if (cta == G - 1) p.status[ST_SLOTS] = s_base + cta_total;
         if (!CLUSTER) {
             __threadfence();
             if (atomicAdd(&bar[1], 1) == G - 1) { bar[0] = 0; bar[1] = 0; }
         }
     }
     PTRACE(4);
+}
+
+template <bool CLUSTER>
+__global__ void __launch_bounds__(PCG_PREP_NT, 1) k_choose_prep(ChooseP p, int chunk, int32_t* bar, int32_t* totals) {
+    __shared__ int s_info[PCG_PREP_ITEMS];
+    choose_prep<CLUSTER>(p, chunk, bar, totals, s_info, blockIdx.x, gridDim.x);
+}
+
+#define FRONT_ROWS 4
+#define FRONT_POOL_MAX 8192
+#define FRONT_POOL_CL 4
+
+struct FrontP {
+    const float* feat;
+    int64_t n_table, ldf;
+    int F;
+    const float* w;
+    const float* b;
+    float* score;
+    const int32_t* pool;
+    float* ps_score;
+    int32_t* ps_pos;
+    int32_t* ps_id;
+    const uint32_t* stage_src;
+    uint32_t* stage_dst;
+    int64_t stage_words;
+    const uint32_t* cursor;
+    uint32_t count;
+    int64_t src_stride;
+    int n_pool_cl;
+};
+
+#ifdef PCG_TRACE
+#define FTRACE(slot) do { if (g_trace && threadIdx.x == 0) atomicMax((unsigned long long*)&g_trace[(int64_t)p.R * p.B * PCG_TRACE_SLOTS + (slot)], (unsigned long long)trace_now()); } while (0)
+#else
+#define FTRACE(slot) do {} while (0)
+#endif
+
+template <int ROWS, class RowOf, class Store>
+__device__ __forceinline__ void score_rows(const float* __restrict__ feat, int64_t ldf, const float* sw, float bias,
+                                           int64_t lo, int64_t hi, int64_t warp0, int64_t nwarps, RowOf row_of,
+                                           Store store) {
+    const int lane = threadIdx.x & 31, l = lane & 7, sub = lane >> 3;
+    const int V = (int)(ldf >> 2);
+    for (int64_t vb = lo + warp0 * 4 * ROWS; vb < hi; vb += nwarps * 4 * ROWS) {
+        const float* rowp[ROWS];
+        float acc[ROWS];
+#pragma unroll
+        for (int u = 0; u < ROWS; ++u) {
+            const int64_t v = vb + 4 * u + sub;
+            rowp[u] = v < hi ? feat + row_of(v) * ldf : nullptr;
+            acc[u] = 0.f;
+        }
+#pragma unroll 1
+        for (int c = l; c < V; c += 8) {
+            float4 x[ROWS];
+#pragma unroll
+            for (int u = 0; u < ROWS; ++u) x[u] = rowp[u] ? ld_f4(rowp[u] + 4 * c) : make_float4(0.f, 0.f, 0.f, 0.f);
+            const float4 ww = *reinterpret_cast<const float4*>(sw + 4 * c);
+#pragma unroll
+            for (int u = 0; u < ROWS; ++u) {
+                acc[u] = fmaf(x[u].x, ww.x, acc[u]); acc[u] = fmaf(x[u].y, ww.y, acc[u]);
+                acc[u] = fmaf(x[u].z, ww.z, acc[u]); acc[u] = fmaf(x[u].w, ww.w, acc[u]);
+            }
+        }
+#pragma unroll
+        for (int u = 0; u < ROWS; ++u) {
+            float a = acc[u];
+            a += __shfl_xor_sync(PCG_FULL, a, 4);
+            a += __shfl_xor_sync(PCG_FULL, a, 2);
+            a += __shfl_xor_sync(PCG_FULL, a, 1);
+            if (l == 0 && rowp[u]) store(vb + 4 * u + sub, a + bias);
+        }
+    }
+}
+
+__global__ void __launch_bounds__(PCG_PREP_NT, 1)
+    k_front(ChooseP p, FrontP f, int chunk, int32_t* bar, int32_t* totals) {
+    extern __shared__ __align__(16) unsigned char front_smem[];
+    constexpr int NT = PCG_PREP_NT;
+    cg::cluster_group cl = cg::this_cluster();
+    const int cid = blockIdx.x / PCG_CL, rank = (int)cl.block_rank(), tid = threadIdx.x;
+    if (cid == 0) {
+        if (f.stage_words) {
+            const uint32_t* src = f.stage_src;
+            if (f.cursor) src += (int64_t)(*(volatile const uint32_t*)f.cursor % f.count) * f.src_stride;
+            stage_copy(src, f.stage_dst, f.stage_words, (int64_t)rank * NT + tid, (int64_t)PCG_CL * NT);
+            __threadfence();
+            cl.sync();
+        }
+        choose_prep<true>(p, chunk, bar, totals, reinterpret_cast<int*>(front_smem), rank, PCG_CL);
+        FTRACE(5);
+        return;
+    }
+    float* sw = reinterpret_cast<float*>(front_smem);
+    for (int c = tid; c < f.ldf; c += NT) sw[c] = c < f.F ? f.w[c] : 0.f;
+    const float bias = f.b ? f.b[0] : 0.f;
+    __syncthreads();
+    if (cid > f.n_pool_cl) {
+        const int64_t t = blockIdx.x - (int64_t)PCG_CL * (1 + f.n_pool_cl), T = gridDim.x - (int64_t)PCG_CL * (1 + f.n_pool_cl);
+        float* score = f.score;
+        score_rows<FRONT_ROWS>(f.feat, f.ldf, sw, bias, 0, f.n_table, t * (NT / 32) + (tid >> 5), T * (NT / 32),
+                               [](int64_t v) { return v; }, [&](int64_t v, float s) { score[v] = s; });
+        FTRACE(7);
+        return;
+    }
+    const int P = p.P;
+    unsigned long long* keys = reinterpret_cast<unsigned long long*>(front_smem + f.ldf * 4);
+    const int share = (P + PCG_CL - 1) / PCG_CL;
+    {
+        const int lo = min(P, rank * share), hi = min(P, lo + share);
+        const int32_t* pool = f.pool;
+        score_rows<FRONT_ROWS>(f.feat, f.ldf, sw, bias, lo, hi, tid >> 5, NT / 32,
+                               [&](int64_t i) { return (int64_t)__ldg(pool + i); },
+                               [&](int64_t i, float s) { keys[i] = ((unsigned long long)orderable(s) << 32) | (unsigned)i; });
+    }
+    cl.sync();
+    for (int q = 1; q < PCG_CL; ++q) {
+        const int r = (rank + q) & (PCG_CL - 1);
+        const unsigned long long* rk = cl.map_shared_rank(keys, r);
+        const int lo = min(P, r * share), hi = min(P, lo + share);
+        for (int i = lo + tid; i < hi; i += NT) keys[i] = rk[i];
+    }
+    cl.sync();
+    const int g = (cid - 1) * PCG_CL + rank, per = (P + PCG_CL * f.n_pool_cl - 1) / (PCG_CL * f.n_pool_cl);
+    const int e0 = min(P, g * per), e1 = min(P, e0 + per);
+    const int e = tid >> 4, part = tid & 15;
+    for (int i0 = e0; i0 < e1; i0 += NT / 16) {
+        const int i = i0 + e;
+        const unsigned long long mine = i < e1 ? keys[i] : ~0ull;
+        int cnt = 0;
+#pragma unroll 4
+        for (int j = part; j < P; j += 16) cnt += keys[j] < mine;
+        cnt += __shfl_xor_sync(PCG_FULL, cnt, 1);
+        cnt += __shfl_xor_sync(PCG_FULL, cnt, 2);
+        cnt += __shfl_xor_sync(PCG_FULL, cnt, 4);
+        cnt += __shfl_xor_sync(PCG_FULL, cnt, 8);
+        if (part == 0 && i < e1) {
+            f.ps_score[cnt] = __uint_as_float(unorderable((uint32_t)(mine >> 32)));
+            f.ps_pos[cnt] = i;
+            f.ps_id[cnt] = __ldg(f.pool + i);
+        }
+    }
+    FTRACE(6);
 }
 
 __global__ void k_select_all(const int64_t* __restrict__ indptr, const int32_t* __restrict__ indices, int64_t n_nodes,
@@ -1349,35 +1494,14 @@
 };
 static SideState g_dev[PCG_MAX_DEVICES];
 
-extern "C" int pcg_choose(const int64_t* indptr, const int32_t* indices, int64_t n_nodes, int64_t row_lo, int R,
-                          const float* score,
-                          const float* entry_score, const float* center_score, const int32_t* targets,
-                          const int64_t* labels, int B, const double* thresh_host, const int32_t* k_override,
-                          double rho, const float* ps_score, const int32_t* ps_pos, const int32_t* ps_id,
-                          const int32_t* entry_pool_pos, int P, int train,
-                          int64_t max_degree, int32_t* sel_idx, float* sel_dist, int64_t cap_slots,
-                          int32_t* slot_item, int32_t* it_slot0, int32_t* it_m, int64_t* it_base, int32_t* it_done,
-                          int32_t* it_rep, void* workspace, size_t workspace_bytes, int32_t* status, int phases,
-                          pcg_stream_t stream_) {
-    cudaStream_t stream = (cudaStream_t)stream_;
-    PCG_REQUIRE(R >= 1 && R <= PCG_MAX_REL, "pcg_choose: R=%d outside [1,%d]", R, PCG_MAX_REL);
-    PCG_REQUIRE(phases >= 1 && phases <= 3, "pcg_choose: phases must be 1 (prepare), 2 (select) or 3 (both)");
-    PCG_REQUIRE(B >= 0, "pcg_choose: negative batch");
-    if (B == 0) {
-        if (status) cudaMemsetAsync(status, 0, PCG_STATUS_WORDS * sizeof(int32_t), stream);
-        return 0;
-    }
-    PCG_REQUIRE((phases & 2) == 0 || score || (entry_score && center_score), "pcg_choose: need a score table or explicit scores");
-    PCG_REQUIRE(!(train && P > 0) || (ps_score && ps_pos && ps_id), "pcg_choose: sorted pool arrays missing");
-    PCG_REQUIRE(indptr && indices && targets && sel_idx && slot_item && it_slot0 && it_m && it_base && it_done &&
-                    it_rep && status,
-                "pcg_choose: null pointer");
-    const int sms = device_sms();
-    WsLayout L = ws_layout(B, R, max_degree, n_nodes, sms);
-    PCG_REQUIRE(workspace && workspace_bytes >= L.total, "pcg_choose: workspace too small (%zu < %zu)", workspace_bytes,
-                L.total);
-    cudaError_t e;
-    ChooseP p;
+static void choose_params(ChooseP& p, const WsLayout& L, const int64_t* indptr, const int32_t* indices, int64_t n_nodes,
+                          int64_t row_lo, int R, const float* score, const float* entry_score, const float* center_score,
+                          const int32_t* targets, const int64_t* labels, int B, const double* thresh_host,
+                          const int32_t* k_override, double rho, const float* ps_score, const int32_t* ps_pos,
+                          const int32_t* ps_id, const int32_t* entry_pool_pos, int P, int train, int32_t* sel_idx,
+                          float* sel_dist, int64_t cap_slots, int32_t* slot_item, int32_t* it_slot0, int32_t* it_m,
+                          int64_t* it_base, int32_t* it_done, int32_t* it_rep, void* workspace, int32_t* status,
+                          cudaStream_t stream) {
     p.indptr = indptr; p.indices = indices; p.score = score; p.entry_score = entry_score;
     p.center_score = center_score; p.targets = targets; p.labels = labels; p.k_override = k_override;
     p.ps_score = ps_score; p.ps_pos = ps_pos; p.ps_id = ps_id; p.entry_pool_pos = entry_pool_pos;
@@ -1397,18 +1521,54 @@
     p.sticky = (int32_t*)(ws + L.bar) + 2;
     p.bits_slab = (uint32_t*)(ws + L.bits_slab);
     p.slab_words = L.slab_words;
+    SideState& S = g_dev[pcg_current_device()];
+    if (S.huge16_state == 0) {
+        int mc = 0;
+        cudaError_t pe = launch_huge<16>(p, 1, stream, true, &mc);
+        S.huge16_state = (pe == cudaSuccess && mc >= 1) ? 1 : 2;
+        (void)cudaGetLastError();
+    }
+    p.huge16_ok = S.huge16_state == 1;
+}
+
+extern "C" int pcg_choose(const int64_t* indptr, const int32_t* indices, int64_t n_nodes, int64_t row_lo, int R,
+                          const float* score,
+                          const float* entry_score, const float* center_score, const int32_t* targets,
+                          const int64_t* labels, int B, const double* thresh_host, const int32_t* k_override,
+                          double rho, const float* ps_score, const int32_t* ps_pos, const int32_t* ps_id,
+                          const int32_t* entry_pool_pos, int P, int train,
+                          int64_t max_degree, int32_t* sel_idx, float* sel_dist, int64_t cap_slots,
+                          int32_t* slot_item, int32_t* it_slot0, int32_t* it_m, int64_t* it_base, int32_t* it_done,
+                          int32_t* it_rep, void* workspace, size_t workspace_bytes, int32_t* status, int phases,
+                          pcg_stream_t stream_) {
+    cudaStream_t stream = (cudaStream_t)stream_;
+    PCG_REQUIRE(R >= 1 && R <= PCG_MAX_REL, "pcg_choose: R=%d outside [1,%d]", R, PCG_MAX_REL);
+    PCG_REQUIRE(phases >= 1 && phases <= 3, "pcg_choose: phases must be 1 (prepare), 2 (select) or 3 (both)");
+    PCG_REQUIRE(B >= 0, "pcg_choose: negative batch");
+    if (B == 0) {
+        if (status) cudaMemsetAsync(status, 0, PCG_STATUS_WORDS * sizeof(int32_t), stream);
+        return 0;
+    }
+    PCG_REQUIRE((phases & 2) == 0 || score || (entry_score && center_score), "pcg_choose: need a score table or explicit scores");
+    PCG_REQUIRE(!(train && P > 0) || (ps_score && ps_pos && ps_id), "pcg_choose: sorted pool arrays missing");
+    PCG_REQUIRE(indptr && indices && targets && sel_idx && slot_item && it_slot0 && it_m && it_base && it_done &&
+                    it_rep && status,
+                "pcg_choose: null pointer");
+    const int sms = device_sms();
+    WsLayout L = ws_layout(B, R, max_degree, n_nodes, sms);
+    PCG_REQUIRE(workspace && workspace_bytes >= L.total, "pcg_choose: workspace too small (%zu < %zu)", workspace_bytes,
+                L.total);
+    cudaError_t e;
+    ChooseP p;
+    choose_params(p, L, indptr, indices, n_nodes, row_lo, R, score, entry_score, center_score, targets, labels, B,
+                  thresh_host, k_override, rho, ps_score, ps_pos, ps_id, entry_pool_pos, P, train, sel_idx, sel_dist,
+                  cap_slots, slot_item, it_slot0, it_m, it_base, it_done, it_rep, workspace, status, stream);
+    char* ws = (char*)workspace;
     const int W = R * B;
     SideState& S = g_dev[pcg_current_device()];
     cudaStream_t* g_side = S.side;
     cudaEvent_t* g_join = S.join;
     cudaEvent_t& g_fork = S.fork;
-    if (S.huge16_state == 0) {
-        int mc = 0;
-        cudaError_t pe = launch_huge<16>(p, 1, stream, true, &mc);
-        S.huge16_state = (pe == cudaSuccess && mc >= 1) ? 1 : 2;
-        (void)cudaGetLastError();
-    }
-    p.huge16_ok = S.huge16_state == 1;
     if (phases & 1) {
         cudaLaunchConfig_t cfg = {};
         cfg.blockDim = dim3(PCG_PREP_NT);
@@ -1494,6 +1654,74 @@
     return pcg_check_launch("pcg_choose");
 }
 
+static int g_front_clusters[PCG_MAX_DEVICES];
+
+extern "C" int pcg_front(const float* feat, int64_t n_table, int F, int64_t ldf, const float* w, const float* b, float* score,
+                         const int32_t* pool, int P, float* ps_score, int32_t* ps_pos, int32_t* ps_id,
+                         const void* stage_src, void* stage_dst, size_t stage_bytes, const uint32_t* cursor, uint32_t count,
+                         int64_t src_stride_bytes, const int64_t* indptr, const int32_t* indices, int64_t n_nodes,
+                         int64_t row_lo, int R, const int32_t* targets, const int64_t* labels, int B,
+                         const double* thresh_host, double rho, const int32_t* entry_pool_pos, int64_t max_degree,
+                         int64_t cap_slots, int32_t* slot_item, int32_t* it_slot0, int32_t* it_m, int64_t* it_base,
+                         int32_t* it_done, int32_t* it_rep, void* workspace, size_t workspace_bytes, int32_t* status,
+                         pcg_stream_t stream_) {
+    cudaStream_t stream = (cudaStream_t)stream_;
+    PCG_REQUIRE(R >= 1 && R <= PCG_MAX_REL, "pcg_front: R=%d outside [1,%d]", R, PCG_MAX_REL);
+    PCG_REQUIRE(B >= 1 && (int64_t)R * B <= 8 * PCG_PREP_ITEMS, "pcg_front: %d items outside [1, %d]", R * B,
+                8 * PCG_PREP_ITEMS);
+    PCG_REQUIRE(P >= 1 && P <= FRONT_POOL_MAX, "pcg_front: pool of %d outside [1, %d]", P, FRONT_POOL_MAX);
+    PCG_REQUIRE(feat && w && score && pool && ps_score && ps_pos && ps_id && indptr && indices && targets && labels &&
+                    slot_item && it_slot0 && it_m && it_base && it_done && it_rep && status,
+                "pcg_front: null pointer");
+    PCG_REQUIRE(ldf % 4 == 0 && F <= ldf && F > 0 && ldf * 4 <= 48 * 1024 && ((uintptr_t)feat & 15) == 0,
+                "pcg_front: need F <= ldf, ldf %% 4 == 0, 16-byte aligned rows (F=%d ldf=%lld)", F, (long long)ldf);
+    PCG_REQUIRE(stage_bytes == 0 || (stage_src && stage_dst), "pcg_front: staging pointers missing");
+    PCG_REQUIRE(stage_bytes % 4 == 0 && ((uintptr_t)stage_src & 3) == 0 && ((uintptr_t)stage_dst & 3) == 0,
+                "pcg_front: the staged copy works on aligned 32-bit words");
+    PCG_REQUIRE(!cursor || (count > 0 && src_stride_bytes % 4 == 0),
+                "pcg_front: a plan cursor needs count > 0 and a stride of whole words");
+    WsLayout L = ws_layout(B, R, max_degree, n_nodes, device_sms());
+    PCG_REQUIRE(workspace && workspace_bytes >= L.total, "pcg_front: workspace too small (%zu < %zu)", workspace_bytes,
+                L.total);
+    ChooseP p;
+    choose_params(p, L, indptr, indices, n_nodes, row_lo, R, score, nullptr, nullptr, targets, labels, B, thresh_host,
+                  nullptr, rho, ps_score, ps_pos, ps_id, entry_pool_pos, P, 1, nullptr, nullptr, cap_slots, slot_item,
+                  it_slot0, it_m, it_base, it_done, it_rep, workspace, status, stream);
+    FrontP f;
+    f.feat = feat; f.n_table = n_table; f.ldf = ldf; f.F = F; f.w = w; f.b = b; f.score = score;
+    f.pool = pool; f.ps_score = ps_score; f.ps_pos = ps_pos; f.ps_id = ps_id;
+    f.stage_src = (const uint32_t*)stage_src; f.stage_dst = (uint32_t*)stage_dst; f.stage_words = (int64_t)(stage_bytes / 4);
+    f.cursor = cursor; f.count = count; f.src_stride = src_stride_bytes / 4;
+    const size_t max_dyn = (size_t)48 * 1024 + (size_t)FRONT_POOL_MAX * 8;
+    const size_t dyn = std::max((size_t)PCG_PREP_ITEMS * 4, (size_t)ldf * 4 + (size_t)P * 8);
+    cudaLaunchConfig_t cfg = {};
+    cfg.gridDim = dim3(PCG_CL);
+    cfg.blockDim = dim3(PCG_PREP_NT);
+    cfg.dynamicSmemBytes = max_dyn;
+    cfg.stream = stream;
+    cudaLaunchAttribute attr[1];
+    attr[0].id = cudaLaunchAttributeClusterDimension;
+    attr[0].val.clusterDim.x = PCG_CL; attr[0].val.clusterDim.y = 1; attr[0].val.clusterDim.z = 1;
+    cfg.attrs = attr;
+    cfg.numAttrs = 1;
+    int& most = g_front_clusters[pcg_current_device()];
+    cudaError_t e;
+    if (most == 0) {
+        e = cudaFuncSetAttribute(k_front, cudaFuncAttributeMaxDynamicSharedMemorySize, (int)max_dyn);
+        if (e == cudaSuccess) e = cudaOccupancyMaxActiveClusters(&most, k_front, &cfg);
+        if (e != cudaSuccess) { most = 0; pcg_set_error("pcg_front: occupancy: %s", cudaGetErrorString(e)); return (int)e; }
+        if (most < 3) most = 3;
+    }
+    f.n_pool_cl = std::min(std::min(FRONT_POOL_CL, (P + 511) / 512), most - 2);
+    cfg.gridDim = dim3((unsigned)(most * PCG_CL));
+    cfg.dynamicSmemBytes = dyn;
+    const int chunk = (R * B + PCG_CL - 1) / PCG_CL;
+    char* ws = (char*)workspace;
+    e = cudaLaunchKernelEx(&cfg, k_front, p, f, chunk, (int32_t*)(ws + L.bar), (int32_t*)(ws + L.totals));
+    if (e != cudaSuccess) { pcg_set_error("pcg_front: launch: %s", cudaGetErrorString(e)); return (int)e; }
+    return pcg_check_launch("pcg_front");
+}
+
 extern "C" int pcg_select_all(const int64_t* indptr, const int32_t* indices, int64_t n_nodes, int R,
                               const int32_t* targets, int B, int add_self, int64_t cap_slots, int32_t* slot_item,
                               int32_t* it_slot0, int32_t* it_m, int64_t* it_base, int32_t* it_extra, int32_t* it_done,
diff --git a/pc-gnn_b200/csrc/pcg_common.cuh b/pc-gnn_b200/csrc/pcg_common.cuh
--- a/pc-gnn_b200/csrc/pcg_common.cuh
+++ b/pc-gnn_b200/csrc/pcg_common.cuh
@@ -82,3 +82,31 @@
 __device__ __forceinline__ void f4_add(float4& a, const float4& b) {
     a.x += b.x; a.y += b.y; a.z += b.z; a.w += b.w;
 }
+
+__device__ __forceinline__ uint32_t ld_sys(const uint32_t* p) {
+    uint32_t v;
+    asm volatile("ld.volatile.global.u32 %0, [%1];" : "=r"(v) : "l"(p) : "memory");
+    return v;
+}
+__device__ __forceinline__ void st_sys(uint32_t* p, uint32_t v) {
+    asm volatile("st.volatile.global.u32 [%0], %1;" ::"l"(p), "r"(v) : "memory");
+}
+__device__ __forceinline__ void stage_copy(const uint32_t* src, uint32_t* dst, int64_t n, int64_t first, int64_t stride) {
+    for (int64_t i = first; i < n; i += 4 * stride) {
+        uint32_t v[4];
+#pragma unroll
+        for (int u = 0; u < 4; ++u) v[u] = i + u * stride < n ? ld_sys(src + i + u * stride) : 0u;
+#pragma unroll
+        for (int u = 0; u < 4; ++u)
+            if (i + u * stride < n) st_sys(dst + i + u * stride, v[u]);
+    }
+}
+
+__device__ __forceinline__ uint32_t orderable(float f) {
+    const uint32_t u = __float_as_uint(f);
+    return (u & 0x80000000u) ? ~u : (u | 0x80000000u);
+}
+
+__device__ __forceinline__ uint32_t unorderable(uint32_t k) {
+    return (k & 0x80000000u) ? (k ^ 0x80000000u) : ~k;
+}
diff --git a/pc-gnn_b200/csrc/pcg_misc.cu b/pc-gnn_b200/csrc/pcg_misc.cu
--- a/pc-gnn_b200/csrc/pcg_misc.cu
+++ b/pc-gnn_b200/csrc/pcg_misc.cu
@@ -63,25 +63,6 @@
     }
 }
 
-__device__ __forceinline__ uint32_t ld_sys(const uint32_t* p) {
-    uint32_t v;
-    asm volatile("ld.volatile.global.u32 %0, [%1];" : "=r"(v) : "l"(p) : "memory");
-    return v;
-}
-__device__ __forceinline__ void st_sys(uint32_t* p, uint32_t v) {
-    asm volatile("st.volatile.global.u32 [%0], %1;" ::"l"(p), "r"(v) : "memory");
-}
-__device__ __forceinline__ void stage_copy(const uint32_t* src, uint32_t* dst, int64_t n, int64_t first, int64_t stride) {
-    for (int64_t i = first; i < n; i += 4 * stride) {
-        uint32_t v[4];
-#pragma unroll
-        for (int u = 0; u < 4; ++u) v[u] = i + u * stride < n ? ld_sys(src + i + u * stride) : 0u;
-#pragma unroll
-        for (int u = 0; u < 4; ++u)
-            if (i + u * stride < n) st_sys(dst + i + u * stride, v[u]);
-    }
-}
-
 __global__ void __launch_bounds__(256) k_stage(const uint32_t* src, uint32_t* dst, int64_t n, uint32_t* cursor,
                                                uint32_t count, int64_t src_stride, int64_t dst_stride, int bump) {
     uint32_t at = 0;
@@ -142,14 +123,6 @@
     if (p < P) pool_score[p] = score[pool[p]];
 }
 
-__device__ __forceinline__ uint32_t orderable(float f) {
-    const uint32_t u = __float_as_uint(f);
-    return (u & 0x80000000u) ? ~u : (u | 0x80000000u);
-}
-
-__device__ __forceinline__ uint32_t unorderable(uint32_t k) {
-    return (k & 0x80000000u) ? (k ^ 0x80000000u) : ~k;
-}
 #define RANK_NT 512
 #define RANK_PER 32
 __global__ void __launch_bounds__(RANK_NT) k_sort_pool_rank(const float* __restrict__ pool_score, int gather,
diff --git a/pc-gnn_b200/engine.py b/pc-gnn_b200/engine.py
--- a/pc-gnn_b200/engine.py
+++ b/pc-gnn_b200/engine.py
@@ -348,19 +348,7 @@
         s = sel if sel is not None else self._new_selection(B, R, cap_slots, True, False)
         maxdeg = self.max_degree if max_degree is None else max_degree
         nn_ = self.N if n_nodes is None else n_nodes
-        ws_bytes = self.lib.pcg_choose_workspace_bytes(B, R, maxdeg, nn_)
-        if workspace is not None:
-            if workspace.numel() < ws_bytes:
-                raise _lib.PcgError(f"choose workspace has {workspace.numel()} bytes, this call needs {ws_bytes}")
-            ws = workspace
-        elif self._ws is None or self._ws.numel() < ws_bytes or self._ws_nodes != nn_:
-            if self._ws is None or self._ws.numel() < ws_bytes:
-                self._ws = torch.empty(int(ws_bytes), dtype=torch.uint8, device=self.device)
-            _lib.check(self.lib.pcg_choose_workspace_init(self._ws.data_ptr(), self._ws.numel(), nn_, _lib.stream_ptr()),
-                       "pcg_choose_workspace_init")
-            self._ws_nodes = nn_
-        if workspace is None:
-            ws = self._ws
+        ws, ws_bytes = self._choose_workspace(B, R, maxdeg, nn_, workspace)
         th = (C.c_double * R)(*[float(x) for x in thresh])
         use_table = entry_score is None
         if sorted_pool is None and self.sorted_pool is not None and use_table:
@@ -383,6 +371,50 @@
         _lib.check(rc, "pcg_choose")
         return (s, dist) if want_dist else s
 
+    def _choose_workspace(self, B, R, maxdeg, nn_, workspace):
+        ws_bytes = self.lib.pcg_choose_workspace_bytes(B, R, maxdeg, nn_)
+        if workspace is not None:
+            if workspace.numel() < ws_bytes:
+                raise _lib.PcgError(f"choose workspace has {workspace.numel()} bytes, this call needs {ws_bytes}")
+            return workspace, ws_bytes
+        if self._ws is None or self._ws.numel() < ws_bytes or self._ws_nodes != nn_:
+            if self._ws is None or self._ws.numel() < ws_bytes:
+                self._ws = torch.empty(int(ws_bytes), dtype=torch.uint8, device=self.device)
+            _lib.check(self.lib.pcg_choose_workspace_init(self._ws.data_ptr(), self._ws.numel(), nn_, _lib.stream_ptr()),
+                       "pcg_choose_workspace_init")
+            self._ws_nodes = nn_
+        return self._ws, ws_bytes
+
+    def front_supported(self, B: int) -> bool:
+        return (0 < self.P <= _lib.FRONT_MAX_POOL and 0 < self.R * B <= _lib.FRONT_MAX_ITEMS
+                and self.score_group is None and self._bcast is None)
+
+    def front(self, targets, labels, thresh, rho: float, cap_slots: int, clf_weight: torch.Tensor,
+              clf_bias: torch.Tensor, *, stage=None, workspace=None) -> Selection:
+        B = int(targets.shape[0])
+        R = self.R
+        if not self.front_supported(B):
+            raise _lib.PcgError(f"front: batch of {B} with a pool of {self.P} is outside what pcg_front serves")
+        s = self._new_selection(B, R, cap_slots, True, False)
+        ws, ws_bytes = self._choose_workspace(B, R, self.max_degree, self.N, workspace)
+        th = (C.c_double * R)(*[float(x) for x in thresh])
+        w = clf_weight.detach()
+        w = w if w.is_contiguous() else w.contiguous()
+        ps, pp, pi, _ = self.sorted_pool
+        cursor = stage[3] if stage is not None and len(stage) > 3 else None
+        rc = self.lib.pcg_front(
+            self.feat.data_ptr(), self.N_global, self.F, self.ldf, w.data_ptr(), clf_bias.detach().data_ptr(),
+            self.score.data_ptr(), self.pool.data_ptr(), self.P, ps.data_ptr(), pp.data_ptr(), pi.data_ptr(),
+            stage[0] if stage is not None else None, stage[1] if stage is not None else None,
+            int(stage[2]) if stage is not None else 0, cursor, int(stage[4]) if cursor else 0,
+            int(stage[5]) if cursor else 0, self.indptr.data_ptr(), self.indices.data_ptr(), self.N, self.row_lo, R,
+            targets.data_ptr(), labels.data_ptr(), B, th, float(rho), _lib.ptr(self.entry_pool_pos), self.max_degree,
+            cap_slots, s.slot_item.data_ptr(), s.it_slot0.data_ptr(), s.it_m.data_ptr(), s.it_base.data_ptr(),
+            s.it_done.data_ptr(), s.it_rep.data_ptr(), ws.data_ptr(), int(ws_bytes), s.status.data_ptr(),
+            _lib.stream_ptr())
+        _lib.check(rc, "pcg_front")
+        return s
+
     def overflow_since_reset(self) -> bool:
         if self._ws is None:
             return False
diff --git a/pc-gnn_b200/layers.py b/pc-gnn_b200/layers.py
--- a/pc-gnn_b200/layers.py
+++ b/pc-gnn_b200/layers.py
@@ -396,7 +396,10 @@
         own_scores = self.score_override is None and not self.scores_external
         stage, self.stage_in = self.stage_in, None
 
-        if own_scores and eng.P and train_flag:
+        if own_scores and train_flag and eng.front_supported(int(targets.shape[0])):
+            sel = eng.front(targets, lab, self.thresholds, rho, cap, self.label_clf.weight, self.label_clf.bias,
+                            stage=stage, workspace=workspace)
+        elif own_scores and eng.P and train_flag:
             pool_score = eng.pool_scores(self.label_clf.weight, self.label_clf.bias, stage=stage)
             side1 = eng.side_stream(1)
             side.wait_stream(cur)
diff --git a/profiles/front_roles.py b/profiles/front_roles.py
--- /dev/null
+++ b/profiles/front_roles.py
@@ -0,0 +1,42 @@
+import ctypes
+import os
+import sys
+
+import numpy as np
+import torch
+
+sys.path.insert(0, os.path.abspath(os.path.join(os.path.dirname(__file__), "..")))
+import bench
+from pcgnn_b200 import _lib
+from pcgnn_b200.engine import Engine
+from pcgnn_b200.synth import make_graph
+
+wl = sys.argv[1] if len(sys.argv) > 1 else "yelp"
+spec, batch, embed, desc = bench.WORKLOADS[wl]
+data = make_graph(spec, seed=bench.SEED)
+eng = Engine(data.graph, "cuda")
+eng.set_features(torch.from_numpy(data.feat).cuda())
+eng.set_pool(sorted(data.train_pos))
+R = data.graph.n_rel
+S = 40
+L = _lib.lib()
+trace = torch.zeros(batch * R * S + 16, dtype=torch.int64, device="cuda")
+L.pcg_debug_set_trace.argtypes = [ctypes.c_void_p]
+assert L.pcg_debug_set_trace(trace.data_ptr()) == 0
+rng = np.random.default_rng(0)
+w = torch.from_numpy(rng.normal(size=(2, data.feat.shape[1])).astype(np.float32) * 0.3).cuda()
+b = torch.zeros(2, device="cuda")
+flush = torch.empty(256 << 20, dtype=torch.uint8, device="cuda")
+print(f"{wl}: {desc}; pool {eng.P}")
+for it, (nodes, labels) in enumerate(bench.make_batches(data, 4, batch, bench.SEED)):
+    t, host = eng.upload_targets(nodes.astype(np.int32))
+    lab = torch.from_numpy(labels).cuda()
+    cap = eng.slots_bound(host, [0.5] * R, 0.5, True)
+    trace.zero_()
+    flush.zero_()
+    eng.front(t, lab, [0.5] * R, 0.5, cap, w, b)
+    torch.cuda.synchronize()
+    x = trace[batch * R * S:batch * R * S + 8].cpu().numpy().astype(np.float64)
+    t0 = x[0]
+    print(f"iter {it}: prep phases end +{(x[1] - t0) / 1e3:.1f} / +{(x[2] - t0) / 1e3:.1f} / +{(x[3] - t0) / 1e3:.1f} us; "
+          f"role ends: table +{(x[7] - t0) / 1e3:.1f} us, pool +{(x[6] - t0) / 1e3:.1f} us, prep +{(x[5] - t0) / 1e3:.1f} us")
```

Measured after the change: 10.93 million (median of 6 runs). 4.6% lower.
